# RuanJohn/Mava

Measured on AMD Instinct MI355X. Metric: env-steps/sec (whole node), ff_mappo RWARE tiny-4ag, higher is better.
Workload: dtype f32 via 2 x f16 split operands on the MFMA (3 products, f32 accumulate); 1 GPU; ff_mappo RWARE tiny-4ag-shaped synthetic obs, 4096 envs/GPU (update_batch_size=1 x num_envs=4096), rollout_length=128, ppo_epochs=4, num_minibatches=2, agents=4, obs=70/264, actions=5, one step = one PPO update = 524288 env-steps per GPU; parallelism=dp1

## Files before the change

### include/mava_hip.h

```cpp
#ifndef MAVA_HIP_H
#define MAVA_HIP_H

#include <stddef.h>
#include <stdint.h>

#ifdef __cplusplus
extern "C" {
#endif

typedef struct ihipStream_t* mava_stream_t;

const char* mava_last_error(void);
int mava_abi_version(void);

typedef struct mava_ctx mava_ctx;
enum {
  MAVA_CTX_MATMUL_MODE = 0,
  MAVA_CTX_CRITIC_AGGREGATION = 1,
  MAVA_CTX_GAE_VARIANT = 2,
  MAVA_CTX_POLICY_VARIANT = 3,
  MAVA_CTX_H2_LAUNCHES = 4,
  MAVA_CTX_TRAIN_VARIANT = 5,
  MAVA_CTX_W8_LAUNCHES = 6,
  MAVA_CTX_W1_SPLIT_FRESH = 7,
  MAVA_CTX_EXACT_TILES = 8
};
int mava_ctx_create(mava_ctx** out);
int mava_ctx_destroy(mava_ctx* ctx);
int mava_ctx_set(mava_ctx* ctx, int key, long value);
int mava_ctx_get(const mava_ctx* ctx, int key, long* value);

int mava_gae_f32(const mava_ctx* ctx, const float* reward, const float* value, const uint8_t* done,
                 const float* last_val, const uint8_t* last_done, int T, int N, float gamma,
                 float lambda, float* adv, float* tgt, mava_stream_t s);

int mava_permutation_i32(long n, uint64_t seed, uint64_t counter, int32_t* out, mava_stream_t s);

int mava_clip_adam(float* p, const float* g, float* m, float* v, int32_t* count,
                   const int* seg_off, const float* seg_lr, int n_seg, float grad_scale,
                   float max_norm, int decay, int steps_per_update, int num_updates, float b1,
                   float b2, float eps, const float* loss_sums, float vf_coef, float ent_coef,
                   float* metrics_out, mava_stream_t s);

size_t mava_ppo_finish_workspace_bytes(int Pa, int Pc);
int mava_ppo_finish_f32(mava_ctx* ctx, const float* slab_a, long stride_a, const float* slab_c, long stride_c, int n_slab,
                        int Pa, int Pc, float* g, float* p, float* m, float* v, int32_t* count, float lr_a, float lr_c,
                        float grad_scale, float max_norm, int decay, int steps_per_update, int num_updates, float b1,
                        float b2, float eps, float vf_coef, float ent_coef, float* metrics_out, int critic_din,
                        void* workspace, size_t workspace_bytes, mava_stream_t s);

int mava_slab_reduce_f32(const float* slab, int n_slab, long slab_stride, int n, int accumulate,
                         float* out, mava_stream_t s);

int mava_slab_reduce2_f32(const float* slab, int n_slab, long slab_stride, int n_main,
                          float* out_main, int n_tail, float* out_tail, int accumulate,
                          mava_stream_t s);

int mava_mlp_param_count(int din, int n_out);

int mava_mlp_forward_f32(const mava_ctx* ctx, const float* params, int din, int n_out, const float* x, int x_share,
                         int rows, float* out, mava_stream_t s);

int mava_policy_step_f32(const mava_ctx* ctx, const float* actor_params, int actor_din, int n_actions,
                         const float* agents_view, const uint8_t* action_mask,
                         const float* critic_params, int critic_din, const float* critic_input,
                         int critic_share, int critic_rows, int value_broadcast, int rows,
                         uint64_t seed, uint32_t step, const uint32_t* step_base, uint32_t row_offset, int greedy,
                         const int32_t* forced_action, int32_t* action, float* log_prob,
                         float* value, float* logits, mava_stream_t s);


int mava_adv_stats_blocks(void);

int mava_adv_stats_f64(const float* advantages, const int32_t* idx, long idx_base, int Rb, int A,
                       double* partials, mava_stream_t s);
int mava_adv_stats_batched_f64(const float* advantages, const int32_t* idx, long idx_stride, int Rb, int A,
                               int n_batch, double* partials, mava_stream_t s);

int mava_ppo_actor_grad_f32(mava_ctx* ctx, const float* params, int din, int n_actions, const float* agents_view,
                            const uint8_t* action_mask, const int32_t* action,
                            const float* old_log_prob, const float* advantages,
                            const double* adv_stats, const int32_t* idx, long idx_base, int Rb,
                            int A, float clip_eps, float ent_coef, float* slab, long slab_stride,
                            int n_slab, mava_stream_t s);

int mava_policy_step_continuous_f32(const mava_ctx* ctx, const float* actor_params, int actor_din, int action_dim, float min_scale,
                                    const float* agents_view, const float* critic_params, int critic_din,
                                    const float* critic_input, int critic_share, int critic_rows,
                                    int value_broadcast, int rows, uint64_t seed, uint32_t step,
                                    const uint32_t* step_base, uint32_t row_offset, int greedy,
                                    const float* forced_action, float* action, float* log_prob, float* value,
                                    float* mean, mava_stream_t s);
int mava_ppo_actor_grad_continuous_f32(const float* params, int din, int action_dim, float min_scale, const float* agents_view,
                                       const float* action, const float* old_log_prob, const float* advantages,
                                       const double* adv_stats, const int32_t* idx, long idx_base, int Rb, int A,
                                       float clip_eps, float ent_coef, uint64_t seed, uint32_t ent_step,
                                       uint32_t row_offset, float* slab, long slab_stride, int n_slab,
                                       mava_stream_t s);

int mava_ppo_critic_grad_f32(mava_ctx* ctx, const float* params, int din, const float* critic_input, int x_share,
                             const float* old_value, const float* targets, const int32_t* idx,
                             long idx_base, int Rb, int A, float clip_eps, float vf_coef,
                             float* slab, long slab_stride, int n_slab, mava_stream_t s);


int mava_synth_rware_step(int E, int A, int O, int n_actions, int gs_tiles, int state_dim, int time_limit,
                          uint64_t seed, uint32_t t, const uint32_t* t_base, uint32_t env_offset, int is_reset,
                          int32_t* step_count, float* run_return, int32_t* run_length,
                          float* ep_return, int32_t* ep_length, float* agents_view,
                          float* global_state, uint8_t* action_mask, int32_t* obs_step_count,
                          float* reward, uint8_t* done, float* info_return, int32_t* info_length,
                          uint8_t* info_terminal, const int32_t* action, int reward_mode, mava_stream_t s);

int mava_lbf_step(int E, int A, int F, int G, int fov, int max_agent_level, int force_coop, int individual_rewards,
                  int time_limit, uint64_t seed, uint32_t t, const uint32_t* t_base, uint32_t env_offset, int is_reset,
                  int32_t* agent_pos, int32_t* agent_level, int32_t* food_pos, int32_t* food_level, uint8_t* food_alive,
                  float* total_food_level, int32_t* step_count, float* run_return, int32_t* run_length,
                  float* ep_return, int32_t* ep_length, float* agents_view, float* global_state,
                  uint8_t* action_mask, int32_t* obs_step_count, float* reward, uint8_t* done, float* info_return,
                  int32_t* info_length, uint8_t* info_terminal, const int32_t* action, mava_stream_t s);

int mava_lbf_step_real_next(int E, int A, int F, int G, int fov, int max_agent_level, int force_coop, int individual_rewards,
                            int time_limit, uint64_t seed, uint32_t t, const uint32_t* t_base, uint32_t env_offset, int is_reset,
                            int32_t* agent_pos, int32_t* agent_level, int32_t* food_pos, int32_t* food_level, uint8_t* food_alive,
                            float* total_food_level, int32_t* step_count, float* run_return, int32_t* run_length,
                            float* ep_return, int32_t* ep_length, float* agents_view, float* global_state,
                            uint8_t* action_mask, int32_t* obs_step_count, float* reward, uint8_t* done, float* info_return,
                            int32_t* info_length, uint8_t* info_terminal, const int32_t* action, float* real_view,
                            uint8_t* real_mask, uint8_t* terminated, mava_stream_t s);

int mava_rware_step(int E, int A, int S, int R, int H, int W, int sensor_range, int time_limit, int collision_terminates,
                    const uint32_t* highway_rows, const int32_t* shelf_home, uint64_t seed, uint32_t t,
                    const uint32_t* t_base, uint32_t env_offset, int is_reset, int32_t* agent_pos, int32_t* agent_dir,
                    int32_t* agent_carry, int32_t* shelf_pos, int32_t* request_queue, int32_t* step_count,
                    float* run_return, int32_t* run_length, float* ep_return, int32_t* ep_length, float* agents_view,
                    float* global_state, uint8_t* action_mask, int32_t* obs_step_count, float* reward, uint8_t* done,
                    float* info_return, int32_t* info_length, uint8_t* info_terminal, const int32_t* action,
                    mava_stream_t s);

int mava_rware_step_real_next(int E, int A, int S, int R, int H, int W, int sensor_range, int time_limit,
                              int collision_terminates, const uint32_t* highway_rows, const int32_t* shelf_home,
                              uint64_t seed, uint32_t t, const uint32_t* t_base, uint32_t env_offset, int is_reset,
                              int32_t* agent_pos, int32_t* agent_dir, int32_t* agent_carry, int32_t* shelf_pos,
                              int32_t* request_queue, int32_t* step_count, float* run_return, int32_t* run_length,
                              float* ep_return, int32_t* ep_length, float* agents_view, float* global_state,
                              uint8_t* action_mask, int32_t* obs_step_count, float* reward, uint8_t* done,
                              float* info_return, int32_t* info_length, uint8_t* info_terminal, const int32_t* action,
                              float* real_view, uint8_t* real_mask, uint8_t* terminated, mava_stream_t s);

int mava_connector_step(int E, int A, int G, int time_limit, uint64_t seed, uint32_t t, const uint32_t* t_base,
                        uint32_t env_offset, int is_reset, int32_t* head, int32_t* target, uint8_t* connected,
                        uint8_t* grid, int32_t* step_count, float* run_return, int32_t* run_length, float* ep_return,
                        int32_t* ep_length, float* agents_view, float* global_state, uint8_t* action_mask,
                        int32_t* obs_step_count, float* reward, uint8_t* done, float* info_return, int32_t* info_length,
                        uint8_t* info_terminal, const int32_t* action, mava_stream_t s);

int mava_connector_step_real_next(int E, int A, int G, int time_limit, uint64_t seed, uint32_t t, const uint32_t* t_base,
                                  uint32_t env_offset, int is_reset, int32_t* head, int32_t* target, uint8_t* connected,
                                  uint8_t* grid, int32_t* step_count, float* run_return, int32_t* run_length,
                                  float* ep_return, int32_t* ep_length, float* agents_view, float* global_state,
                                  uint8_t* action_mask, int32_t* obs_step_count, float* reward, uint8_t* done,
                                  float* info_return, int32_t* info_length, uint8_t* info_terminal, const int32_t* action,
                                  float* real_view, uint8_t* real_mask, uint8_t* terminated, mava_stream_t s);

int mava_cleaner_step(int E, int A, int R, int C, int time_limit, uint64_t seed, uint32_t t, const uint32_t* t_base,
                      uint32_t env_offset, int is_reset, int32_t* pos, uint8_t* grid, int32_t* step_count,
                      float* run_return, int32_t* run_length, float* ep_return, int32_t* ep_length, float* agents_view,
                      float* global_state, uint8_t* action_mask, int32_t* obs_step_count, float* reward, uint8_t* done,
                      float* info_return, int32_t* info_length, uint8_t* info_terminal, uint8_t* info_won,
                      const int32_t* action, mava_stream_t s);

int mava_cleaner_step_real_next(int E, int A, int R, int C, int time_limit, uint64_t seed, uint32_t t,
                                const uint32_t* t_base, uint32_t env_offset, int is_reset, int32_t* pos, uint8_t* grid,
                                int32_t* step_count, float* run_return, int32_t* run_length, float* ep_return,
                                int32_t* ep_length, float* agents_view, float* global_state, uint8_t* action_mask,
                                int32_t* obs_step_count, float* reward, uint8_t* done, float* info_return,
                                int32_t* info_length, uint8_t* info_terminal, uint8_t* info_won, const int32_t* action,
                                float* real_view, uint8_t* real_mask, uint8_t* terminated, mava_stream_t s);

int mava_smax_step(int E, int A, int Ne, uint64_t ally_types, uint64_t enemy_types, int time_limit, int see_enemy_actions,
                   int walls_cause_death, uint64_t seed, uint32_t t, const uint32_t* t_base, uint32_t env_offset,
                   int is_reset, float* pos, float* health, int32_t* cd, int32_t* last_action, int32_t* step_count,
                   float* run_return, int32_t* run_length, float* ep_return, int32_t* ep_length, float* agents_view,
                   float* global_state, uint8_t* action_mask, int32_t* obs_step_count, float* reward, uint8_t* done,
                   float* info_return, int32_t* info_length, uint8_t* info_terminal, uint8_t* info_won,
                   const int32_t* action, mava_stream_t s);

int mava_smax_step_real_next(int E, int A, int Ne, uint64_t ally_types, uint64_t enemy_types, int time_limit,
                             int see_enemy_actions, int walls_cause_death, uint64_t seed, uint32_t t,
                             const uint32_t* t_base, uint32_t env_offset, int is_reset, float* pos, float* health,
                             int32_t* cd, int32_t* last_action, int32_t* step_count, float* run_return,
                             int32_t* run_length, float* ep_return, int32_t* ep_length, float* agents_view,
                             float* global_state, uint8_t* action_mask, int32_t* obs_step_count, float* reward,
                             uint8_t* done, float* info_return, int32_t* info_length, uint8_t* info_terminal,
                             uint8_t* info_won, const int32_t* action, float* real_view, uint8_t* real_mask,
                             uint8_t* terminated, mava_stream_t s);

int mava_spread_step(int E, int A, int add_agent_id, int time_limit, uint64_t seed, uint32_t t, const uint32_t* t_base,
                     uint32_t env_offset, int is_reset, float* agent_pos, float* landmark_pos, int32_t* step_count,
                     float* run_return, int32_t* run_length, float* ep_return, int32_t* ep_length, float* agents_view,
                     float* global_state, uint8_t* action_mask, int32_t* obs_step_count, float* reward, uint8_t* done,
                     float* info_return, int32_t* info_length, uint8_t* info_terminal, const float* action,
                     mava_stream_t s);

int mava_spread_step_real_next(int E, int A, int add_agent_id, int time_limit, uint64_t seed, uint32_t t,
                               const uint32_t* t_base, uint32_t env_offset, int is_reset, float* agent_pos,
                               float* landmark_pos, int32_t* step_count, float* run_return, int32_t* run_length,
                               float* ep_return, int32_t* ep_length, float* agents_view, float* global_state,
                               uint8_t* action_mask, int32_t* obs_step_count, float* reward, uint8_t* done,
                               float* info_return, int32_t* info_length, uint8_t* info_terminal, const float* action,
                               float* real_view, uint8_t* real_mask, uint8_t* terminated, float* real_state,
                               mava_stream_t s);

int mava_rollout_ff_f32(const float* actor_params, int n_actions, const float* critic_params, int critic_shared,
                        int E, int A, int O, int T, int time_limit, uint64_t policy_seed, uint64_t env_seed,
                        uint32_t t0, uint32_t row_offset, uint32_t env_offset, int reward_mode,
                        int32_t* step_count, float* run_return, int32_t* run_length, float* ep_return,
                        int32_t* ep_length, float* agents_view, float* global_state, uint8_t* action_mask,
                        int32_t* obs_step_count, int32_t* action, float* value, float* reward, float* log_prob,
                        uint8_t* done, float* last_val, float* info_return, int32_t* info_length,
                        uint8_t* info_terminal, float* adv, float* tgt, float gamma, float gae_lambda, mava_stream_t s);


int mava_rec_dense_f32(const mava_ctx* ctx, const float* x, int x_rowmajor, const int32_t* idx, int Rm, int E, int A,
                       int x_share, int x_ld, int accumulate, const float* w, int ldw, const float* bias,
                       const float* gate, float* y, int y_ld, int K, int N, int rows, int relu, mava_stream_t s);

int mava_rec_xty_f32(const mava_ctx* ctx, const float* x, int x_rowmajor, const int32_t* idx, int Rm, int E, int A,
                     int x_share, int x_ld, const float* y, int y_ld, const float* y_tail, int y_split, int y_tail_ld, int K, int N,
                     int rows, int want_bias, float out_scale, float* slab, long slab_stride, int n_slab, mava_stream_t s);
int mava_rec_gather_t32_f32(const float* x, const int32_t* idx, int Rm, int E, int A, int x_share, int x_ld, int K,
                            int rows, int k_pad, float* out, mava_stream_t s);

int mava_gru_scan_fwd_f32(const mava_ctx* ctx, int T, int Rm, int E, int A, const int32_t* idx, const uint8_t* done,
                          const float* h0, int h0_t32, const float* wh, const float* bhn,
                          const float* gi, float* hs, float* hprev, float* saved, mava_stream_t s);

int mava_gru_scan_bwd_f32(const mava_ctx* ctx, int T, int Rm, int E, int A, const int32_t* idx, const uint8_t* done,
                          const float* wh, const float* saved, const float* hprev, const float* dh_out,
                          float* dgi, float* dgh, int dgh_n_only, mava_stream_t s);

int mava_seq_actor_loss_f32(int T, int Rm, int E, int A, int n_actions, const int32_t* idx,
                            const float* logits, const uint8_t* mask, const int32_t* action,
                            const float* old_log_prob, const float* advantages, const double* adv_stats,
                            int n_stats, float clip_eps, float ent_coef, float grad_scale, float* dlogits,
                            float* loss_partials, int n_blocks, mava_stream_t s);
int mava_seq_actor_loss_continuous_f32(int T, int Rm, int E, int A, int action_dim, float min_scale, const int32_t* idx,
                                       const float* mean, const float* log_std, const float* log_std_rows,
                                       const float* action, const float* old_log_prob, const float* advantages,
                                       const double* adv_stats, int n_stats, float clip_eps, float ent_coef, uint64_t seed,
                                       uint32_t ent_step, uint32_t row_offset, float grad_scale, float* dmean,
                                       float* dlog_std_rows, float* loss_partials, float* dscale_partials, int n_blocks,
                                       mava_stream_t s);
int mava_seq_sample_continuous_f32(int rows, int action_dim, float min_scale, const float* mean, const float* log_std,
                                   const float* log_std_rows, uint64_t seed,
                                   uint32_t step, uint32_t row_offset, int greedy, float* action, float* log_prob,
                                   mava_stream_t s);
int mava_seq_critic_loss_f32(int T, int Rm, int E, int A, int agents_per_row, const int32_t* idx, const float* values,
                             const float* old_value, const float* targets, float clip_eps, float vf_coef,
                             float grad_scale, float* dvalues, float* loss_partials, int n_blocks, mava_stream_t s);

int mava_rec_out_f32(int T, int Rm, int E, int A, int n_out, int agents_per_row, const int32_t* idx, const float* hs,
                     const float* params_post_head, const uint8_t* mask, const int32_t* action, const float* f0,
                     const float* f1, const double* adv_stats, int n_stats, float clip_eps, float coef, float grad_scale,
                     int is_actor, float* dh, float* slab, long slab_stride, int n_slab, mava_stream_t s);

int mava_seq_sample_f32(int rows, int n_actions, const float* logits, const uint8_t* mask, uint64_t seed,
                        uint32_t step, uint32_t row_offset, int greedy, int32_t* action, float* log_prob,
                        mava_stream_t s);

int mava_rec_step_f32(const float* actor_params, int actor_din, int n_actions, const float* agents_view,
                      const uint8_t* action_mask, const uint8_t* done_a, const float* h_actor_in,
                      float* h_actor_out, int rows_a, uint64_t seed, uint32_t step, uint32_t row_offset,
                      int greedy, int32_t* action, float* log_prob, const float* critic_params, int critic_din,
                      const float* critic_input, int critic_share, const uint8_t* done_c, int done_c_stride,
                      const float* h_critic_in, float* h_critic_out, int rows_c, int value_broadcast,
                      float* value, mava_stream_t s);
int mava_rec_step_continuous_f32(const float* actor_params, int actor_din, int action_dim, float min_scale, const float* agents_view,
                                 const uint8_t* done_a, const float* h_actor_in, float* h_actor_out, int rows_a,
                                 uint64_t seed, uint32_t step, uint32_t row_offset, int greedy, float* action,
                                 float* log_prob, const float* critic_params, int critic_din,
                                 const float* critic_input, int critic_share, const uint8_t* done_c, int done_c_stride,
                                 const float* h_critic_in, float* h_critic_out, int rows_c, int value_broadcast,
                                 float* value, mava_stream_t s);

long mava_rec_step_pack_bytes(int din);
int mava_rec_step_pack_f32(const float* params, int din, void* pack, mava_stream_t s);
int mava_rec_step_packed_f32(const void* pack_a, const void* pack_c, const float* actor_params, int actor_din,
                             int n_actions, float min_scale, const float* agents_view, const uint8_t* action_mask, const uint8_t* done_a,
                             const float* h_actor_in, float* h_actor_out, int rows_a, uint64_t seed, uint32_t step,
                             uint32_t row_offset, int greedy, int32_t* action, float* action_f, float* log_prob,
                             const float* critic_params, int critic_din, const float* critic_input, int critic_share,
                             const uint8_t* done_c, int done_c_stride, const float* h_critic_in, float* h_critic_out,
                             int rows_c, int value_broadcast, float* value, mava_stream_t s);

int mava_rec_q_step_f32(const float* params, int din, int n_actions, const float* agents_view, const uint8_t* action_mask,
                        const uint8_t* done, const float* h_in, float* h_out, int rows, float eps, uint64_t seed, uint32_t step,
                        uint32_t row_offset, int32_t* action, float* q_out, mava_stream_t s);
int mava_replay_add_f32(int E, int A, int O, int n_actions, int capacity, int slot, const float* obs, const uint8_t* action_mask,
                        const int32_t* action, const float* reward, const uint8_t* terminal, const uint8_t* term_or_trunc,
                        const float* next_obs, const uint8_t* next_mask, float* b_obs, uint8_t* b_mask, int32_t* b_action,
                        float* b_reward, uint8_t* b_terminal, uint8_t* b_term_or_trunc, float* b_next_obs,
                        uint8_t* b_next_mask, mava_stream_t s);
int mava_replay_sample_f32(int E, int A, int O, int n_actions, int capacity, uint32_t n_added, int B, int S, int Rp, uint64_t seed,
                           uint32_t counter, const float* b_obs, const uint8_t* b_mask, const int32_t* b_action,
                           const float* b_reward, const uint8_t* b_terminal, const uint8_t* b_term_or_trunc,
                           const float* b_next_obs, const uint8_t* b_next_mask, float* obs, uint8_t* action_mask, int32_t* action,
                           float* reward, uint8_t* terminal, uint8_t* term_or_trunc, float* next_obs, uint8_t* next_mask,
                           int32_t* pairs, mava_stream_t s);
int mava_q_td_loss_f32(int L, int Rp, int n_actions, int n_real, const float* q, const float* q_next_online,
                       const float* q_next_target, const int32_t* action, const float* reward, const uint8_t* terminal_next,
                       const uint8_t* next_mask, float gamma, float grad_scale, float* dq, float* partials, int nblk,
                       mava_stream_t s);
int mava_target_update_f32(long n, const float* online, float* target, float tau, int hard, mava_stream_t s);

int mava_qmix_state_t32_f32(int L, int B, int A, int O, int Rp, int k_pad, const float* obs, const float* next_obs, float* state,
                            float* next_state, mava_stream_t s);
int mava_qmix_td_f32(int mode, int L, int B, int A, int Rp, int n_actions, int Em, const float* q, const float* q_next_online,
                     const float* q_next_target, const int32_t* action, const float* reward, const uint8_t* terminal_next,
                     const uint8_t* next_mask, const float* w1, const float* b1, const float* w2, const float* b2,
                     const float* w1_target, const float* b1_target, const float* w2_target, const float* b2_target, float gamma,
                     float grad_scale, float* dq, float* d_w1, float* d_b1, float* d_w2, float* d_b2, float* partials, int nblk,
                     mava_stream_t s);

int mava_sac_replay_add_f32(int E, int A, int O, int D, int S, int capacity, int head, const float* obs, const float* action,
                            const float* reward, const uint8_t* done, const float* next_obs, const float* gs,
                            const float* next_gs, float* b_obs, float* b_action, float* b_reward, uint8_t* b_done,
                            float* b_next_obs, float* b_gs, float* b_next_gs, mava_stream_t s);
int mava_sac_replay_sample_f32(int A, int O, int D, int S, int capacity, uint32_t n_added, int B, int Rp, uint64_t seed,
                               uint32_t counter, const float* b_obs, const float* b_action, const float* b_reward,
                               const uint8_t* b_done, const float* b_next_obs, const float* b_gs, const float* b_next_gs,
                               float* obs, float* action, float* reward, uint8_t* done, float* next_obs, float* gs,
                               float* next_gs, int32_t* index, mava_stream_t s);
int mava_sac_sample_f32(int rows, int n_real, int action_dim, float min_scale, const float* mean, const float* log_std,
                        uint64_t seed, uint32_t step, uint32_t row_offset, float* action, float* log_prob, float* eps,
                        mava_stream_t s);
int mava_sac_concat_f32(int rows, int n_real, int O, int x_share, int A, int action_dim, int joint, const float* state,
                        const float* action, const float* action_new, float* x, int x_ld, mava_stream_t s);
int mava_sac_q_loss_f32(int rows, int n_real, int A, const float* q1, const float* q2, const float* q1_target,
                        const float* q2_target, const float* log_prob_next, const float* reward, const uint8_t* done,
                        const float* log_alpha, float gamma, float grad_scale, float* dq1, float* dq2, float* target,
                        float* partials, int nblk, mava_stream_t s);
int mava_sac_actor_grad_f32(int rows, int n_real, int A, int action_dim, float min_scale, const float* mean,
                            const float* log_std, const float* eps, const float* action, const float* log_alpha,
                            const float* q1, const float* q2, const float* dx1, const float* dx2, int K, int action_offset,
                            int joint, float q_scale, float grad_scale, float* dmean, float* dlog_std, float* partials,
                            int nblk, mava_stream_t s);
int mava_sac_alpha_loss_f32(int n_real, int A, const float* log_prob, const float* log_alpha, float target_entropy,
                            float* grad, float* loss_parts, mava_stream_t s);

int mava_t32_convert_f32(const float* src, int N, int rows, int to_t32, float* dst, mava_stream_t s);

int mava_t32_norm_act_f32(const float* x, int N, long rows, int use_layer_norm, const float* ln_bias, int act, float* y,
                          float* xhat, float* rstd, mava_stream_t s);
int mava_t32_norm_act_bwd_f32(const float* dy, const float* y, int N, long rows, int use_layer_norm, const float* xhat,
                              const float* rstd, int act, float* dz, float* dx, mava_stream_t s);
int mava_t32_gru_mask_f32(const float* h, const uint8_t* done_t, const int32_t* idx, int E, int A, int Hd, long rows,
                          float* hprev, mava_stream_t s);
int mava_t32_gru_gates_f32(const float* gi, const float* gh, const float* bhn, const float* hprev, int Hd, long rows, float* hs,
                           float* saved, float* hprev_next, const uint8_t* done_next, const int32_t* idx, int E, int A,
                           mava_stream_t s);
int mava_t32_gru_gates_bwd_f32(const float* saved, const float* hprev, const float* dh_out, const float* acc_next,
                               const float* dhp_next, const uint8_t* done_next, const int32_t* idx, int E, int A, int Hd,
                               long rows, float* dgi, float* dgh, float* dhp, mava_stream_t s);
int mava_t32_colsum_f32(const float* y, int N, long rows, float scale, float* slab, long slab_stride, int n_slab,
                        mava_stream_t s);
int mava_t32_im2col_f32(const float* src, int src_flat, long samples, int Hin, int Win, int C, int k, int stride,
                        float* dst, mava_stream_t s);
int mava_t32_col2im_f32(const float* dcol, int src_flat, long samples, int Hin, int Win, int C, int k, int stride,
                        float* dsrc, mava_stream_t s);
int mava_t32_flatten_f32(const float* src, long samples, int P, int C, int to_flat, float* dst, mava_stream_t s);

int mava_mat_attn_fwd_f32(const float* q, const float* k, const float* v, long rows, int D, int B, int A, int n_head,
                          int causal, float* y, float* p, int n_blocks, mava_stream_t s);
int mava_mat_attn_bwd_f32(const float* dy, const float* q, const float* k, const float* v, long rows, int D, int B, int A,
                          int n_head, int causal, float* dq, float* dk, float* dv, int n_blocks, mava_stream_t s);
int mava_mat_ln_fwd_f32(const float* x, const float* res, const float* scale, const float* bias, int N, long rows,
                        long valid_rows, float* y, float* xhat, float* rstd, int n_blocks, mava_stream_t s);
int mava_mat_ln_bwd_f32(const float* dy, const float* xhat, const float* rstd, const float* scale, int N, long rows,
                        long valid_rows, float out_scale, float* dx, float* slab, long slab_stride, int n_slab, mava_stream_t s);
int mava_mat_gelu_f32(const float* x, long n, float* y, mava_stream_t s);
int mava_mat_gelu_bwd_f32(const float* dy, const float* x, long n, float* dx, mava_stream_t s);
int mava_mat_shift_onehot_f32(const int32_t* action, const int32_t* idx, int B, int A, int n_actions, int known, long rows,
                              int n_pad, float* out, mava_stream_t s);
int mava_mat_sample_f32(int B, int A, int agent, int n_actions, const float* logits, const uint8_t* mask, uint64_t seed,
                        uint32_t step, uint32_t row_offset, int greedy, int32_t* action, float* log_prob, mava_stream_t s);
int mava_mat_loss_f32(int Bm, int A, int n_actions, long rows, const int32_t* idx, const float* logits, const float* values,
                      const uint8_t* mask, const int32_t* action, const float* old_log_prob, const float* advantages,
                      const float* old_value, const float* targets, const double* adv_stats, int n_stats, float clip_eps,
                      float ent_coef, float vf_coef, float grad_scale, float* dlogits, float* dvalues, float* loss_partials,
                      int n_blocks, mava_stream_t s);

int mava_comm_unique_id(uint8_t* id128);
int mava_comm_create(void** h, int rank, int world, const uint8_t* id128);
int mava_allreduce_sum_f32(void* h, float* buf, size_t n, mava_stream_t s);
int mava_broadcast_f32(void* h, float* buf, size_t n, int root, mava_stream_t s);
int mava_comm_destroy(void* h);

#ifdef __cplusplus
}
#endif
#endif
```

### mava_amd/_lib.py

```python
from __future__ import annotations

import ctypes as C
import os
from typing import Optional

import torch

_HERE = os.path.dirname(os.path.abspath(__file__))
LIB_PATH = os.environ.get("MAVA_LIB_PATH") or os.path.join(_HERE, "libmavahip.so")

_lib: Optional[C.CDLL] = None


class MavaHipError(RuntimeError):
    pass


vp = C.c_void_p
i32 = C.c_int
u32 = C.c_uint32
u64 = C.c_uint64
f32 = C.c_float
lng = C.c_long

_SIGNATURES = {
    "mava_abi_version": [],
    "mava_ctx_create": [vp],
    "mava_ctx_destroy": [vp],
    "mava_ctx_set": [vp, i32, lng],
    "mava_ctx_get": [vp, i32, vp],
    "mava_gae_f32": [vp, vp, vp, vp, vp, vp, i32, i32, f32, f32, vp, vp, vp],
    "mava_permutation_i32": [lng, u64, u64, vp, vp],
    "mava_clip_adam": [vp, vp, vp, vp, vp, C.POINTER(i32), C.POINTER(f32), i32, f32, f32, i32, i32, i32,
                       f32, f32, f32, vp, f32, f32, vp, vp],
    "mava_slab_reduce_f32": [vp, i32, lng, i32, i32, vp, vp],
    "mava_ppo_finish_workspace_bytes": [i32, i32],
    "mava_ppo_finish_f32": [vp, vp, lng, vp, lng, i32, i32, i32, vp, vp, vp, vp, vp, f32, f32, f32, f32, i32, i32, i32, f32, f32, f32,
                            f32, f32, vp, i32, vp, C.c_size_t, vp],
    "mava_slab_reduce2_f32": [vp, i32, lng, i32, vp, i32, vp, i32, vp],
    "mava_mlp_param_count": [i32, i32],
    "mava_mlp_forward_f32": [vp, vp, i32, i32, vp, i32, i32, vp, vp],
    "mava_policy_step_f32": [vp, vp, i32, i32, vp, vp, vp, i32, vp, i32, i32, i32, i32, u64, u32, vp, u32, i32,
                             vp, vp, vp, vp, vp, vp],
    "mava_policy_step_continuous_f32": [vp, vp, i32, i32, f32, vp, vp, i32, vp, i32, i32, i32, i32, u64, u32, vp, u32, i32, vp, vp, vp, vp, vp, vp],
    "mava_ppo_actor_grad_continuous_f32": [vp, i32, i32, f32, vp, vp, vp, vp, vp, vp, lng, i32, i32, f32, f32, u64, u32, u32, vp, lng, i32, vp],
    "mava_seq_actor_loss_continuous_f32": [i32, i32, i32, i32, i32, f32, vp, vp, vp, vp, vp, vp, vp, vp, i32, f32, f32, u64, u32, u32, f32, vp, vp, vp, vp, i32, vp],
    "mava_seq_sample_continuous_f32": [i32, i32, f32, vp, vp, vp, u64, u32, u32, i32, vp, vp, vp],
    "mava_adv_stats_blocks": [],
    "mava_adv_stats_f64": [vp, vp, lng, i32, i32, vp, vp],
    "mava_adv_stats_batched_f64": [vp, vp, lng, i32, i32, i32, vp, vp],
    "mava_ppo_actor_grad_f32": [vp, vp, i32, i32, vp, vp, vp, vp, vp, vp, vp, lng, i32, i32, f32, f32, vp, lng, i32,
                                vp],
    "mava_ppo_critic_grad_f32": [vp, vp, i32, vp, i32, vp, vp, vp, lng, i32, i32, f32, f32, vp, lng, i32, vp],
    "mava_synth_rware_step": [i32, i32, i32, i32, i32, i32, i32, u64, u32, vp, u32, i32] + [vp] * 14 + [vp, i32, vp],
    "mava_lbf_step": [i32] * 9 + [u64, u32, vp, u32, i32] + [vp] * 21 + [vp],
    "mava_lbf_step_real_next": [i32] * 9 + [u64, u32, vp, u32, i32] + [vp] * 24 + [vp],
    "mava_rware_step": [i32] * 9 + [vp, vp, u64, u32, vp, u32, i32] + [vp] * 20 + [vp],
    "mava_rware_step_real_next": [i32] * 9 + [vp, vp, u64, u32, vp, u32, i32] + [vp] * 23 + [vp],
    "mava_connector_step": [i32] * 4 + [u64, u32, vp, u32, i32] + [vp] * 19 + [vp],
    "mava_connector_step_real_next": [i32] * 4 + [u64, u32, vp, u32, i32] + [vp] * 22 + [vp],
    "mava_cleaner_step": [i32] * 5 + [u64, u32, vp, u32, i32] + [vp] * 18 + [vp],
    "mava_cleaner_step_real_next": [i32] * 5 + [u64, u32, vp, u32, i32] + [vp] * 21 + [vp],
    "mava_smax_step": [i32] * 3 + [u64, u64] + [i32] * 3 + [u64, u32, vp, u32, i32] + [vp] * 20 + [vp],
    "mava_smax_step_real_next": [i32] * 3 + [u64, u64] + [i32] * 3 + [u64, u32, vp, u32, i32] + [vp] * 23 + [vp],
    "mava_spread_step": [i32] * 4 + [u64, u32, vp, u32, i32] + [vp] * 17 + [vp],
    "mava_spread_step_real_next": [i32] * 4 + [u64, u32, vp, u32, i32] + [vp] * 21 + [vp],
    "mava_rec_q_step_f32": [vp, i32, i32, vp, vp, vp, vp, vp, i32, f32, u64, u32, u32, vp, vp, vp],
    "mava_replay_add_f32": [i32] * 6 + [vp] * 16 + [vp],
    "mava_replay_sample_f32": [i32] * 5 + [u32, i32, i32, i32, u64, u32] + [vp] * 17 + [vp],
    "mava_q_td_loss_f32": [i32, i32, i32, i32] + [vp] * 7 + [f32, f32, vp, vp, i32, vp],
    "mava_target_update_f32": [lng, vp, vp, f32, i32, vp],
    "mava_qmix_state_t32_f32": [i32] * 6 + [vp] * 4 + [vp],
    "mava_qmix_td_f32": [i32] * 7 + [vp] * 15 + [f32, f32] + [vp] * 6 + [i32, vp],
    "mava_sac_replay_add_f32": [i32] * 7 + [vp] * 14 + [vp],
    "mava_sac_replay_sample_f32": [i32] * 5 + [u32, i32, i32, u64, u32] + [vp] * 15 + [vp],
    "mava_sac_sample_f32": [i32, i32, i32, f32, vp, vp, u64, u32, u32, vp, vp, vp, vp],
    "mava_sac_concat_f32": [i32] * 7 + [vp] * 4 + [i32, vp],
    "mava_sac_q_loss_f32": [i32] * 3 + [vp] * 8 + [f32, f32] + [vp] * 4 + [i32, vp],
    "mava_sac_actor_grad_f32": [i32] * 4 + [f32] + [vp] * 9 + [i32, i32, i32, f32, f32] + [vp] * 3 + [i32, vp],
    "mava_sac_alpha_loss_f32": [i32, i32, vp, vp, f32, vp, vp, vp],
    "mava_rollout_ff_f32": [vp, i32, vp, i32, i32, i32, i32, i32, i32, u64, u64, u32, u32, u32, i32] + [vp] * 18 + [vp, vp, f32, f32, vp],
    "mava_rec_dense_f32": [vp, vp, i32, vp, i32, i32, i32, i32, i32, i32, vp, i32, vp, vp, vp, i32, i32, i32, i32, i32, vp],
    "mava_rec_xty_f32": [vp, vp, i32, vp, i32, i32, i32, i32, i32, vp, i32, vp, i32, i32, i32, i32, i32, i32, f32, vp, lng, i32, vp],
    "mava_rec_gather_t32_f32": [vp, vp, i32, i32, i32, i32, i32, i32, i32, i32, vp, vp],
    "mava_gru_scan_fwd_f32": [vp, i32, i32, i32, i32, vp, vp, vp, i32, vp, vp, vp, vp, vp, vp, vp],
    "mava_t32_gru_mask_f32": [vp, vp, vp, i32, i32, i32, lng, vp, vp],
    "mava_t32_gru_gates_f32": [vp, vp, vp, vp, i32, lng, vp, vp, vp, vp, vp, i32, i32, vp],
    "mava_t32_gru_gates_bwd_f32": [vp, vp, vp, vp, vp, vp, vp, i32, i32, i32, lng, vp, vp, vp, vp],
    "mava_gru_scan_bwd_f32": [vp, i32, i32, i32, i32, vp, vp, vp, vp, vp, vp, vp, vp, i32, vp],
    "mava_seq_actor_loss_f32": [i32, i32, i32, i32, i32, vp, vp, vp, vp, vp, vp, vp, i32, f32, f32, f32, vp, vp, i32, vp],
    "mava_rec_step_continuous_f32": [vp, i32, i32, f32, vp, vp, vp, vp, i32, u64, u32, u32, i32, vp, vp, vp, i32, vp, i32, vp, i32, vp, vp, i32, i32, vp, vp],
    "mava_rec_step_f32": [vp, i32, i32, vp, vp, vp, vp, vp, i32, u64, u32, u32, i32, vp, vp, vp, i32, vp, i32, vp, i32, vp, vp,
                          i32, i32, vp, vp],
    "mava_seq_critic_loss_f32": [i32, i32, i32, i32, i32, vp, vp, vp, vp, f32, f32, f32, vp, vp, i32, vp],
    "mava_rec_out_f32": [i32, i32, i32, i32, i32, i32, vp, vp, vp, vp, vp, vp, vp, vp, i32, f32, f32, f32, i32, vp, vp, lng, i32, vp],
    "mava_rec_step_pack_bytes": [i32],
    "mava_t32_norm_act_f32": [vp, i32, lng, i32, vp, i32, vp, vp, vp, vp],
    "mava_t32_norm_act_bwd_f32": [vp, vp, i32, lng, i32, vp, vp, i32, vp, vp, vp],
    "mava_t32_colsum_f32": [vp, i32, lng, f32, vp, lng, i32, vp],
    "mava_t32_im2col_f32": [vp, i32, lng, i32, i32, i32, i32, i32, vp, vp],
    "mava_t32_col2im_f32": [vp, i32, lng, i32, i32, i32, i32, i32, vp, vp],
    "mava_t32_flatten_f32": [vp, lng, i32, i32, i32, vp, vp],
    "mava_comm_unique_id": [vp],
    "mava_comm_create": [vp, i32, i32, vp],
    "mava_allreduce_sum_f32": [vp, vp, C.c_size_t, vp],
    "mava_broadcast_f32": [vp, vp, C.c_size_t, i32, vp],
    "mava_comm_destroy": [vp],
    "mava_rec_step_pack_f32": [vp, i32, vp, vp],
    "mava_rec_step_packed_f32": [vp, vp, vp, i32, i32, f32, vp, vp, vp, vp, vp, i32, u64, u32, u32, i32, vp, vp, vp, vp, i32, vp, i32, vp, i32, vp, vp, i32, i32, vp, vp],
    "mava_seq_sample_f32": [i32, i32, vp, vp, u64, u32, u32, i32, vp, vp, vp],
    "mava_t32_convert_f32": [vp, i32, i32, i32, vp, vp],
    "mava_mat_attn_fwd_f32": [vp, vp, vp, lng, i32, i32, i32, i32, i32, vp, vp, i32, vp],
    "mava_mat_attn_bwd_f32": [vp, vp, vp, vp, lng, i32, i32, i32, i32, i32, vp, vp, vp, i32, vp],
    "mava_mat_ln_fwd_f32": [vp, vp, vp, vp, i32, lng, lng, vp, vp, vp, i32, vp],
    "mava_mat_ln_bwd_f32": [vp, vp, vp, vp, i32, lng, lng, f32, vp, vp, lng, i32, vp],
    "mava_mat_gelu_f32": [vp, lng, vp, vp],
    "mava_mat_gelu_bwd_f32": [vp, vp, lng, vp, vp],
    "mava_mat_shift_onehot_f32": [vp, vp, i32, i32, i32, i32, lng, i32, vp, vp],
    "mava_mat_sample_f32": [i32, i32, i32, i32, vp, vp, u64, u32, u32, i32, vp, vp, vp],
    "mava_mat_loss_f32": [i32, i32, i32, lng, vp, vp, vp, vp, vp, vp, vp, vp, vp, vp, i32, f32, f32, f32, f32, vp, vp, vp, i32, vp],
}
_RESTYPES = {"mava_last_error": C.c_char_p, "mava_rec_step_pack_bytes": C.c_long, "mava_ppo_finish_workspace_bytes": C.c_size_t}


def declared_symbols():
    return sorted(set(_SIGNATURES) | set(_RESTYPES))


def lib() -> C.CDLL:
    global _lib
    if _lib is None:
        if not os.path.exists(LIB_PATH):
            raise MavaHipError(
                f"{LIB_PATH} is missing: build it with `python -m mava_amd.build` "
                "(hipcc --offload-arch=gfx950). There is no CPU fallback."
            )
        _lib = C.CDLL(LIB_PATH)
        _lib.mava_last_error.restype = C.c_char_p
        _lib.mava_last_error.argtypes = []
        for name, args in _SIGNATURES.items():
            fn = getattr(_lib, name)
            fn.argtypes = args
            fn.restype = _RESTYPES.get(name, C.c_int)
    return _lib


class Ctx:

    MATMUL_MODE, CRITIC_AGGREGATION, GAE_VARIANT, POLICY_VARIANT, H2_LAUNCHES, TRAIN_VARIANT, W8_LAUNCHES, W1_SPLIT_FRESH = 0, 1, 2, 3, 4, 5, 6, 7
    EXACT_TILES = 8

    def __init__(self, matmul_mode: str = "f32", critic_aggregation: bool = True):
        if matmul_mode not in ("f32", "f16x2"):
            raise ValueError(f"matmul_mode must be 'f16x2' or 'f32', got {matmul_mode!r}")
        h = C.c_void_p()
        check(lib().mava_ctx_create(C.byref(h)), "mava_ctx_create")
        self.handle: Optional[int] = h.value
        self.set(self.MATMUL_MODE, 1 if matmul_mode == "f16x2" else 0)
        self.set(self.CRITIC_AGGREGATION, int(bool(critic_aggregation)))

    def set(self, key: int, value: int) -> None:
        check(lib().mava_ctx_set(self.handle, key, int(value)), "mava_ctx_set")

    def get(self, key: int) -> int:
        out = C.c_long()
        check(lib().mava_ctx_get(self.handle, key, C.byref(out)), "mava_ctx_get")
        return int(out.value)

    @property
    def matmul_mode(self) -> str:
        return "f16x2" if self.get(self.MATMUL_MODE) == 1 else "f32"

    @property
    def h2_launches(self) -> int:
        return self.get(self.H2_LAUNCHES)

    def close(self) -> None:
        if getattr(self, "handle", None) is not None and _lib is not None:
            _lib.mava_ctx_destroy(self.handle)
        self.handle = None

    def __del__(self):
        try:
            self.close()
        except Exception:
            pass


def ctx_ptr(ctx: Optional["Ctx"]) -> Optional[int]:
    return None if ctx is None else ctx.handle


def check(rc: int, what: str) -> None:
    if rc != 0:
        msg = lib().mava_last_error().decode("utf-8", "replace")
        raise MavaHipError(f"{what} failed with code {rc}: {msg}")


TIMERS: Optional[dict] = None


def launch(what: str, fn, *args, ok=(0,)) -> int:
    if TIMERS is None:
        rc = fn(*args)
    else:
        a, b = torch.cuda.Event(enable_timing=True), torch.cuda.Event(enable_timing=True)
        a.record()
        rc = fn(*args)
        b.record()
        TIMERS.setdefault(what, []).append((a, b))
    if rc not in ok:
        check(rc, what)
    return rc


def ptr(t: Optional[torch.Tensor]) -> Optional[int]:
    if t is None:
        return None
    return t.data_ptr()


def stream_ptr() -> int:
    return torch.cuda.current_stream().cuda_stream
```

### mava_amd/csrc/permutation.hip

```cpp
#include "common.h"

namespace {

constexpr int PERM_ROUNDS = 16;

struct PermKeys {
  uint32_t k[PERM_ROUNDS];
};

__device__ __host__ inline uint32_t perm_mix(uint32_t x, uint32_t k) {
  uint32_t h = x + k;
  h ^= h >> 16;
  h *= 0x7FEB352Du;
  h ^= h >> 15;
  h *= 0x846CA68Bu;
  h ^= h >> 16;
  return h;
}

__global__ __launch_bounds__(256) void permutation_kernel(uint32_t n, int lb, int rb, PermKeys keys,
                                                          int32_t* __restrict__ out) {
  const uint32_t i = blockIdx.x * 256u + threadIdx.x;
  if (i >= n) return;
  const uint32_t mask_r = (1u << rb) - 1u;
  uint32_t v = i;
  do {
    uint32_t L = v >> rb, R = v & mask_r;
#pragma unroll
    for (int r = 0; r < PERM_ROUNDS; r += 2) {
      L ^= perm_mix(R, keys.k[r]) >> (32 - lb);
      R ^= perm_mix(L, keys.k[r + 1]) >> (32 - rb);
    }
    v = (L << rb) | R;
  } while (v >= n);
  out[i] = (int32_t)v;
}

}

extern "C" int mava_permutation_i32(long n, uint64_t seed, uint64_t counter, int32_t* out, hipStream_t s) {
  MAVA_ARG_CHECK(n >= 1 && n < (1L << 31), 0, "mava_permutation_i32: n=%ld (1 <= n < 2^31)", n);
  MAVA_ARG_CHECK(out, 1, "mava_permutation_i32: null pointer argument");
  int b = 2;
  while ((1L << b) < n) ++b;
  const int lb = b >> 1, rb = b - lb;
  PermKeys keys;
  uint64_t st = seed + 0x9E3779B97F4A7C15ull * (counter + 1);
  for (int r = 0; r < PERM_ROUNDS; ++r) {
    st += 0x9E3779B97F4A7C15ull;
    uint64_t z = st;
    z = (z ^ (z >> 30)) * 0xBF58476D1CE4E5B9ull;
    z = (z ^ (z >> 27)) * 0x94D049BB133111EBull;
    z ^= z >> 31;
    keys.k[r] = (uint32_t)(z >> 32);
  }
  hipLaunchKernelGGL(permutation_kernel, dim3(mava_cdiv(n, 256)), dim3(256), 0, s, (uint32_t)n, lb, rb, keys, out);
  MAVA_LAUNCH_CHECK();
  return MAVA_OK;
}
```

### mava_amd/csrc/ppo_train.hip

```cpp
#include "mlp_core.h"
#include "ppo_train_task.h"
#include "ctx.h"
#include "tanh_normal.h"

namespace {

constexpr int STATS_BLOCKS = 128;
constexpr int LDT = 33;


#ifdef MAVA_STAMPS
#define STAMP_DECL unsigned long long st_prev = __builtin_readcyclecounter(), st_acc[16] = {0, 0, 0, 0, 0, 0, 0, 0, 0, 0, 0, 0, 0, 0, 0, 0};
#define STAMP(i)                                                   \
  do {                                                             \
    const unsigned long long st_now = __builtin_readcyclecounter(); \
    st_acc[i] += st_now - st_prev;                                 \
    st_prev = st_now;                                              \
  } while (0)
#else
#define STAMP_DECL
#define STAMP(i)
#endif

struct TrainLdsLayout {
  int h1t, h2t, dz2t, dz1t, yp, dy, xs, misc, end;
  int ldx;
};

template <int NO>
TrainLdsLayout make_layout(int kt1) {
  TrainLdsLayout L;
  const int tile = MLP_H * LDT;
  L.h1t = MlpLds<NO>::END;
  L.h2t = L.h1t + tile;
  L.dz2t = L.h2t + tile;
  L.yp = L.dz2t + tile;
  L.dy = L.yp + 4 * 32 * (NO + 1);
  L.ldx = 32 * kt1 + 4;
  L.xs = (L.dy + 32 * LDT + 3) & ~3;
  L.misc = L.xs + 32 * L.ldx;
  L.end = L.misc + 16;
  L.dz1t = L.h2t;
  if ((size_t)(L.end + tile) * sizeof(float) <= 163840) {
    L.dz1t = L.end;
    L.end += tile;
  }
  return L;
}

__global__ __launch_bounds__(256) void adv_stats_kernel(const float* __restrict__ adv,
                                                        const int32_t* __restrict__ idx,
                                                        long idx_base, int Rb, int A,
                                                        double* __restrict__ partials, long idx_stride) {
  __shared__ double sh[2][4];
  if (idx) idx += (long)blockIdx.y * idx_stride;
  partials += (long)blockIdx.y * 2 * gridDim.x;
  double s1 = 0.0, s2 = 0.0;
  const long stride = (long)gridDim.x * 256;
  for (long b0 = (long)blockIdx.x * 256 + threadIdx.x; b0 < Rb; b0 += 4 * stride) {
    long p[4];
#pragma unroll
    for (int u = 0; u < 4; ++u) {
      const long b = b0 + u * stride;
      const long bc = b < Rb ? b : b0;
      p[u] = idx ? (long)idx[bc] : idx_base + bc;
    }
#pragma unroll
    for (int u = 0; u < 4; ++u) {
      if (b0 + u * stride < Rb) {
        const float* row = adv + p[u] * A;
        for (int a = 0; a < A; ++a) {
          const double v = (double)row[a];
          s1 += v;
          s2 += v * v;
        }
      }
    }
  }
  for (int o = 32; o > 0; o >>= 1) {
    s1 += __shfl_down(s1, o, 64);
    s2 += __shfl_down(s2, o, 64);
  }
  const int lane = threadIdx.x & 63, w = threadIdx.x >> 6;
  if (lane == 0) { sh[0][w] = s1; sh[1][w] = s2; }
  __syncthreads();
  if (threadIdx.x == 0) {
    partials[2 * blockIdx.x + 0] = ((sh[0][0] + sh[0][1]) + sh[0][2]) + sh[0][3];
    partials[2 * blockIdx.x + 1] = ((sh[1][0] + sh[1][1]) + sh[1][2]) + sh[1][3];
  }
}

template <int V, int NR>
__device__ __forceinline__ void stage_load(const float* __restrict__ xrow, int nv, int l8, float (&xr)[NR]) {
#pragma unroll
  for (int i = 0; i < NR / V; ++i) {
    const int c = l8 + 8 * i;
    const int cc = (c < nv) ? c : 0;
    if (V == 4) {
      const float4 v = reinterpret_cast<const float4*>(xrow)[cc];
      xr[4 * i + 0] = v.x; xr[4 * i + 1] = v.y; xr[4 * i + 2] = v.z; xr[4 * i + 3] = v.w;
    } else {
      xr[i] = xrow[cc];
    }
  }
}
template <int V, int NR>
__device__ __forceinline__ void stage_write(float* xs_row, float* dummy, int nv, int l8, const float (&xr)[NR]) {
#pragma unroll
  for (int i = 0; i < NR / V; ++i) {
    const int c = l8 + 8 * i;
    float* q = (c < nv) ? (xs_row + V * c) : dummy;
    if (V == 4) {
      *reinterpret_cast<float4*>(q) = make_float4(xr[4 * i + 0], xr[4 * i + 1], xr[4 * i + 2], xr[4 * i + 3]);
    } else {
      *q = xr[i];
    }
  }
}

template <int CTRL>
__device__ __forceinline__ float dpp_f(float v) {
  return __builtin_bit_cast(float, __builtin_amdgcn_update_dpp(0, __builtin_bit_cast(int, v), CTRL, 0xF, 0xF, true));
}
template <int G, typename Op>
__device__ __forceinline__ float group_allreduce(float v, Op op) {
  v = op(v, dpp_f<0xB1>(v));
  v = op(v, dpp_f<0x4E>(v));
  if (G >= 8) v = op(v, dpp_f<0x141>(v));
  if (G >= 16) v = op(v, dpp_f<0x140>(v));
  if (G >= 32) v = op(v, __shfl_xor(v, 16, 64));
  return v;
}

template <int NO, int KT1, bool ACTOR, int XV, bool CONT>
__global__ __launch_bounds__(256, 1) void ppo_train_kernel(TrainTask tk, TrainLdsLayout L) {
  static_assert(!CONT || ACTOR, "the continuous head belongs to the actor");
  extern __shared__ __attribute__((aligned(16))) float lds[];
  float* const W2s = lds + MlpLds<NO>::W2;
  float* const W3s = lds + MlpLds<NO>::W3;
  float* const H1T = lds + L.h1t;
  float* const H2T = lds + L.h2t;
  float* const DZ1T = lds + L.dz1t;
  float* const DZ2T = lds + L.dz2t;
  float* const YP = lds + L.yp;
  float* const DY = lds + L.dy;
  float* const XS = lds + L.xs;
  float* const misc = lds + L.misc;
  constexpr int ldx = 32 * KT1 + 4;

  const int tid = threadIdx.x;
  const int lane = tid & 63, w = tid >> 6, h = lane >> 5, j = lane & 31;
  const int srow = tid >> 3, l8 = tid & 7;
  const int din = tk.din, no = tk.no;
  const long R = (!ACTOR && tk.agg > 1) ? (long)tk.Rb : (long)tk.Rb * tk.A;
  const float invR = 1.0f / (float)((long)tk.Rb * tk.A);
  constexpr int NR = 4 * KT1;

  mlp_fill_lds<NO>(lds, tk.params, din, no, 256);
  for (int i = tid; i < 32 * ldx; i += 256) XS[i] = 0.0f;
  for (int i = tid; i < 32 * LDT; i += 256) DY[i] = 0.0f;
  __syncthreads();
  if (tid < 32) XS[tid * ldx + din] = 1.0f;
  if (ACTOR && tid == 0) {
    double s1 = 0.0, s2 = 0.0;
    for (int i = 0; i < STATS_BLOCKS; ++i) { s1 += tk.stats[2 * i]; s2 += tk.stats[2 * i + 1]; }
    const double mean = s1 / (double)R;
    double var = s2 / (double)R - mean * mean;
    if (var < 0.0) var = 0.0;
    misc[0] = (float)mean;
    misc[1] = 1.0f / ((float)sqrt(var) + 1e-8f);
  }
  __syncthreads();
  const float adv_mean = ACTOR ? misc[0] : 0.0f;
  const float adv_rstd = ACTOR ? misc[1] : 0.0f;

  const float* const wcol1 = tk.params + 32 * w + j;
  const int fbase = 32 * w + 4 * h;

  f32x16 gW1[KT1], gW2[4];
#pragma unroll
  for (int t = 0; t < KT1; ++t)
#pragma unroll
    for (int r = 0; r < 16; ++r) gW1[t][r] = 0.0f;
#pragma unroll
  for (int t = 0; t < 4; ++t)
#pragma unroll
    for (int r = 0; r < 16; ++r) gW2[t][r] = 0.0f;
  f32x16 gW3;
#pragma unroll
  for (int r = 0; r < 16; ++r) gW3[r] = 0.0f;
  float w3h[16];
#pragma unroll
  for (int r = 0; r < 16; ++r) {
    const int f = fbase + (r & 3) + 8 * (r >> 2);
    w3h[r] = ACTOR ? ((j < NO) ? W3s[f * NO + j] : 0.0f) : W3s[f];
  }
  float w3a[ACTOR ? NO / 2 : 1];
#pragma unroll
  for (int s2 = 0; s2 < (ACTOR ? NO / 2 : 1); ++s2)
    w3a[s2] = ACTOR ? W3s[(32 * w + j) * NO + 2 * s2 + h] : 0.0f;
  float ab3 = 0.0f;
  float ab2[16], aW3r[ACTOR ? 1 : 16];
#pragma unroll
  for (int r = 0; r < 16; ++r) ab2[r] = 0.0f;
#pragma unroll
  for (int r = 0; r < (ACTOR ? 1 : 16); ++r) aW3r[r] = 0.0f;
  float loss_a = 0.f, loss_b = 0.f;
  float als = 0.0f;
  const float ls_raw = CONT ? tk.params[mlp_param_count(tk.din, tk.no) + ((lane & (NO - 1)) < tk.no ? (lane & (NO - 1)) : 0)] : 0.0f;
  const float sc_lo = CONT ? tn::scale_of(ls_raw, tk.min_scale) : 1.0f;


  constexpr int NP = ACTOR ? NO / 8 : 1;
  constexpr int GR = ACTOR ? 64 / NO : 32;
  const int lo = ACTOR ? (lane & (NO - 1)) : 0;
  auto loss_row = [&](int q) -> int { return ACTOR ? (8 * w + q * GR + lane / NO) : j; };
  const int slot = 2 * w + h;
  const int slot_c = (!ACTOR && tk.agg > 1) ? (slot < tk.agg ? slot : 0) : 0;
  auto load_row = [&](long fr, int& act, float& f0, float& f1, uint32_t& m) {
    if (ACTOR && CONT) {
      act = __builtin_bit_cast(int, tk.action_f[fr * no + (lo < no ? lo : 0)]);
      f0 = tk.old_logp[fr];
      f1 = tk.adv[fr];
      m = (uint32_t)fr;
    } else if (ACTOR) {
      act = tk.action[fr];
      f0 = tk.old_logp[fr];
      f1 = tk.adv[fr];
      const uint8_t* mk = (tk.mask != nullptr && lo < no) ? (tk.mask + fr * no + lo) : nullptr;
      m = 1u;
      if (mk != nullptr) m = *mk;
    } else {
      act = 0;
      const long fa = (tk.agg > 1) ? fr * tk.agg + slot_c : fr;
      f0 = tk.old_value[fa];
      f1 = tk.targets[fa];
      m = 0u;
    }
  };
  const uint32_t Au = (!ACTOR && tk.agg > 1) ? 1u : (uint32_t)tk.A;

  const uint32_t q_step = 32u * gridDim.x, b_step = q_step / Au, a_step = q_step % Au;
  const uint32_t b_last = (uint32_t)(R - 1) / Au, a_last = (uint32_t)(R - 1) % Au;
  struct Cursor { uint32_t q, b, a; };
  auto cursor_at = [&](int r) {
    Cursor c;
    c.q = 32u * blockIdx.x + (uint32_t)r;
    c.b = c.q / Au;
    c.a = c.q - c.b * Au;
    return c;
  };
  auto cursor_advance = [&](Cursor& c) {
    c.q += q_step; c.b += b_step; c.a += a_step;
    if (c.a >= Au) { c.a -= Au; c.b += 1u; }
  };
  auto cursor_gather = [&](const Cursor& c, int32_t& p_raw, uint32_t& a_out) {
    const bool in = c.q < (uint32_t)R;
    const uint32_t b = in ? c.b : b_last;
    a_out = in ? c.a : a_last;
    p_raw = tk.idx ? tk.idx[b] : (int32_t)(tk.idx_base + (long)b);
  };
  auto stage_row = [&](int32_t p_raw, uint32_t a) -> uint32_t {
    const uint32_t fr = (uint32_t)p_raw * Au + a;
    return (tk.xshare == 1) ? fr : ((uint32_t)tk.xshare == Au ? (uint32_t)p_raw : fr / (uint32_t)tk.xshare);
  };
  float* const xs_dummy = misc + 4;
  auto stage_issue = [&](uint32_t xrow_idx, float (&xr)[NR]) {
    stage_load<XV, NR>(tk.x + (long)xrow_idx * din, din / XV, l8, xr);
  };
  auto stage_commit = [&](const float (&xr)[NR]) {
    stage_write<XV, NR>(XS + srow * ldx, xs_dummy, din / XV, l8, xr);
  };

  constexpr int RD = (2 * KT1 <= 6) ? (2 * KT1) : (((2 * KT1) % 6 == 0) ? 6 : 4);
  constexpr bool W1_RESIDENT = (RD == 2 * KT1);
  float wr[RD][8];
  const float* const wcol1h = wcol1 + 8 * h * MLP_H;
#pragma unroll
  for (int d = 0; d < RD; ++d)
#pragma unroll
    for (int s = 0; s < 8; ++s) wr[d][s] = wcol1h[(16 * d + s) * MLP_H];

  const long ntiles = (R + 31) / 32;
  long it = blockIdx.x;
  float xr[NR];
  int r_act[NP] = {}, n_act[NP] = {};
  float r_f0[NP] = {}, r_f1[NP] = {}, n_f0[NP] = {}, n_f1[NP] = {};
  uint32_t r_m[NP] = {}, n_m[NP] = {};
  Cursor cs = cursor_at(srow), cl[NP];
#pragma unroll
  for (int q = 0; q < NP; ++q) cl[q] = cursor_at(loss_row(q));
  int32_t ps_next = 0, pl_next[NP] = {};
  uint32_t as_next = 0, al_next[NP] = {};
  if (it < ntiles) {
    cursor_gather(cs, ps_next, as_next);
    stage_issue(stage_row(ps_next, as_next), xr);
#pragma unroll
    for (int q = 0; q < NP; ++q) {
      cursor_gather(cl[q], pl_next[q], al_next[q]);
      load_row((long)((uint32_t)pl_next[q] * Au + al_next[q]), r_act[q], r_f0[q], r_f1[q], r_m[q]);
    }
    stage_commit(xr);
    cursor_advance(cs);
#pragma unroll
    for (int q = 0; q < NP; ++q) cursor_advance(cl[q]);
    if (it + gridDim.x < ntiles) {
      cursor_gather(cs, ps_next, as_next);
#pragma unroll
      for (int q = 0; q < NP; ++q) cursor_gather(cl[q], pl_next[q], al_next[q]);
      cursor_advance(cs);
#pragma unroll
      for (int q = 0; q < NP; ++q) cursor_advance(cl[q]);
    }
  }
  __syncthreads();

  STAMP_DECL
  for (; it < ntiles; it += gridDim.x) {
    STAMP(9);
    const bool valid = (it * 32 + j) < R;
    const long itn = it + gridDim.x;
    const bool have_next = itn < ntiles;
    uint32_t xrow_next = stage_row(ps_next, as_next);
    uint32_t fr_next[NP];
#pragma unroll
    for (int q = 0; q < NP; ++q) fr_next[q] = (uint32_t)pl_next[q] * Au + al_next[q];
    asm volatile("" : "+v"(xrow_next));
#pragma unroll
    for (int q = 0; q < NP; ++q) asm volatile("" : "+v"(fr_next[q]));

    f32x16 h1;
#pragma unroll
    for (int r = 0; r < 16; ++r) h1[r] = 0.0f;
    {
      const float* xb = XS + j * ldx + 8 * h;
      constexpr int NB = 2 * KT1;
      static_assert(NB % RD == 0, "ring depth must divide the batch count");
      float xo[RD][8];
      {
        const float4 v0 = *reinterpret_cast<const float4*>(xb), v1 = *reinterpret_cast<const float4*>(xb + 4);
        xo[0][0] = v0.x; xo[0][1] = v0.y; xo[0][2] = v0.z; xo[0][3] = v0.w;
        xo[0][4] = v1.x; xo[0][5] = v1.y; xo[0][6] = v1.z; xo[0][7] = v1.w;
      }
#pragma unroll 1
      for (int g = 0; g < NB / RD; ++g) {
#pragma unroll
        for (int d = 0; d < RD; ++d) {
          const int b = g * RD + d;
          const int bn = (b + 1 < NB) ? (b + 1) : b;
          {
            const float4 v0 = *reinterpret_cast<const float4*>(xb + 16 * bn);
            const float4 v1 = *reinterpret_cast<const float4*>(xb + 16 * bn + 4);
            float(&xn)[8] = xo[(d + 1) % RD];
            xn[0] = v0.x; xn[1] = v0.y; xn[2] = v0.z; xn[3] = v0.w;
            xn[4] = v1.x; xn[5] = v1.y; xn[6] = v1.z; xn[7] = v1.w;
          }
          if (16 * b <= din) {
#pragma unroll
            for (int s = 0; s < 8; ++s) h1 = MFMA32(wr[d][s], xo[d][s], h1);
          }
          if (!W1_RESIDENT) {
            int bf = b - 1 + RD;
            bf = (bf >= NB) ? (bf - NB) : bf;
            const float* wb = wcol1h + bf * (16 * MLP_H);
#pragma unroll
            for (int s = 0; s < 8; ++s) wr[(d + RD - 1) % RD][s] = wb[s * MLP_H];
          }
          __builtin_amdgcn_sched_barrier(0);
        }
      }
      if (!W1_RESIDENT) {
#pragma unroll
        for (int s = 0; s < 8; ++s) wr[RD - 1][s] = wcol1h[(16 * (RD - 1) + s) * MLP_H];
      }
    }
    STAMP(12);
    uint32_t relu1 = 0;
// ... 557 lines not shown
```

### mava_amd/csrc/rollout_h2.hip

```cpp
#include "h2_core.h"

#ifdef MAVA_STAMPS
#define RSTAMP_DECL unsigned long long rs_prev = __builtin_readcyclecounter(), rs_acc[8] = {0, 0, 0, 0, 0, 0, 0, 0};
#define RSTAMP(i)                                                   \
  do {                                                              \
    __builtin_amdgcn_sched_barrier(0);                              \
    const unsigned long long rs_now = __builtin_readcyclecounter(); \
    rs_acc[i] += rs_now - rs_prev;                                  \
    rs_prev = rs_now;                                               \
    __builtin_amdgcn_sched_barrier(0);                              \
  } while (0)
static __device__ unsigned long long g_rollout_stamps[16];
#else
#define RSTAMP_DECL
#define RSTAMP(i)
#endif

namespace {
using namespace h2;
typedef _Float16 half2v __attribute__((ext_vector_type(2)));

constexpr uint32_t ENV_STREAM = 0x454E5653u;
constexpr uint32_t POLICY_STREAM = 0x504f4c49u;

struct RolloutArgs {
  const float* pa;
  const float* pc;
  int E, A, O, no, T, time_limit;
  uint32_t pseed_lo, pseed_hi, eseed_lo, eseed_hi;
  uint32_t t0;
  uint32_t row_offset;
  uint32_t env_offset;
  int reward_mode;
  int32_t* step_count;
  float* run_return; int32_t* run_length; float* ep_return; int32_t* ep_length;
  float* agents_view;
  float* global_state;
  uint8_t* action_mask;
  int32_t* obs_step_count;
  int32_t* action; float* value; float* reward; float* log_prob; uint8_t* done;
  float* last_val;
  float* info_return; int32_t* info_length; uint8_t* info_terminal;
  float* adv; float* tgt;
  float gamma, lam;
};

struct RolloutLds {
  int xa, xa_row, xa_plane, xc, xc_row, xc_plane, h1, wl, ypa, ypc, act, mask, small, gum, xlf, end;
};
constexpr int W1_REG_STEPS = 12;

template <int NO, int S1A, int S1C, bool SHARED>
RolloutLds make_rollout_lds() {
  constexpr int KTA = (S1A + 1) / 2, KTC = (S1C + 1) / 2;
  RolloutLds L;
  L.xa = 0;
  L.xa_row = 2 * 32 * KTA + 16;
  L.xa_plane = 32 * L.xa_row;
  L.xc = L.xa + 2 * 2 * L.xa_plane;
  L.xc_row = 2 * 32 * KTC + 16;
  L.xc_plane = ((S1C > W1_REG_STEPS) ? 16 : 32) * L.xc_row;
  L.h1 = L.xc + (SHARED ? 2 * L.xc_plane : 0);
  L.wl = L.h1 + (SHARED ? 3 : 4) * IMG_BYTES;
  L.ypa = L.wl + ((S1C > W1_REG_STEPS) ? (S1C - W1_REG_STEPS) * 4 * 64 * 32 : 0);
  L.ypc = L.ypa + 2 * 4 * 32 * (NO + 1) * 4;
  L.act = L.ypc + 2 * 4 * 32 * 4;
  L.mask = L.act + 64 * 4;
  L.small = L.mask + 64 * 32;
  L.gum = L.small + (128 + 32 + 128 + 4 + 128) * 4;
  L.gum = (L.gum + 15) & ~15;
  L.xlf = L.gum + 64 * NO * 4;
  L.end = L.xlf + 16;
  L.end = (L.end + 15) & ~15;
  return L;
}

template <int NO, int S1A, int S1C, bool SHARED, int ROLE>
__device__ __forceinline__ void rollout_body(const RolloutArgs& a, const RolloutLds& L, u8* lds) {
  constexpr bool ACT_ROLE = ROLE == 0;
  const int t512 = threadIdx.x;
  const int tid = t512 & 255, lane = tid & 63, w = tid >> 6, h = lane >> 5, r = lane & 31;
  const int A = a.A, O = a.O, no = a.no, W = A + O, E = a.E;
  const int EB = 64 / A;
  const int e0 = blockIdx.x * EB;
  const int din_a = W, din_c = SHARED ? A * O : W;
  constexpr int NTC = SHARED ? 1 : 2;
  float* const B2a = reinterpret_cast<float*>(lds + L.small);
  float* const B3a = B2a + 128;
  float* const B2c = B3a + 32;
  float* const B3c = B2c + 128;
  float* const W3c = B3c + 4;
  int* const ACT = reinterpret_cast<int*>(lds + L.act);
  u8* const MASK = lds + L.mask;
  float* const GUM = reinterpret_cast<float*>(lds + L.gum);
  unsigned* const XLF = reinterpret_cast<unsigned*>(lds + L.xlf);
  float* const YPA = reinterpret_cast<float*>(lds + L.ypa);
  float* const YPC = reinterpret_cast<float*>(lds + L.ypc);
  const int xa_row = L.xa_row, xa_plane = L.xa_plane, xc_row = L.xc_row, xc_plane = L.xc_plane;

  for (int i = t512 * 16; i < L.end; i += 512 * 16) *reinterpret_cast<uint4*>(lds + i) = make_uint4(0, 0, 0, 0);
  __syncthreads();
  const int oW2a = mlp_off_w2(din_a), oW3a = mlp_off_w3(din_a), oW2c = mlp_off_w2(din_c), oW3c = mlp_off_w3(din_c);
  if (ACT_ROLE) {
    if (tid < 128) B2a[tid] = a.pa[mlp_off_b2(din_a) + tid];
    if (tid < no) B3a[tid] = a.pa[mlp_off_b3(din_a, no) + tid];
  } else {
    if (tid < 128) {
      B2c[tid] = a.pc[mlp_off_b2(din_c) + tid];
      W3c[tid] = a.pc[oW3c + tid];
    }
    if (tid == 0) B3c[0] = a.pc[mlp_off_b3(din_c, 1)];
  }
  constexpr int S1R = ACT_ROLE ? S1A : S1C;
  constexpr int S1REG = (S1R > W1_REG_STEPS) ? W1_REG_STEPS : S1R;
  constexpr int XC_ROWS = (S1C > W1_REG_STEPS) ? 16 : 32;
  uint4* const WL = reinterpret_cast<uint4*>(lds + L.wl) + 2 * (w * 64 + lane);
  const float* const PR = ACT_ROLE ? a.pa : a.pc;
  const int din_r = ACT_ROLE ? din_a : din_c, oW2r = ACT_ROLE ? oW2a : oW2c;
  Frag W1r[S1REG], W2r[8], W3h[2];
  {
    float c1 = 0.0f, c2 = 0.0f;
#pragma unroll
    for (int s = 0; s < S1R; ++s) {
      float v[8];
#pragma unroll
      for (int e = 0; e < 8; ++e) {
        const int k = 16 * s + 8 * h + e;
        v[e] = (k <= din_r) ? PR[k * MLP_H + 32 * w + r] : 0.0f;
      }
      const Frag f = split8_carry(v, c1);
      if (s < S1REG) {
        W1r[s] = f;
      } else {
        WL[512 * (s - S1REG)] = __builtin_bit_cast(uint4, f.hi);
        WL[512 * (s - S1REG) + 1] = __builtin_bit_cast(uint4, f.lo);
      }
      __builtin_amdgcn_sched_barrier(0);
    }
#pragma unroll
    for (int s = 0; s < 8; ++s) {
      float v[8];
#pragma unroll
      for (int e = 0; e < 8; ++e) v[e] = PR[oW2r + (16 * s + 8 * h + e) * MLP_H + 32 * w + r];
      W2r[s] = split8_carry(v, c2);
      __builtin_amdgcn_sched_barrier(0);
    }
#pragma unroll
    for (int s = 0; s < (ACT_ROLE ? 2 : 0); ++s) {
      float v[8];
#pragma unroll
      for (int e = 0; e < 8; ++e) {
        const int f = 32 * w + 16 * s + 8 * (e >> 2) + 4 * h + (e & 3);
        v[e] = (r < no) ? a.pa[oW3a + f * no + r] * W3_SCALE : 0.0f;
      }
      W3h[s] = split8(v);
    }
  }
  {
    const long slot0_av = 0;
    uint32_t lo_any = 0;
    for (int i = t512; i < 64 * W; i += 512) {
      const int row = i / W, c = i - row * W;
      const int e = e0 + row / A;
      const float v = (e < E) ? a.agents_view[slot0_av + ((long)e0 * A + row) * W + c] : 0.0f;
      _Float16 x0, x1;
      split1(v, x0, x1);
      u8* p = lds + L.xa + (row >> 5) * 2 * xa_plane + (row & 31) * xa_row + 2 * c;
      *reinterpret_cast<_Float16*>(p) = x0;
      *reinterpret_cast<_Float16*>(p + xa_plane) = x1;
      lo_any |= (uint32_t)__builtin_bit_cast(uint16_t, x1) & 0x7FFFu;
    }
    if (t512 < 64) {
      u8* p = lds + L.xa + (t512 >> 5) * 2 * xa_plane + (t512 & 31) * xa_row + 2 * din_a;
      *reinterpret_cast<_Float16*>(p) = (_Float16)1.0f;
    }
    if (SHARED) {
      const int gw = A * O;
      for (int i = t512; i < EB * gw; i += 512) {
        const int le = i / gw, c = i - le * gw;
        const float v = (e0 + le < E) ? a.global_state[(long)(e0 + le) * gw + c] : 0.0f;
        _Float16 x0, x1;
        split1(v, x0, x1);
        u8* p = lds + L.xc + le * xc_row + 2 * c;
        *reinterpret_cast<_Float16*>(p) = x0;
        *reinterpret_cast<_Float16*>(p + xc_plane) = x1;
        lo_any |= (uint32_t)__builtin_bit_cast(uint16_t, x1) & 0x7FFFu;
      }
      if (t512 < XC_ROWS) *reinterpret_cast<_Float16*>(lds + L.xc + t512 * xc_row + 2 * din_c) = (_Float16)1.0f;
    }
    for (int i = t512; i < 64 * no; i += 512) {
      const int row = i / no, o = i - row * no;
      MASK[row * 32 + o] = (e0 + row / A < E) ? a.action_mask[((long)e0 * A + row) * no + o] : 1;
    }
    if (lo_any != 0) *XLF = 1u;
  }
  __syncthreads();

  const int bk_le = tid / A, bk_ag = tid - bk_le * A;
  const bool bk_on = !ACT_ROLE && tid < 64 && (e0 + bk_le) < E;
  const long bk_k = (long)(e0 + bk_le) * A + bk_ag;
  int sc_reg = bk_on ? a.step_count[bk_k] : 0;
  float rr_reg = 0.0f, er_reg = 0.0f;
  int rl_reg = 0, el_reg = 0;
  if (bk_on && bk_ag == 0) {
    rr_reg = a.run_return[e0 + bk_le]; rl_reg = a.run_length[e0 + bk_le];
    er_reg = a.ep_return[e0 + bk_le]; el_reg = a.ep_length[e0 + bk_le];
  }

  const bool x_lo = __builtin_amdgcn_readfirstlane((int)*XLF) != 0;
  const int rowB = r * IMG_ROW + 16 * h;
  const long EA = (long)E * A;
  const uint32_t nch = (O - 2 + 15) / 16 > 0 ? (O - 2 + 15) / 16 : 1;

  constexpr int NT = ACT_ROLE ? 2 : NTC;
  RSTAMP_DECL
  auto forward = [&](bool active, bool noise, uint32_t noise_step) __attribute__((always_inline)) {
    f32x16 z[NT];
#pragma unroll
    for (int i = 0; i < NT; ++i)
#pragma unroll
      for (int q = 0; q < 16; ++q) z[i][q] = 0.0f;
    if (active) {
      auto x_frag = [&](int s, int t) {
        return (!ACT_ROLE && SHARED) ? read_row_frag(lds + L.xc, xc_plane, (r & (XC_ROWS - 1)) * xc_row + 16 * h + 32 * s)
                                     : read_row_frag(lds + L.xa + t * 2 * xa_plane, xa_plane, r * xa_row + 16 * h + 32 * s);
      };
      auto w_frag = [&](int s) {
        Frag wf;
        wf.hi = __builtin_bit_cast(half8, WL[512 * (s - S1REG)]);
        wf.lo = __builtin_bit_cast(half8, WL[512 * (s - S1REG) + 1]);
        return wf;
      };
      auto x_hi = [&](int s, int t) -> half8 {
        return (!ACT_ROLE && SHARED)
                   ? *reinterpret_cast<const half8*>(lds + L.xc + (r & (XC_ROWS - 1)) * xc_row + 16 * h + 32 * s)
                   : *reinterpret_cast<const half8*>(lds + L.xa + t * 2 * xa_plane + r * xa_row + 16 * h + 32 * s);
      };
      if (x_lo) {
      Frag bn[NT], wn;
#pragma unroll
      for (int t = 0; t < NT; ++t) bn[t] = x_frag(0, t);
      if (S1REG == 0) wn = w_frag(0);
#pragma unroll
      for (int s = 0; s < S1R; ++s) {
        Frag b[NT];
#pragma unroll
        for (int t = 0; t < NT; ++t) b[t] = bn[t];
        const Frag wf = (s < S1REG) ? W1r[s < S1REG ? s : 0] : wn;
        if (s + 1 < S1R) {
#pragma unroll
          for (int t = 0; t < NT; ++t) bn[t] = x_frag(s + 1, t);
          if (s + 1 >= S1REG) wn = w_frag(s + 1);
        }
#pragma unroll
        for (int t = 0; t < NT; ++t) z[t] = mfma3(wf, b[t], z[t]);
        __builtin_amdgcn_sched_barrier(0);
      }
      } else {
      half8 bn[NT];
      Frag wn;
#pragma unroll
      for (int t = 0; t < NT; ++t) bn[t] = x_hi(0, t);
      if (S1REG == 0) wn = w_frag(0);
#pragma unroll
      for (int s = 0; s < S1R; ++s) {
        half8 b[NT];
#pragma unroll
        for (int t = 0; t < NT; ++t) b[t] = bn[t];
        const Frag wf = (s < S1REG) ? W1r[s < S1REG ? s : 0] : wn;
        if (s + 1 < S1R) {
#pragma unroll
          for (int t = 0; t < NT; ++t) bn[t] = x_hi(s + 1, t);
          if (s + 1 >= S1REG) wn = w_frag(s + 1);
        }
#pragma unroll
        for (int t = 0; t < NT; ++t) {
          z[t] = __builtin_amdgcn_mfma_f32_32x32x16_f16(wf.lo, b[t], z[t], 0, 0, 0);
          z[t] = __builtin_amdgcn_mfma_f32_32x32x16_f16(wf.hi, b[t], z[t], 0, 0, 0);
        }
        __builtin_amdgcn_sched_barrier(0);
      }
      }
#pragma unroll
      for (int i = 0; i < NT; ++i) {
#pragma unroll
        for (int q = 0; q < 16; ++q) z[i][q] = fmaxf(z[i][q], 0.0f);
        half4 ph[4], pl[4];
        write_image(lds + L.h1 + ((ACT_ROLE ? 0 : 2) + i) * IMG_BYTES, r, 32 * w + 4 * h, z[i], ph, pl);
      }
    }
    if (ACT_ROLE && noise) {
      const int grow = tid >> 2, c = tid & 3;
      if (c < NO / 4) {
        const uint32_t gid = a.row_offset + (uint32_t)(e0 * A + grow);
        const Philox4 rnd = philox4x32_10(gid, noise_step, (uint32_t)c, POLICY_STREAM, a.pseed_lo, a.pseed_hi);
        float4 g;
        g.x = -logf(-logf(u01_open(rnd.x)));
        g.y = -logf(-logf(u01_open(rnd.y)));
        g.z = -logf(-logf(u01_open(rnd.z)));
        g.w = -logf(-logf(u01_open(rnd.w)));
        *reinterpret_cast<float4*>(GUM + grow * NO + 4 * c) = g;
      }
    }
    RSTAMP(0);
    __syncthreads();
    RSTAMP(1);
    if (active) {
      const float* b2 = ACT_ROLE ? B2a : B2c;
#pragma unroll
      for (int i = 0; i < NT; ++i)
#pragma unroll
        for (int q = 0; q < 16; ++q) z[i][q] = b2[32 * w + (q & 3) + 8 * (q >> 2) + 4 * h];
      {
        auto h_frag = [&](int s, int t) {
          return read_row_frag(lds + L.h1 + ((ACT_ROLE ? 0 : 2) + t) * IMG_BYTES, IMG_PLANE, rowB + 32 * s);
        };
        Frag bn[NT];
#pragma unroll
        for (int t = 0; t < NT; ++t) bn[t] = h_frag(0, t);
#pragma unroll
        for (int s = 0; s < 8; ++s) {
          Frag b[NT];
#pragma unroll
          for (int t = 0; t < NT; ++t) b[t] = bn[t];
          if (s + 1 < 8) {
#pragma unroll
            for (int t = 0; t < NT; ++t) bn[t] = h_frag(s + 1, t);
          }
#pragma unroll
          for (int t = 0; t < NT; ++t) z[t] = mfma3(W2r[s], b[t], z[t]);
          __builtin_amdgcn_sched_barrier(0);
        }
      }
      if (ACT_ROLE) {
#pragma unroll
        for (int t = 0; t < NT; ++t) {
          half4 ph[4], pl[4];
#pragma unroll
          for (int g = 0; g < 4; ++g)
#pragma unroll
            for (int e = 0; e < 4; ++e) {
              _Float16 x0, x1;
              split1(fmaxf(z[t][4 * g + e], 0.0f), x0, x1);
              ph[g][e] = x0;
              pl[g][e] = x1;
            }
          f32x16 y;
#pragma unroll
          for (int q = 0; q < 16; ++q) y[q] = 0.0f;
#pragma unroll
          for (int s = 0; s < 2; ++s) {
            Frag b;
            b.hi = __builtin_shufflevector(ph[2 * s], ph[2 * s + 1], 0, 1, 2, 3, 4, 5, 6, 7);
            b.lo = __builtin_shufflevector(pl[2 * s], pl[2 * s + 1], 0, 1, 2, 3, 4, 5, 6, 7);
            y = mfma3(W3h[s], b, y);
          }
#pragma unroll
          for (int q = 0; q < 16; ++q) {
            const int o = (q & 3) + 8 * (q >> 2) + 4 * h;
            if ((q & 3) + 8 * (q >> 2) < NO) {
              if (o < NO) YPA[((t * 4 + w) * 32 + r) * (NO + 1) + o] = y[q] * W3_UNSCALE;
            }
          }
        }
      } else {
#pragma unroll
        for (int t = 0; t < NT; ++t) {
          float4 w3g[4];
#pragma unroll
          for (int g = 0; g < 4; ++g) w3g[g] = *reinterpret_cast<const float4*>(W3c + 32 * w + 4 * h + 8 * g);
          float part = 0.0f;
#pragma unroll
          for (int q = 0; q < 16; ++q) {
            const float4 tv = w3g[q >> 2];
            const float w3 = (q & 3) == 0 ? tv.x : (q & 3) == 1 ? tv.y : (q & 3) == 2 ? tv.z : tv.w;
            part = fmaf(fmaxf(z[t][q], 0.0f), w3, part);
          }
          part += __shfl_xor(part, 32, 64);
          if (h == 0) YPC[(t * 4 + w) * 32 + r] = part;
        }
      }
    }
    RSTAMP(2);
    __syncthreads();
    RSTAMP(3);
  };
  auto value_of = [&](int crow) -> float {
    const float* yp = YPC + (crow >> 5) * 4 * 32 + (crow & 31);
    return (((yp[0] + yp[32]) + yp[64]) + yp[96]) + B3c[0];
  };

  const int rows_ok = min(64, (E - e0) * A), envs_ok = min(EB, E - e0);
  const int AO = A * O;
  auto write_out = [&](long slot, bool part_gs) {
    if (!part_gs) {
      float* dst = a.agents_view + (slot * EA + (long)e0 * A) * W;
      if ((W & 1) == 0) {
        const int W2 = W >> 1, d_r = 256 / W2, d_f = 256 - d_r * W2;
        int row = tid / W2, f = tid - row * W2;
        for (int j = tid; j < 64 * W2; j += 256) {
          if (row < rows_ok) {
            const u8* xa = lds + L.xa + (row >> 5) * 2 * xa_plane + (row & 31) * xa_row;
            const half2v v = *reinterpret_cast<const half2v*>(xa + 4 * f);
            reinterpret_cast<float2*>(dst)[j] = make_float2((float)v[0], (float)v[1]);
          }
          row += d_r; f += d_f;
          if (f >= W2) { f -= W2; ++row; }
        }
      } else {
        const int d_r = 256 / W, d_f = 256 - d_r * W;
        int row = tid / W, f = tid - row * W;
        for (int j = tid; j < 64 * W; j += 256) {
          if (row < rows_ok) {
            const u8* xa = lds + L.xa + (row >> 5) * 2 * xa_plane + (row & 31) * xa_row;
            dst[j] = (float)*reinterpret_cast<const _Float16*>(xa + 2 * f);
          }
          row += d_r; f += d_f;
          if (f >= W) { f -= W; ++row; }
        }
      }
    }
    if (part_gs && SHARED && a.global_state != nullptr) {
      float* dst = a.global_state + (slot * E + e0) * (long)AO;
      if ((AO & 3) == 0) {
        const int Q = AO >> 2, d_r = 256 / Q, d_f = 256 - d_r * Q;
        int le = tid / Q, k = tid - le * Q;
        for (int j = tid; j < EB * Q; j += 256) {
          if (le < envs_ok) {
            const half4 v = *reinterpret_cast<const half4*>(lds + L.xc + le * xc_row + 8 * k);
            reinterpret_cast<float4*>(dst)[j] = make_float4((float)v[0], (float)v[1], (float)v[2], (float)v[3]);
          }
          le += d_r; k += d_f;
          if (k >= Q) { k -= Q; ++le; }
        }
      } else {
        const int d_r = 256 / AO, d_f = 256 - d_r * AO;
        int le = tid / AO, k = tid - le * AO;
        for (int j = tid; j < EB * AO; j += 256) {
          if (le < envs_ok) dst[j] = (float)*reinterpret_cast<const _Float16*>(lds + L.xc + le * xc_row + 2 * k);
          le += d_r; k += d_f;
          if (k >= AO) { k -= AO; ++le; }
        }
      }
    }
    if (!part_gs) {
      uint8_t* dst = a.action_mask + (slot * EA + (long)e0 * A) * no;
      for (int j = tid; j < rows_ok * no; j += 256) {
        const int row = j / no, o = j - row * no;
        dst[j] = MASK[row * 32 + o];
      }
    }
  };

  for (int t = 0; t < a.T; ++t) {
    const uint32_t step = a.t0 + (uint32_t)t;
    forward(true, true, step);
    if (ACT_ROLE) {
      constexpr int RPP = 256 / NO;
#pragma unroll
      for (int pass = 0; pass < 64 / RPP; ++pass) {
        const int row = pass * RPP + tid / NO, o = tid & (NO - 1);
        const float* yp = YPA + (((row >> 5) * 4) * 32 + (row & 31)) * (NO + 1) + o;
        const float y = (((yp[0] + yp[32 * (NO + 1)]) + yp[2 * 32 * (NO + 1)]) + yp[3 * 32 * (NO + 1)]) + B3a[o];
        const bool legal = (o < no) && (MASK[row * 32 + o] != 0);
        const float z = legal ? y : -FLT_MAX;
        auto fmax_op = [](float p, float q) { return fmaxf(p, q); };
        auto add_op = [](float p, float q) { return p + q; };
        const float mx = group_allreduce<NO>(z, fmax_op);
        const float se = group_allreduce<NO>(expf(z - mx), add_op);
        const float logp = (mx == -FLT_MAX) ? ((o < no) ? -logf((float)no) : -FLT_MAX) : z - (mx + logf(se));
        float sc = (o < no) ? (z + GUM[row * NO + o]) : -FLT_MAX;
        if (!(sc > -FLT_MAX)) sc = -FLT_MAX;
        int best = o;
#pragma unroll
        for (int m = 1; m < NO; m <<= 1) {
          const float so = __shfl_xor(sc, m, 64);
          const int bo = __shfl_xor(best, m, 64);
          const bool take = (so > sc) || (so == sc && bo < best);
          sc = take ? so : sc;
          best = take ? bo : best;
        }
        const float lp = group_allreduce<NO>((o == best) ? logp : 0.0f, add_op);
        const int e = e0 + row / A;
        if (o == 0) {
          ACT[row] = best;
          if (e < E) {
            const long k = (long)t * EA + (long)e0 * A + row;
            a.action[k] = best;
            a.log_prob[k] = lp;
          }
        }
      }
    } else {
      if (tid < 64 && (e0 + tid / A) < E) {
        a.value[(long)t * EA + (long)e0 * A + tid] = value_of(SHARED ? tid / A : tid);
      }
      if (t > 0) write_out((long)t, false);
    }
    if (ACT_ROLE && t > 0) write_out((long)t, true);
    RSTAMP(4);
    __syncthreads();
    RSTAMP(5);
    {
      const uint32_t tn = step + 1;
      const long slot = (long)(t + 1);
      const uint32_t n_view = (uint32_t)(64 * nch);
      for (uint32_t i = ACT_ROLE ? (uint32_t)tid : n_view; i < n_view; i += 256) {
        const uint32_t row = i / nch, c = i - row * nch;
        const uint32_t le = row / A, ag = row - le * A, e = e0 + le;
        if ((int)e >= E) continue;
        const uint32_t ent = (a.env_offset + e) * A + ag;
        const Philox4 rv = philox4x32_10(ent, tn, c, ENV_STREAM, a.eseed_lo, a.eseed_hi);
        const uint32_t wds[4] = {rv.x, rv.y, rv.z, rv.w};
        const uint32_t f0 = 2 + 16 * c;
        const int n = (int)min(16u, (uint32_t)O - f0);
        u8* xa = lds + L.xa + (row >> 5) * 2 * xa_plane + (row & 31) * xa_row;
        u8* xc = lds + L.xc + le * xc_row + 2 * (ag * O);
        const bool pk_a = (n == 16) && (((uint32_t)A + f0) & 1u) == 0;
        const bool pk_c = (n == 16) && ((ag * (uint32_t)O + f0) & 1u) == 0;
        uint32_t pr[8];
#pragma unroll
        for (int q = 0; q < 16; q += 2) {
          const uint32_t b0 = (((wds[q >> 2] >> (8 * (q & 3))) & 0xFFu) < 51u) ? 0x3C00u : 0u;
          const uint32_t b1 = (((wds[(q + 1) >> 2] >> (8 * ((q + 1) & 3))) & 0xFFu) < 51u) ? 0x3C00u : 0u;
          pr[q >> 1] = b0 | (b1 << 16);
        }
        if (pk_a) {
#pragma unroll
          for (int q = 0; q < 8; ++q) *reinterpret_cast<uint32_t*>(xa + 2 * (A + f0) + 4 * q) = pr[q];
        } else {
#pragma unroll
          for (int q = 0; q < 16; ++q) {
            if (q < n) *reinterpret_cast<uint16_t*>(xa + 2 * (A + f0 + q)) = (uint16_t)(pr[q >> 1] >> (16 * (q & 1)));
          }
        }
        if (SHARED) {
          if (pk_c) {
#pragma unroll
            for (int q = 0; q < 8; ++q) *reinterpret_cast<uint32_t*>(xc + 2 * f0 + 4 * q) = pr[q];
          } else {
#pragma unroll
            for (int q = 0; q < 16; ++q) {
              if (q < n) *reinterpret_cast<uint16_t*>(xc + 2 * (f0 + q)) = (uint16_t)(pr[q >> 1] >> (16 * (q & 1)));
            }
          }
        }
      }
      if (!ACT_ROLE && tid >= 64 && tid < 128) {
        const uint32_t row = (uint32_t)(tid - 64);
        const uint32_t le = row / A, ag = row - le * A, e = e0 + le;
        if ((int)e < E) {
          const uint32_t ent = (a.env_offset + e) * A + ag;
          u8* xa = lds + L.xa + (row >> 5) * 2 * xa_plane + (row & 31) * xa_row;
          u8* xc = lds + L.xc + le * xc_row + 2 * (ag * O);
          const Philox4 cm = philox4x32_10(ent, tn, 0xFFFFu, ENV_STREAM, a.eseed_lo, a.eseed_hi);
          const float c0 = (float)(cm.x % 10u), c1 = (float)(cm.y % 10u);
          *reinterpret_cast<_Float16*>(xa + 2 * A) = (_Float16)c0;
          *reinterpret_cast<_Float16*>(xa + 2 * (A + 1)) = (_Float16)c1;
          if (SHARED) {
            *reinterpret_cast<_Float16*>(xc) = (_Float16)c0;
            *reinterpret_cast<_Float16*>(xc + 2) = (_Float16)c1;
          }
          const bool m1 = !((cm.z & 0xFFu) < 51u);
          for (int o = 0; o < no; ++o) MASK[row * 32 + o] = (o == 1 && no > 1) ? (m1 ? 1 : 0) : 1;
        }
      }
      if (bk_on) {
        const uint32_t env_id = a.env_offset + (uint32_t)(e0 + bk_le);
        const Philox4 ev = philox4x32_10(env_id, tn, 0u, ENV_STREAM ^ 1u, a.eseed_lo, a.eseed_hi);
        float rew = (u01_open(ev.x) < 0.02f) ? 1.0f : 0.0f;
        if (a.reward_mode == 1) {
          int hits = 0;
          for (int a2 = 0; a2 < A; ++a2) {
            const Philox4 pc2 = philox4x32_10(env_id * A + a2, tn - 1u, 0xFFFFu, ENV_STREAM, a.eseed_lo, a.eseed_hi);
            hits += (ACT[bk_le * A + a2] == (int)((pc2.x % 10u) % (uint32_t)no)) ? 1 : 0;
          }
          rew = (float)hits / (float)A;
        }
        const int sc_new = sc_reg + 1;
        const bool term = (sc_new >= a.time_limit) || (u01_open(ev.y) < 0.002f);
        const int sc_obs = term ? 0 : sc_new;
        sc_reg = sc_obs;
        a.obs_step_count[slot * EA + bk_k] = sc_obs;
        a.reward[(long)t * EA + bk_k] = rew;
        a.done[(long)t * EA + bk_k] = term ? 1 : 0;
        if (bk_ag == 0) {
          const float new_ret = rr_reg + rew;
          const int new_len = rl_reg + 1;
          er_reg = term ? new_ret : er_reg;
          el_reg = term ? new_len : el_reg;
          rr_reg = term ? 0.0f : new_ret;
          rl_reg = term ? 0 : new_len;
          const long ie = (long)t * E + e0 + bk_le;
          a.info_return[ie] = er_reg;
          a.info_length[ie] = el_reg;
          a.info_terminal[ie] = term ? 1 : 0;
        }
      }
    }
    RSTAMP(6);
    __syncthreads();
    RSTAMP(7);
  }
#ifdef MAVA_STAMPS
  if (blockIdx.x == 0 && tid == 0)
    for (int i = 0; i < 8; ++i) g_rollout_stamps[(ACT_ROLE ? 0 : 8) + i] = rs_acc[i];
#endif
  write_out((long)a.T, ACT_ROLE);
  forward(!ACT_ROLE, false, 0u);
  if (bk_on) {
    const float lv = value_of(SHARED ? tid / A : tid);
    a.last_val[bk_k] = lv;
    if (a.adv != nullptr) {
      float g = 0.0f, nv = lv;
      const float gl = a.gamma * a.lam;
      for (int tb = a.T; tb > 0; tb -= 8) {
        float rw[8], vv[8];
        uint8_t dd[8];
#pragma unroll
        for (int i = 0; i < 8; ++i) {
          const int t = tb - 1 - i;
          const long k = (long)(t >= 0 ? t : 0) * EA + bk_k;
          rw[i] = a.reward[k]; vv[i] = a.value[k]; dd[i] = a.done[k];
        }
#pragma unroll
        for (int i = 0; i < 8; ++i) {
          const int t = tb - 1 - i;
          if (t >= 0) {
            const float nd = dd[i] ? 0.0f : 1.0f;
            const float delta = rw[i] + a.gamma * nv * nd - vv[i];
            g = delta + gl * nd * g;
            const long k = (long)t * EA + bk_k;
            a.adv[k] = g;
            a.tgt[k] = g + vv[i];
            nv = vv[i];
          }
        }
      }
    }
  }
  if (bk_on) {
    a.step_count[bk_k] = sc_reg;
    if (bk_ag == 0) {
      a.run_return[e0 + bk_le] = rr_reg; a.run_length[e0 + bk_le] = rl_reg;
      a.ep_return[e0 + bk_le] = er_reg; a.ep_length[e0 + bk_le] = el_reg;
    }
  }
}

template <int NO, int S1A, int S1C, bool SHARED>
__global__ __launch_bounds__(512, 2) void rollout_h2_kernel(RolloutArgs a, RolloutLds L) {
  extern __shared__ __attribute__((aligned(16))) u8 lds[];
  if (threadIdx.x < 256) {
    rollout_body<NO, S1A, S1C, SHARED, 0>(a, L, lds);
  } else {
    rollout_body<NO, S1A, S1C, SHARED, 1>(a, L, lds);
  }
}

int g_rollout_last_instance = 0;

template <int NO, int S1A, int S1C, bool SHARED>
int launch_rollout(const RolloutArgs& a, hipStream_t s) {
  g_rollout_last_instance = NO * 100000 + S1A * 1000 + S1C * 10 + (SHARED ? 1 : 0);
  const RolloutLds L = make_rollout_lds<NO, S1A, S1C, SHARED>();
  MAVA_ARG_CHECK(L.end <= 163840, 8, "mava_rollout_ff_f32: %d bytes of LDS exceed the 160 KiB of a CU", L.end);
  const int lds_bytes = L.end > 83968 ? L.end : 83968;
  static bool attr_set = false;
  if (!attr_set) {
    MAVA_HIP_CHECK(hipFuncSetAttribute((const void*)rollout_h2_kernel<NO, S1A, S1C, SHARED>,
                                       hipFuncAttributeMaxDynamicSharedMemorySize, lds_bytes));
    attr_set = true;
  }
  const int EB = 64 / a.A;
  hipLaunchKernelGGL((rollout_h2_kernel<NO, S1A, S1C, SHARED>), dim3(mava_cdiv(a.E, EB)), dim3(512), lds_bytes, s, a, L);
  MAVA_LAUNCH_CHECK();
  return MAVA_OK;
}

}

#ifdef MAVA_STAMPS
extern "C" int mava_debug_get_rollout_stamps(unsigned long long* out16) {
  return -(int)hipMemcpyFromSymbol(out16, HIP_SYMBOL(g_rollout_stamps), 16 * sizeof(unsigned long long));
}
#endif

extern "C" int mava_debug_rollout_last_instance(void) { return g_rollout_last_instance; }

extern "C" int mava_rollout_ff_f32(const float* actor_params, int n_actions, const float* critic_params, int critic_shared,
                                   int E, int A, int O, int T, int time_limit, uint64_t policy_seed, uint64_t env_seed,
                                   uint32_t t0, uint32_t row_offset, uint32_t env_offset, int reward_mode,
                                   int32_t* step_count, float* run_return, int32_t* run_length, float* ep_return,
                                   int32_t* ep_length, float* agents_view, float* global_state, uint8_t* action_mask,
                                   int32_t* obs_step_count, int32_t* action, float* value, float* reward, float* log_prob,
                                   uint8_t* done, float* last_val, float* info_return, int32_t* info_length,
                                   uint8_t* info_terminal, float* adv, float* tgt, float gamma, float gae_lambda,
                                   hipStream_t s) {
  MAVA_ARG_CHECK(E >= 1 && A >= 1 && O >= 2 && T >= 1 && n_actions >= 1 && time_limit >= 1, 0,
                 "mava_rollout_ff_f32: bad shape E=%d A=%d O=%d T=%d nA=%d", E, A, O, T, n_actions);
  MAVA_ARG_CHECK(actor_params && critic_params && step_count && run_return && run_length && ep_return && ep_length &&
                     agents_view && action_mask && obs_step_count && action && value && reward && log_prob && done &&
                     last_val && info_return && info_length && info_terminal && (!critic_shared || global_state),
                 1, "mava_rollout_ff_f32: null pointer argument");
  if (64 % A != 0 || n_actions > 8) return 1;
  if (critic_shared && A < 2) return 1;
  const int s1a = (A + O + 1 + 15) / 16, s1c = critic_shared ? (A * O + 1 + 15) / 16 : s1a;
  RolloutArgs a = {};
  a.pa = actor_params; a.pc = critic_params; a.E = E; a.A = A; a.O = O; a.no = n_actions; a.T = T; a.time_limit = time_limit;
  a.pseed_lo = (uint32_t)policy_seed; a.pseed_hi = (uint32_t)(policy_seed >> 32);
  a.eseed_lo = (uint32_t)env_seed; a.eseed_hi = (uint32_t)(env_seed >> 32);
  a.t0 = t0; a.row_offset = row_offset; a.env_offset = env_offset; a.reward_mode = reward_mode;
  a.step_count = step_count; a.run_return = run_return; a.run_length = run_length; a.ep_return = ep_return;
  a.ep_length = ep_length; a.agents_view = agents_view; a.global_state = critic_shared ? global_state : nullptr;
  a.action_mask = action_mask; a.obs_step_count = obs_step_count; a.action = action; a.value = value; a.reward = reward;
  a.log_prob = log_prob; a.done = done; a.last_val = last_val; a.info_return = info_return; a.info_length = info_length;
  a.info_terminal = info_terminal;
  MAVA_ARG_CHECK((adv == nullptr) == (tgt == nullptr), 1, "mava_rollout_ff_f32: adv and tgt go together");
  a.adv = adv; a.tgt = tgt; a.gamma = gamma; a.lam = gae_lambda;
  if (critic_shared) {
    if (s1a == 5 && s1c == 17 && A >= 4) return launch_rollout<8, 5, 17, true>(a, s);
#ifndef MAVA_FAST_BUILD
    if (s1a <= 2 && s1c <= 2) return launch_rollout<8, 2, 2, true>(a, s);
    if (s1a <= 2 && s1c <= 4) return launch_rollout<8, 2, 4, true>(a, s);
    if (s1a <= 5 && s1c <= 9) return launch_rollout<8, 5, 9, true>(a, s);
#endif
    return 1;
  }
  if (s1a == 5) return launch_rollout<8, 5, 5, false>(a, s);
#ifndef MAVA_FAST_BUILD
  if (s1a <= 2) return launch_rollout<8, 2, 2, false>(a, s);
#endif
  return 1;
}
```

### mava_amd/learner.py

```python
from __future__ import annotations

import math
import contextlib
import os
from typing import Any, Dict, List, Optional, Tuple

import torch

from . import ops, parallel
from .guards import check_f16_range
from .learner_common import bind_learn, matmul_ctx
from .networks import FeedForwardActor, FeedForwardValueNet, MLPTorso, make_action_head
from .types import (AdamState, ExperimentOutput, LearnerState, Observation, ObservationGlobalState, OptStates, Params,
                    TimeStep)

NUM_CU = 256


def _dist_info() -> Tuple[int, int]:
    return parallel.rank_world()


class _Replica:

    def __init__(self, env, T: int, n_upd: int, critic_uses_state: bool, device, continuous: bool = False):
        E, A = env.num_envs, env.num_agents
        self.env = env
        self.state = env.alloc_state()
        d = device
        self.agents_view = torch.empty((T + 1, E, A, env.obs_dim), device=d)
        self.global_state = torch.empty((T + 1, E, env.gs_tiles, env.state_dim), device=d)
        self.action_mask = torch.empty((T + 1, E, A, env.action_dim), dtype=torch.uint8, device=d)
        self.step_count = torch.empty((T + 1, E, A), dtype=torch.int32, device=d)
        self.action = (torch.empty((T, E, A, env.action_dim), device=d) if continuous
                       else torch.empty((T, E, A), dtype=torch.int32, device=d))
        self.value = torch.empty((T, E, A), device=d)
        self.reward = torch.empty((T, E, A), device=d)
        self.log_prob = torch.empty((T, E, A), device=d)
        self.done = torch.empty((T, E, A), dtype=torch.uint8, device=d)
        self.last_val = torch.empty((E, A), device=d)
        self.adv = torch.empty((T, E, A), device=d)
        self.tgt = torch.empty((T, E, A), device=d)
        self.info_return = torch.zeros((n_upd, T, E), device=d)
        self.info_length = torch.zeros((n_upd, T, E), dtype=torch.int32, device=d)
        self.info_terminal = torch.zeros((n_upd, T, E), dtype=torch.uint8, device=d)
        self.cur_return = torch.zeros((T, E), device=d)
        self.cur_length = torch.zeros((T, E), dtype=torch.int32, device=d)
        self.cur_terminal = torch.zeros((T, E), dtype=torch.uint8, device=d)
        self.last_reward = torch.zeros((E, A), device=d)
        self.last_done = torch.zeros((E, A), dtype=torch.uint8, device=d)

    def obs_slot(self, t: int) -> Dict[str, torch.Tensor]:
        return {"agents_view": self.agents_view[t], "global_state": self.global_state[t],
                "action_mask": self.action_mask[t], "step_count": self.step_count[t]}


class FFLearner:
    def __init__(self, env, config, centralised_critic: bool, device: Optional[torch.device] = None):
        self.config = config
        self.centralised = centralised_critic
        self.device = device if device is not None else torch.device("cuda", torch.cuda.current_device())
        self.rank, self.world = _dist_info()
        s, arch = config.system, config.arch
        self.E, self.U, self.T = int(arch.num_envs), int(s.update_batch_size), int(s.rollout_length)
        self.K, self.M = int(s.ppo_epochs), int(s.num_minibatches)
        if (self.T * self.E) % self.M:
            raise ValueError("rollout_length * num_envs must be divisible by num_minibatches (ff_mappo.py:277-279)")
        self.n_upd = int(s.get("num_updates_per_eval", 1))
        self.reps: List[_Replica] = []
        if env.num_envs != self.E:
            raise ValueError(f"env.num_envs={env.num_envs} != arch.num_envs={self.E}")
        if centralised_critic and not getattr(env, "add_global_state", False):
            raise ValueError("Global state must be provided to the centralised critic.")
        action_head = make_action_head(config.network.get("action_head", None), env.action_dim)
        self.continuous = type(action_head).__name__ == "ContinuousActionHead"
        self.min_scale = float(getattr(action_head, "min_scale", 1e-3))
        self._env_reads_action = not self.continuous or getattr(env, "continuous_actions", False)
        for u in range(self.U):
            rep_env = env.clone(env_offset=getattr(env, "env_offset", 0) + (self.rank * self.U + u) * self.E)
            self.reps.append(_Replica(rep_env, self.T, self.n_upd, centralised_critic, self.device, self.continuous))
        env0 = self.reps[0].env
        self.A, self.nA = env0.num_agents, env0.action_dim
        config.system.num_agents = self.A
        self.Oa = env0.obs_dim
        if centralised_critic:
            self.Oc = env0.state_dim
            self.critic_share = self.A if env0.global_state_shared else 1
        else:
            self.Oc = self.Oa
            self.critic_share = 1

        net = config.network
        from . import generic_networks as gn

        self.generic = (not gn.is_default_mlp(net.actor_network.pre_torso) or not gn.is_default_mlp(net.critic_network.pre_torso)
                        or (self.continuous and not action_head.independent_std))
        if self.generic:
            if (self.E * env0.num_agents) % 32 or ((self.T * self.E // self.M) * env0.num_agents) % 32:
                raise ValueError("the general network path needs num_envs * num_agents and the agent rows of a minibatch to be "
                                 "multiples of 32")
            obs_shape = getattr(env0, "obs_shape", None)
            state_shape = getattr(env0, "state_shape", None) if centralised_critic else obs_shape
            self.actor_network = gn.GenericActor(gn.torso_from_config(net.actor_network.pre_torso), action_head, self.Oa, obs_shape)
            self.critic_network = gn.GenericCritic(gn.torso_from_config(net.critic_network.pre_torso), centralised_critic, self.Oc,
                                                   state_shape)
        else:
            a_torso = MLPTorso(**{k: v for k, v in net.actor_network.pre_torso.items() if k != "_target_"})
            c_torso = MLPTorso(**{k: v for k, v in net.critic_network.pre_torso.items() if k != "_target_"})
            self.actor_network = FeedForwardActor(a_torso, action_head, self.Oa)
            self.critic_network = FeedForwardValueNet(c_torso, centralised_critic, self.Oc)
        self.Pa, self.Pc = self.actor_network.num_params, self.critic_network.num_params
        self.P = self.Pa + self.Pc

        d = self.device
        self.p = torch.zeros(self.P, device=d)
        self.m = torch.zeros(self.P, device=d)
        self.v = torch.zeros(self.P, device=d)
        self.count = torch.zeros(2, dtype=torch.int32, device=d)
        self.g = torch.zeros(self.P + 4, device=d)
        self.seg_off = [0, self.Pa, self.P]
        self.seg_lr = [float(s.actor_lr), float(s.critic_lr)]

        self.Rb = self.T * self.E // self.M
        ntiles = (self.Rb * self.A + 31) // 32
        self.rccl_cus = int(s.get("rccl_cus", None) if s.get("rccl_cus", None) is not None
                            else os.environ.get("MAVA_RCCL_CUS", "8" if self.world > 1 else "0"))
        self.n_slab = max(1, min(NUM_CU - max(0, min(self.rccl_cus, NUM_CU - 1)), ntiles))
        self.slab_a = torch.zeros((self.n_slab, self.Pa + 2), device=d)
        self.slab_c = torch.zeros((self.n_slab, self.Pc + 2), device=d)
        self.stats = torch.zeros((ops.lib().mava_adv_stats_blocks(), 2), dtype=torch.float64, device=d)
        self.train_metrics = torch.zeros((self.n_upd, self.K, self.M, 4), device=d)
        self.perm_count = 0
        self.t_global = 0
        self.ent_step = 0
        self.step_dev = torch.zeros(1, dtype=torch.int32, device=d)
        mode = os.environ.get("MAVA_GRAPH_ROLLOUT", "1")
        self.graph_rollout = (mode == "force" or (mode != "0" and self.world == 1)) and not self.generic
        self._graphs: Dict[int, Any] = {}
        self._graph_seen: set = set()
        self.seed = int(s.seed)
        self.timers: Optional[Dict[str, list]] = None
        self.matmul_mode, self.ctx = matmul_ctx(s, critic_aggregation=os.environ.get("MAVA_CRITIC_AGGREGATION", "1") != "0")
        self.ctx.set(self.ctx.TRAIN_VARIANT, int(os.environ.get("MAVA_TRAIN_VARIANT", "0")))
        for net_ in (self.actor_network, self.critic_network):
            net_.ctx = self.ctx
        self.fused_rollout = (self.matmul_mode == "f16x2" and not self.continuous and not self.generic
                              and os.environ.get("MAVA_FUSED_ROLLOUT", "1") != "0"
                              and bool(getattr(env0, "supports_fused_rollout", False))
                              and int(getattr(env0, "synth_state_dim", 0)) == 0
                              and (not centralised_critic or (env0.gs_tiles == 1 and env0.global_state_shared)))
        self._learn_calls = 0
        self.fused_tail = (self.world == 1 and not self.generic and os.environ.get("MAVA_FUSED_TAIL", "1") != "0")
        self._finish_ws = ops.ppo_finish_workspace(self.Pa, self.Pc, d) if self.fused_tail else None
        self._finish_ws_mr = (ops.ppo_finish_workspace(self.Pa, self.Pc, d)
                              if (not self.fused_tail and not self.generic and os.environ.get("MAVA_FUSED_TAIL", "1") != "0") else None)
        if self.fused_tail and self.U > 1:
            self.slab_a = torch.zeros((self.U * self.n_slab, self.Pa + 2), device=d)
            self.slab_c = torch.zeros((self.U * self.n_slab, self.Pc + 2), device=d)

    def _timed(self, name: str, fn, *args, **kwargs):
        if self.timers is None:
            return fn(*args, **kwargs)
        a, b = torch.cuda.Event(enable_timing=True), torch.cuda.Event(enable_timing=True)
        a.record()
        out = fn(*args, **kwargs)
        b.record()
        self.timers.setdefault(name, []).append((a, b))
        return out

    def init_params(self, actor_seed: int, critic_seed: int) -> None:
        self.p[: self.Pa].copy_(self.actor_network.init_flat(actor_seed))
        self.p[self.Pa :].copy_(self.critic_network.init_flat(critic_seed))
        self.m.zero_()
        self.v.zero_()
        self.count.zero_()

    def reset_envs(self) -> None:
        for rep in self.reps:
            rep.env.step_into(rep.state, 0, rep.obs_slot(0), is_reset=True)
        self.t_global = 0
        self.ent_step = 0
        self.step_dev.zero_()
        self.perm_count = 0

    def _params_tree(self) -> Params:
        lead = (1, self.U)
        return Params(self.actor_network.tree(self.p[: self.Pa], lead), self.critic_network.tree(self.p[self.Pa :], lead))

    def _opt_tree(self) -> OptStates:
        lead = (1, self.U)
        out = []
        for i, (net, sl) in enumerate(((self.actor_network, slice(0, self.Pa)), (self.critic_network, slice(self.Pa, self.P)))):
            out.append(AdamState(self.count[i].expand(1, self.U), net.tree(self.m[sl], lead), net.tree(self.v[sl], lead)))
        return OptStates(*out)

    def _timestep(self, slot: int) -> TimeStep:
        def stack(f):
            return torch.stack([f(r) for r in self.reps], 0).unsqueeze(0)

        av = stack(lambda r: r.agents_view[slot])
        mask = stack(lambda r: r.action_mask[slot]).bool()
        sc = stack(lambda r: r.step_count[slot])
        if self.centralised:
            gs = stack(lambda r: r.global_state[slot].expand(-1, self.A, -1) if r.env.gs_tiles == 1 else r.global_state[slot])
            obs: Any = ObservationGlobalState(av, mask, gs, sc)
        else:
            obs = Observation(av, mask, sc)
        done = stack(lambda r: r.last_done[:, 0]).bool()
        step_type = torch.where(done, 2, 1).to(torch.int8)
        reward = stack(lambda r: r.last_reward)
        n = max(self.n_upd - 1, 0)
        extras = {"episode_metrics": {
            "episode_return": stack(lambda r: r.info_return[n, -1]),
            "episode_length": stack(lambda r: r.info_length[n, -1]),
            "is_terminal_step": stack(lambda r: r.info_terminal[n, -1]).bool()}}
        return TimeStep(step_type, reward, 1.0 - stack(lambda r: r.last_done).float(), obs, extras)

    def learner_state(self) -> LearnerState:
        key = torch.tensor([[[self.seed, self.t_global]] * self.U], dtype=torch.int64)
        env_state = {
            "step_count": torch.stack([r.state.step_count for r in self.reps], 0).unsqueeze(0),
            "running_count_episode_return": torch.stack([r.state.run_return for r in self.reps], 0).unsqueeze(0),
            "running_count_episode_length": torch.stack([r.state.run_length for r in self.reps], 0).unsqueeze(0),
            "episode_return": torch.stack([r.state.ep_return for r in self.reps], 0).unsqueeze(0),
            "episode_length": torch.stack([r.state.ep_length for r in self.reps], 0).unsqueeze(0),
        }
        return LearnerState(self._params_tree(), self._opt_tree(), key, env_state, self._timestep(0))

    def adopt(self, state: LearnerState) -> None:
        pa = self.actor_network.first_leaf(state.params.actor_params)
        if pa.data_ptr() != self.p.data_ptr():
            self.actor_network.flat_from_tree(state.params.actor_params, self.p[: self.Pa])
            self.critic_network.flat_from_tree(state.params.critic_params, self.p[self.Pa :])
            for i, (net, sl, st) in enumerate(((self.actor_network, slice(0, self.Pa), state.opt_states.actor_opt_state),
                                               (self.critic_network, slice(self.Pa, self.P), state.opt_states.critic_opt_state))):
                net.flat_from_tree(st.mu, self.m[sl])
                net.flat_from_tree(st.nu, self.v[sl])
                self.count[i] = int(st.count.reshape(-1)[0])
            self.ctx.set(self.ctx.W1_SPLIT_FRESH, 0)

    def _rollout(self, n: int) -> None:
        if self.fused_rollout and self._rollout_fused(n):
            self.t_global += self.T
            return
        if not self.graph_rollout or self.timers is not None:
            self._rollout_body()
            self._bootstrap_and_gae()
        else:
            key = self.seed
            graph = self._graphs.get(key)
            if graph is None and key in self._graph_seen:
                graph = torch.cuda.CUDAGraph()
                with torch.cuda.graph(graph, capture_error_mode="thread_local"):
                    self._rollout_body()
                    self._bootstrap_and_gae()
                self._graphs[key] = graph
            if graph is None:
                self._graph_seen.add(key)
                self._rollout_body()
                self._bootstrap_and_gae()
            else:
                graph.replay()
        for rep in self.reps:
            rep.info_return[n].copy_(rep.cur_return)
            rep.info_length[n].copy_(rep.cur_length)
            rep.info_terminal[n].copy_(rep.cur_terminal)
        self.t_global += self.T

    def _rollout_fused(self, n: int) -> bool:
        s = self.config.system
        pa, pc = self.p[: self.Pa], self.p[self.Pa :]
        EA = self.E * self.A
        main = torch.cuda.current_stream() if self.device.type == "cuda" else None
        side = self.U > 1 and self.timers is None and main is not None and os.environ.get("MAVA_ROLLOUT_STREAMS", "1") != "0"
        if side and not hasattr(self, "_roll_streams"):
            from .streams import overlapping_stream

            self._roll_streams = [overlapping_stream(self.device) for _ in range(self.U - 1)]
            if any(st is None for st in self._roll_streams):
                self._roll_streams = []
        side = side and len(self._roll_streams) == self.U - 1
        if side:
            for st in self._roll_streams:
                st.wait_stream(main)
        for u, rep in enumerate(self.reps):
            env = rep.env
            with (torch.cuda.stream(self._roll_streams[u - 1]) if (side and u > 0) else contextlib.nullcontext()):
              ok = self._timed(
                "rollout_fused", ops.rollout_ff, pa, pc, n_actions=self.nA, critic_shared=self.centralised, E=self.E,
                A=self.A, O=env.raw_obs_dim, T=self.T, time_limit=env.time_limit, policy_seed=self.seed,
                env_seed=env.seed, t0=self.t_global, row_offset=(self.rank * self.U + u) * EA, env_offset=env.env_offset,
                reward_mode=1 if env.reward_mode == "match" else 0, env_state=rep.state, agents_view=rep.agents_view,
                global_state=rep.global_state, action_mask=rep.action_mask, obs_step_count=rep.step_count,
                action=rep.action, value=rep.value, reward=rep.reward, log_prob=rep.log_prob, done=rep.done,
                last_val=rep.last_val, info_return=rep.info_return[n], info_length=rep.info_length[n],
                info_terminal=rep.info_terminal[n], adv=rep.adv, tgt=rep.tgt, gamma=float(s.gamma),
                gae_lambda=float(s.gae_lambda))
              if not ok:
                assert u == 0
                self.fused_rollout = False
                return False
              rep.last_reward.copy_(rep.reward[self.T - 1])
              rep.last_done.copy_(rep.done[self.T - 1])
        if side:
            for st in self._roll_streams:
                main.wait_stream(st)
        self.step_dev.add_(self.T)
        return True

    def _rollout_body(self) -> None:
        pa, pc = self.p[: self.Pa], self.p[self.Pa :]
        EA = self.E * self.A
        for t in range(self.T):
            step = t
            for u, rep in enumerate(self.reps):
                av = rep.agents_view[t].view(EA, self.Oa)
                if self.centralised:
                    cx = rep.global_state[t].view(-1, self.Oc)
                else:
                    cx = av
                shared = self.critic_share == self.A and self.A > 1
                common = dict(critic_share=1 if shared else self.critic_share, critic_rows=self.E if shared else EA,
                              value_broadcast=self.A if shared else 1, seed=self.seed, step=step,
                              step_base=self.step_dev, row_offset=(self.rank * self.U + u) * EA, ctx=self.ctx)
                if self.generic:
                    self._timed("policy_step", self._generic_act, u, rep, t, step)
                elif self.continuous:
                    self._timed("policy_step", ops.policy_step_continuous, pa, pc, av, cx, action_dim=self.nA, min_scale=self.min_scale,
                                out=(rep.action[t].view(EA, self.nA), rep.log_prob[t].view(EA), rep.value[t].view(EA)),
                                **common)
                else:
                    self._timed("policy_step", ops.policy_step, pa, pc, av, rep.action_mask[t].view(EA, self.nA), cx,
                                n_actions=self.nA,
                                out=(rep.action[t].view(EA), rep.log_prob[t].view(EA), rep.value[t].view(EA)), **common)
                last = t == self.T - 1
                self._timed("env_step", rep.env.step_into, rep.state, step + 1, rep.obs_slot(t + 1), rep.reward[t], rep.done[t],
                            rep.cur_return[t], rep.cur_length[t], rep.cur_terminal[t], t_base=self.step_dev,
                            action=rep.action[t] if self._env_reads_action else None)
                if last:
                    rep.last_reward.copy_(rep.reward[t])
                    rep.last_done.copy_(rep.done[t])
        self.step_dev.add_(self.T)

    def _bootstrap_and_gae(self) -> None:
        s = self.config.system
        pc = self.p[self.Pa :]
        EA = self.E * self.A
        for rep in self.reps:
            cx = rep.global_state[self.T].view(-1, self.Oc) if self.centralised else rep.agents_view[self.T].view(EA, self.Oa)
            if self.generic:
                v = self.critic_network.net.forward(pc, self._gws_roll[1], cx.view(1, self.E, -1, self.Oc), self.critic_share, None, EA,
                                                    self.E, self.A)[0]
                rep.last_val.view(EA).copy_(v)
            else:
                ops.mlp_forward(pc, self.Oc, 1, cx, rows=EA, x_share=self.critic_share, out=rep.last_val.view(EA, 1), ctx=self.ctx)
            self._timed("gae", ops.gae, rep.reward.view(self.T, EA), rep.value.view(self.T, EA), rep.done.view(self.T, EA),
                        rep.last_val.view(EA), float(s.gamma), float(s.gae_lambda),
                        out=(rep.adv.view(self.T, EA), rep.tgt.view(self.T, EA)), ctx=self.ctx)

    def _minibatch(self, n: int, k: int, mb: int, perm: Optional[torch.Tensor]) -> None:
        s = self.config.system
        T, E, A = self.T, self.E, self.A
        TEA = T * E * A
        pa, pc = self.p[: self.Pa], self.p[self.Pa :]
        idx = None if perm is None else perm[mb * self.Rb : (mb + 1) * self.Rb]
        base = mb * self.Rb
        if self.generic:
            return self._minibatch_generic(n, k, mb, idx if idx is not None else torch.arange(base, base + self.Rb, dtype=torch.int32,
                                                                                             device=self.device))
        ns = self.n_slab
        per_rep = self.fused_tail and self.U > 1
        for u, rep in enumerate(self.reps):
            slab_a = self.slab_a[u * ns : (u + 1) * ns] if per_rep else self.slab_a
            av = rep.agents_view[:T].view(TEA, self.Oa)
            if getattr(self, "_stats_batched", False) and perm is self._perm_bufs[k]:
                stats = self._stats_all[u, k * self.M + mb]
            else:
                stats = ops.adv_stats(rep.adv.view(TEA), idx, base, self.Rb, A, out=self.stats)
            if self.continuous:
                self._timed("actor_grad", ops.ppo_actor_grad_continuous, pa, av, rep.action.view(TEA, self.nA),
                            rep.log_prob.view(TEA), rep.adv.view(TEA), stats, idx, base, self.Rb, A, self.nA,
                            float(s.clip_eps), float(s.ent_coef), self.seed, self.ent_step,
                            (self.rank * self.U + u) * TEA, slab_a, min_scale=self.min_scale)
            else:
                self._timed("actor_grad", ops.ppo_actor_grad, pa, av, rep.action_mask[:T].view(TEA, self.nA),
                            rep.action.view(TEA), rep.log_prob.view(TEA), rep.adv.view(TEA), stats, idx, base,
                            self.Rb, A, self.nA, float(s.clip_eps), float(s.ent_coef), slab_a, ctx=self.ctx)
            if not self.fused_tail:
                ops.slab_reduce2(self.slab_a, self.Pa, self.g[: self.Pa], 2, self.g[self.P : self.P + 2], accumulate=u > 0)
        w_actor = parallel.allreduce_sum_async(self.g[: self.Pa])
        for u, rep in enumerate(self.reps):
            av = rep.agents_view[:T].view(TEA, self.Oa)
            cx = rep.global_state[:T].view(-1, self.Oc) if self.centralised else av
            self._timed("critic_grad", ops.ppo_critic_grad, pc, cx, self.critic_share, rep.value.view(TEA), rep.tgt.view(TEA),
                        idx, base, self.Rb, A, float(s.clip_eps), float(s.vf_coef),
                        self.slab_c[u * ns : (u + 1) * ns] if per_rep else self.slab_c, ctx=self.ctx)
            if not self.fused_tail:
                ops.slab_reduce2(self.slab_c, self.Pc, self.g[self.Pa : self.P], 1, self.g[self.P + 2 : self.P + 3], accumulate=u > 0)
        if self.fused_tail:
            self._timed("finish", ops.ppo_finish, self.ctx, self.slab_a, self.slab_c, self.Pa, self.Pc, self.g, self.p, self.m, self.v,
                        self.count, self.seg_lr[0], self.seg_lr[1], grad_scale=1.0 / self.U, max_norm=float(s.max_grad_norm),
                        decay=bool(s.decay_learning_rates), steps_per_update=self.K * self.M,
                        num_updates=int(s.get("num_updates", 1) or 1), vf_coef=float(s.vf_coef), ent_coef=float(s.ent_coef),
                        metrics_out=self.train_metrics[n, k, mb], critic_din=self.Oc, workspace=self._finish_ws)
            self.ent_step += 1
            return
        w_rest = parallel.allreduce_sum_async(self.g[self.Pa :])
        for wk in (w_actor, w_rest):
            if wk is not None:
                wk.wait()
        if self._finish_ws_mr is not None:
            self._timed("clip_adam", ops.ppo_finish, self.ctx, None, None, self.Pa, self.Pc, self.g, self.p, self.m, self.v, self.count,
                        self.seg_lr[0], self.seg_lr[1], grad_scale=1.0 / (self.U * self.world), max_norm=float(s.max_grad_norm),
                        decay=bool(s.decay_learning_rates), steps_per_update=self.K * self.M,
                        num_updates=int(s.get("num_updates", 1) or 1), vf_coef=float(s.vf_coef), ent_coef=float(s.ent_coef),
                        metrics_out=self.train_metrics[n, k, mb], critic_din=self.Oc, workspace=self._finish_ws_mr)
            self.ent_step += 1
            return
        self._timed("clip_adam", ops.clip_adam, self.p, self.g, self.m, self.v, self.count, self.seg_off, self.seg_lr,
                      grad_scale=1.0 / (self.U * self.world), max_norm=float(s.max_grad_norm),
                      decay=bool(s.decay_learning_rates), steps_per_update=self.K * self.M,
                      num_updates=int(s.get("num_updates", 1) or 1), loss_sums=self.g[self.P :], vf_coef=float(s.vf_coef),
                      ent_coef=float(s.ent_coef), metrics_out=self.train_metrics[n, k, mb])
        self.ent_step += 1

    def _generic_setup(self) -> None:
        d = self.device
        EA, Rm = self.E * self.A, self.Rb * self.A
        a, c = self.actor_network.net, self.critic_network.net
        self._gws_roll = (a.workspace(EA, d, False), c.workspace(EA, d, False))
        self._gws = (a.workspace(Rm, d, True), c.workspace(Rm, d, True))
        self._g_scale = float(2 ** math.ceil(math.log2(Rm)))
        self._g_dscale = torch.zeros((self._gws[0].loss_partials.shape[0], max(self.nA, 1)), device=d)

    def _generic_act(self, u: int, rep, t: int, step: int) -> None:
        if not hasattr(self, "_gws_roll"):
            self._generic_setup()
        L, st = ops.lib(), ops.stream_ptr()
        pa, pc = self.p[: self.Pa], self.p[self.Pa :]
        E, A, EA = self.E, self.A, self.E * self.A
        an = self.actor_network
        outs = an.net.forward(pa, self._gws_roll[0], rep.agents_view[t : t + 1], 1, None, EA, E, A)
        seed, row_off = self.seed & (2**64 - 1), ((self.rank * self.U + u) * EA) & 0xFFFFFFFF
        gstep = (self.t_global + step) & 0xFFFFFFFF
        if self.continuous:
            ind = an.independent_std
            ops.check(L.mava_seq_sample_continuous_f32(EA, self.nA, self.min_scale, ops.ptr(outs[0]), ops.ptr(an.log_std(pa)) if ind else None,
                                                       None if ind else ops.ptr(outs[1]), seed, gstep, row_off, 0, ops.ptr(rep.action[t]),
                                                       ops.ptr(rep.log_prob[t]), st), "mava_seq_sample_continuous_f32")
        else:
            ops.check(L.mava_seq_sample_f32(EA, self.nA, ops.ptr(outs[0]), ops.ptr(rep.action_mask[t]), seed, gstep, row_off, 0,
                                            ops.ptr(rep.action[t]), ops.ptr(rep.log_prob[t]), st), "mava_seq_sample_f32")
        cx = rep.global_state[t : t + 1] if self.centralised else rep.agents_view[t : t + 1]
        v = self.critic_network.net.forward(pc, self._gws_roll[1], cx, self.critic_share, None, EA, E, A)[0]
        rep.value[t].view(EA).copy_(v)

    def _minibatch_generic(self, n: int, k: int, mb: int, idx: torch.Tensor) -> None:
        if not hasattr(self, "_gws"):
            self._generic_setup()
        s = self.config.system
        T, E, A = self.T, self.E, self.A
        TE, Rm = T * E, self.Rb * A
        L, st = ops.lib(), ops.stream_ptr()
        pa, pc = self.p[: self.Pa], self.p[self.Pa :]
        idx = idx.contiguous()
        wa, wc = self._gws
        an, cn, gs = self.actor_network, self.critic_network, self._g_scale
        nblk = wa.loss_partials.shape[0]
        for u, rep in enumerate(self.reps):
            acc = u > 0
            outs = an.net.forward(pa, wa, rep.agents_view[:T].view(1, TE, A, self.Oa), 1, idx, Rm, TE, A)
            ops.adv_stats(rep.adv.view(-1), idx, 0, self.Rb, A, out=self.stats)
            if self.continuous:
                ind = an.independent_std
                ops.check(L.mava_seq_actor_loss_continuous_f32(
                    1, Rm, TE, A, self.nA, self.min_scale, ops.ptr(idx), ops.ptr(outs[0]), ops.ptr(an.log_std(pa)) if ind else None,
                    None if ind else ops.ptr(outs[1]), ops.ptr(rep.action), ops.ptr(rep.log_prob), ops.ptr(rep.adv), ops.ptr(self.stats),
                    self.stats.shape[0], float(s.clip_eps), float(s.ent_coef), self.seed & (2**64 - 1), self.ent_step & 0xFFFFFFFF,
                    ((self.rank * self.U + u) * TE * A) & 0xFFFFFFFF, gs, ops.ptr(wa.dout[0]), None if ind else ops.ptr(wa.dout[1]),
                    ops.ptr(wa.loss_partials), ops.ptr(self._g_dscale), nblk, st), "mava_seq_actor_loss_continuous_f32")
                if ind:
                    ops.slab_reduce(self._g_dscale, self.nA, an.log_std(self.g[: self.Pa]), accumulate=acc)
            else:
                ops.check(L.mava_seq_actor_loss_f32(1, Rm, TE, A, self.nA, ops.ptr(idx), ops.ptr(outs[0]), ops.ptr(rep.action_mask[:T]),
                                                    ops.ptr(rep.action), ops.ptr(rep.log_prob), ops.ptr(rep.adv), ops.ptr(self.stats),
                                                    self.stats.shape[0], float(s.clip_eps), float(s.ent_coef), gs, ops.ptr(wa.dout[0]),
                                                    ops.ptr(wa.loss_partials), nblk, st), "mava_seq_actor_loss_f32")
            ops.slab_reduce(wa.loss_partials, 2, self.g[self.P : self.P + 2], accumulate=acc)
            an.net.backward(pa, wa, wa.dout[: len(an.net.heads)], self.g[: self.Pa], accumulate=acc, grad_scale=gs)
        w_actor = parallel.allreduce_sum_async(self.g[: self.Pa])
        for u, rep in enumerate(self.reps):
            acc = u > 0
            cx = (rep.global_state[:T].view(1, TE, -1, self.Oc) if self.centralised else rep.agents_view[:T].view(1, TE, A, self.Oa))
            v = cn.net.forward(pc, wc, cx, self.critic_share, idx, Rm, TE, A)[0]
            ops.check(L.mava_seq_critic_loss_f32(1, Rm, TE, A, 1, ops.ptr(idx), ops.ptr(v), ops.ptr(rep.value), ops.ptr(rep.tgt),
                                                 float(s.clip_eps), float(s.vf_coef), gs, ops.ptr(wc.dout[0]), ops.ptr(wc.loss_partials),
                                                 nblk, st), "mava_seq_critic_loss_f32")
            ops.slab_reduce(wc.loss_partials, 1, self.g[self.P + 2 : self.P + 3], accumulate=acc)
            cn.net.backward(pc, wc, [wc.dout[0]], self.g[self.Pa : self.P], accumulate=acc, grad_scale=gs)
        w_rest = parallel.allreduce_sum_async(self.g[self.Pa :])
        for wk in (w_actor, w_rest):
            if wk is not None:
                wk.wait()
        ops.clip_adam(self.p, self.g, self.m, self.v, self.count, self.seg_off, self.seg_lr,
                      grad_scale=1.0 / (self.U * self.world), max_norm=float(s.max_grad_norm),
                      decay=bool(s.decay_learning_rates), steps_per_update=self.K * self.M,
                      num_updates=int(s.get("num_updates", 1) or 1), loss_sums=self.g[self.P :], vf_coef=float(s.vf_coef),
                      ent_coef=float(s.ent_coef), metrics_out=self.train_metrics[n, k, mb])
        self.ent_step += 1

    def _permutations(self) -> List[torch.Tensor]:
        if not hasattr(self, "_perm_bufs"):
            self._perm_all = torch.empty((self.K, self.T * self.E), dtype=torch.int32, device=self.device)
            self._perm_bufs = [self._perm_all[k] for k in range(self.K)]
            self._stats_all = torch.empty((self.U, self.K * self.M, self.stats.shape[0], 2), dtype=torch.float64, device=self.device)
        for buf in self._perm_bufs:
            ops.permutation(self.T * self.E, self.seed, self.perm_count, out=buf)
            self.perm_count += 1
        return self._perm_bufs

    def update(self, n: int, permutations: Optional[List[torch.Tensor]] = None) -> None:
        own = permutations is None
        if own:
            permutations = self._permutations()
        self.ctx.set(self.ctx.W1_SPLIT_FRESH, 0)
        self._rollout(n)
        self._stats_batched = own and not self.generic and self.T * self.E == self.M * self.Rb
        if self._stats_batched:
            for u, rep in enumerate(self.reps):
                ops.adv_stats_batched(rep.adv.view(-1), self._perm_all.view(-1), self.Rb, self.A, self.K * self.M,
                                      out=self._stats_all[u])
        for k in range(self.K):
            perm = permutations[k]
            for mb in range(self.M):
                self._minibatch(n, k, mb, perm)
        for rep in self.reps:
            rep.agents_view[0].copy_(rep.agents_view[self.T])
            rep.global_state[0].copy_(rep.global_state[self.T])
            rep.action_mask[0].copy_(rep.action_mask[self.T])
            rep.step_count[0].copy_(rep.step_count[self.T])

    def learn(self, learner_state: LearnerState) -> ExperimentOutput:
        self.adopt(learner_state)
        if self.matmul_mode == "f16x2":
            obs = [t for r in self.reps for t in (r.agents_view[0], r.global_state[0] if self.centralised else None)]
            check_f16_range(self.p, obs, self.train_metrics if self._learn_calls else None, type(self).__name__)
        self._learn_calls += 1
        for n in range(self.n_upd):
            self.update(n)
        U = self.U
        episode_metrics = {
            "episode_return": torch.stack([r.info_return for r in self.reps], 1).unsqueeze(0),
            "episode_length": torch.stack([r.info_length for r in self.reps], 1).unsqueeze(0),
            "is_terminal_step": torch.stack([r.info_terminal for r in self.reps], 1).unsqueeze(0).bool(),
        }
        tm = self.train_metrics.unsqueeze(1).expand(self.n_upd, U, self.K, self.M, 4).unsqueeze(0)
        train_metrics = {"total_loss": tm[..., 0], "value_loss": tm[..., 1], "actor_loss": tm[..., 2], "entropy": tm[..., 3]}
        return ExperimentOutput(self.learner_state(), episode_metrics, train_metrics)


def learner_setup(env, keys, config, centralised_critic: bool, device=None):
    key, actor_key, critic_key = (int(k) for k in keys)
    learner = FFLearner(env, config, centralised_critic, device)
    learner.seed = key
    learner.init_params(actor_key, critic_key)
    parallel.broadcast_(learner.p, src=0)
    learner.reset_envs()
    return bind_learn(learner), learner.actor_network, learner.learner_state()


def get_final_step_metrics(metrics: Dict[str, torch.Tensor]) -> Tuple[Dict[str, torch.Tensor], bool]:
    metrics = dict(metrics)
    is_final = metrics.pop("is_terminal_step").bool()
    has_final = bool(is_final.any())
    if not has_final:
        return {k: torch.zeros_like(v) for k, v in metrics.items()}, False
    return {k: v[is_final] for k, v in metrics.items()}, True
```

### mava_amd/ops.py

```python
from __future__ import annotations

import ctypes as C
from typing import Optional, Sequence, Tuple

import torch

from . import _lib
from ._lib import Ctx, check, ctx_ptr, lib, ptr, stream_ptr


def _req(t: torch.Tensor, dtype: torch.dtype, name: str, shape: Optional[Tuple[int, ...]] = None) -> None:
    if not isinstance(t, torch.Tensor):
        raise TypeError(f"{name}: expected a torch.Tensor")
    if not t.is_cuda:
        raise _lib.MavaHipError(f"{name}: tensor must live on the GPU (got {t.device}); there is no CPU path")
    if t.dtype != dtype:
        raise TypeError(f"{name}: expected dtype {dtype}, got {t.dtype}")
    if not t.is_contiguous():
        raise ValueError(f"{name}: tensor must be contiguous")
    if shape is not None and tuple(t.shape) != tuple(shape):
        raise ValueError(f"{name}: expected shape {tuple(shape)}, got {tuple(t.shape)}")


def _as_u8(t: torch.Tensor) -> torch.Tensor:
    return t.view(torch.uint8) if t.dtype == torch.bool else t


def permutation(n: int, seed: int, counter: int, out: Optional[torch.Tensor] = None) -> torch.Tensor:
    if out is None:
        out = torch.empty(n, dtype=torch.int32, device=torch.device("cuda", torch.cuda.current_device()))
    _req(out, torch.int32, "out", (n,))
    check(lib().mava_permutation_i32(n, seed & (2**64 - 1), counter & (2**64 - 1), ptr(out), stream_ptr()), "mava_permutation_i32")
    return out


def gae(reward, value, done, last_val, gamma: float, gae_lambda: float, last_done=None, out=None, ctx: Optional[Ctx] = None):
    T = reward.shape[0]
    N = reward[0].numel() if T > 0 else last_val.numel()
    done = _as_u8(done)
    _req(reward, torch.float32, "reward")
    _req(value, torch.float32, "value", reward.shape)
    _req(done, torch.uint8, "done", reward.shape)
    _req(last_val, torch.float32, "last_val")
    if last_val.numel() != N:
        raise ValueError(f"last_val: expected {N} elements, got {last_val.numel()}")
    if last_done is not None:
        last_done = _as_u8(last_done)
        _req(last_done, torch.uint8, "last_done")
        if last_done.numel() != N:
            raise ValueError(f"last_done: expected {N} elements, got {last_done.numel()}")
    if out is None:
        adv = torch.empty_like(reward)
        tgt = torch.empty_like(reward)
    else:
        adv, tgt = out
        _req(adv, torch.float32, "adv", reward.shape)
        _req(tgt, torch.float32, "tgt", reward.shape)
    check(
        lib().mava_gae_f32(ctx_ptr(ctx), ptr(reward), ptr(value), ptr(done), ptr(last_val), ptr(last_done), T, N,
                           gamma, gae_lambda, ptr(adv), ptr(tgt), stream_ptr()),
        "mava_gae_f32",
    )
    return adv, tgt


def clip_adam(p, g, m, v, count, seg_off: Sequence[int], seg_lr: Sequence[float], *, grad_scale: float,
              max_norm: float, decay: bool = False, steps_per_update: int = 1, num_updates: int = 1,
              b1: float = 0.9, b2: float = 0.999, eps: float = 1e-5, loss_sums=None, vf_coef: float = 0.0,
              ent_coef: float = 0.0, metrics_out=None) -> None:
    n_seg = len(seg_lr)
    if len(seg_off) != n_seg + 1:
        raise ValueError("seg_off must have len(seg_lr)+1 entries")
    total = int(seg_off[-1])
    for name, t in (("p", p), ("g", g), ("m", m), ("v", v)):
        _req(t, torch.float32, name)
        if t.numel() < total:
            raise ValueError(f"{name}: needs at least {total} elements, has {t.numel()}")
    _req(count, torch.int32, "count")
    if count.numel() < n_seg:
        raise ValueError("count: one int32 per segment required")
    if loss_sums is not None:
        _req(loss_sums, torch.float32, "loss_sums")
        if loss_sums.numel() < 3:
            raise ValueError("loss_sums: 3 floats required")
    if metrics_out is not None:
        _req(metrics_out, torch.float32, "metrics_out")
        if metrics_out.numel() < 4:
            raise ValueError("metrics_out: 4 floats required")
    off = (C.c_int * (n_seg + 1))(*[int(x) for x in seg_off])
    lr = (C.c_float * n_seg)(*[float(x) for x in seg_lr])
    check(
        lib().mava_clip_adam(ptr(p), ptr(g), ptr(m), ptr(v), ptr(count), off, lr, n_seg, grad_scale, max_norm,
                             int(decay), steps_per_update, num_updates, b1, b2, eps, ptr(loss_sums), vf_coef,
                             ent_coef, ptr(metrics_out), stream_ptr()),
        "mava_clip_adam",
    )


def slab_reduce(slab: torch.Tensor, n: int, out: torch.Tensor, accumulate: bool = False) -> None:
    _req(slab, torch.float32, "slab")
    _req(out, torch.float32, "out")
    if slab.dim() != 2 or slab.shape[1] < n or out.numel() < n:
        raise ValueError("slab must be (n_slab, stride>=n) and out must hold n floats")
    check(
        lib().mava_slab_reduce_f32(ptr(slab), slab.shape[0], slab.shape[1], n, int(accumulate), ptr(out),
                                   stream_ptr()),
        "mava_slab_reduce_f32",
    )


def slab_reduce_cols(slab: torch.Tensor, col0: int, n: int, out: torch.Tensor, accumulate: bool = False) -> None:
    _req(slab, torch.float32, "slab")
    _req(out, torch.float32, "out")
    if slab.dim() != 2 or col0 < 0 or slab.shape[1] < col0 + n or out.numel() < n:
        raise ValueError("slab must be (n_slab, stride >= col0 + n) and out must hold n floats")
    check(lib().mava_slab_reduce_f32(slab.data_ptr() + 4 * col0, slab.shape[0], slab.shape[1], n, int(accumulate), ptr(out), stream_ptr()),
          "mava_slab_reduce_f32")


def ppo_finish_workspace(Pa: int, Pc: int, device) -> torch.Tensor:
    n = int(lib().mava_ppo_finish_workspace_bytes(Pa, Pc))
    return torch.zeros((n + 7) // 8, dtype=torch.float64, device=device)


def ppo_finish(ctx: Optional[Ctx], slab_a, slab_c, Pa: int, Pc: int, g, p, m, v, count, lr_a: float, lr_c: float, *,
               grad_scale: float, max_norm: float, decay: bool, steps_per_update: int, num_updates: int, vf_coef: float,
               ent_coef: float, metrics_out, critic_din: int, workspace: torch.Tensor, b1: float = 0.9, b2: float = 0.999,
               eps: float = 1e-5) -> None:
    reduced = slab_a is None
    if not reduced:
        _req(slab_a, torch.float32, "slab_a")
        _req(slab_c, torch.float32, "slab_c")
        if slab_a.dim() != 2 or slab_c.dim() != 2 or slab_a.shape[0] != slab_c.shape[0] or slab_a.shape[1] < Pa + 2 or slab_c.shape[1] < Pc + 1:
            raise ValueError("ppo_finish: slabs must be (n_slab, >= P + 2) with equal slab counts")
    for name, t, n in (("g", g, Pa + Pc + 3), ("p", p, Pa + Pc), ("m", m, Pa + Pc), ("v", v, Pa + Pc)):
        _req(t, torch.float32, name)
        if t.numel() < n:
            raise ValueError(f"{name}: needs at least {n} elements")
    _req(count, torch.int32, "count")
    _req(workspace, torch.float64, "workspace")
    if metrics_out is not None:
        _req(metrics_out, torch.float32, "metrics_out")
    check(lib().mava_ppo_finish_f32(ctx_ptr(ctx), ptr(slab_a), 0 if reduced else slab_a.shape[1], ptr(slab_c),
                                    0 if reduced else slab_c.shape[1], 0 if reduced else slab_a.shape[0], Pa, Pc,
                                    ptr(g), ptr(p), ptr(m), ptr(v), ptr(count), lr_a, lr_c, grad_scale, max_norm, int(decay),
                                    steps_per_update, num_updates, b1, b2, eps, vf_coef, ent_coef, ptr(metrics_out), critic_din,
                                    ptr(workspace), workspace.numel() * 8, stream_ptr()), "mava_ppo_finish_f32")


def mlp_param_count(din: int, n_out: int) -> int:
    return lib().mava_mlp_param_count(din, n_out)


def mlp_forward(params: torch.Tensor, din: int, n_out: int, x: torch.Tensor, rows: Optional[int] = None,
                x_share: int = 1, out: Optional[torch.Tensor] = None, ctx: Optional[Ctx] = None) -> torch.Tensor:
    _req(params, torch.float32, "params")
    if params.numel() != mlp_param_count(din, n_out):
        raise ValueError(f"params: expected {mlp_param_count(din, n_out)} floats, got {params.numel()}")
    _req(x, torch.float32, "x")
    if x.dim() != 2 or x.shape[1] != din:
        raise ValueError(f"x: expected (rows, {din}), got {tuple(x.shape)}")
    if rows is None:
        rows = x.shape[0] * x_share
    if (rows + x_share - 1) // x_share > x.shape[0]:
        raise ValueError("x has too few rows for rows/x_share")
    if out is None:
        out = torch.empty((rows, n_out), dtype=torch.float32, device=x.device)
    else:
        _req(out, torch.float32, "out")
        if out.numel() != rows * n_out:
            raise ValueError(f"out: expected {rows * n_out} elements, got {out.numel()}")
    check(lib().mava_mlp_forward_f32(ctx_ptr(ctx), ptr(params), din, n_out, ptr(x), x_share, rows, ptr(out), stream_ptr()),
          "mava_mlp_forward_f32")
    return out


def policy_step(actor_params, critic_params, agents_view, action_mask, critic_input, *, n_actions: int,
                critic_share: int = 1, critic_rows: Optional[int] = None, value_broadcast: int = 1, seed: int,
                step: int, row_offset: int = 0, greedy: bool = False, forced_action=None, out=None,
                want_logits: bool = False, step_base: Optional[torch.Tensor] = None, ctx: Optional[Ctx] = None):
    if step_base is not None:
        _req(step_base, torch.int32, "step_base")
    _req(agents_view, torch.float32, "agents_view")
    rows, actor_din = agents_view.shape
    _req(critic_input, torch.float32, "critic_input")
    critic_din = critic_input.shape[1]
    if critic_rows is None:
        critic_rows = critic_input.shape[0] * critic_share
    if (critic_rows + critic_share - 1) // critic_share > critic_input.shape[0]:
        raise ValueError("critic_input has too few rows")
    _req(actor_params, torch.float32, "actor_params")
    _req(critic_params, torch.float32, "critic_params")
    if actor_params.numel() != mlp_param_count(actor_din, n_actions):
        raise ValueError("actor_params: wrong size")
    if critic_params.numel() != mlp_param_count(critic_din, 1):
        raise ValueError("critic_params: wrong size")
    if action_mask is not None:
        action_mask = _as_u8(action_mask)
        _req(action_mask, torch.uint8, "action_mask", (rows, n_actions))
    if forced_action is not None:
        _req(forced_action, torch.int32, "forced_action", (rows,))
    dev = agents_view.device
    if out is None:
        action = torch.empty((rows,), dtype=torch.int32, device=dev)
        log_prob = torch.empty((rows,), dtype=torch.float32, device=dev)
        value = torch.empty((critic_rows * value_broadcast,), dtype=torch.float32, device=dev)
    else:
        action, log_prob, value = out
        _req(action, torch.int32, "action")
        _req(log_prob, torch.float32, "log_prob")
        _req(value, torch.float32, "value")
        if action.numel() != rows or log_prob.numel() != rows or value.numel() != critic_rows * value_broadcast:
            raise ValueError("policy_step: output buffers have the wrong size")
    logits = torch.empty((rows, n_actions), dtype=torch.float32, device=dev) if want_logits else None
    check(
        lib().mava_policy_step_f32(ctx_ptr(ctx), ptr(actor_params), actor_din, n_actions, ptr(agents_view), ptr(action_mask),
                                   ptr(critic_params), critic_din, ptr(critic_input), critic_share, critic_rows,
                                   value_broadcast, rows, seed & 0xFFFFFFFFFFFFFFFF, step & 0xFFFFFFFF,
                                   ptr(step_base), row_offset & 0xFFFFFFFF, int(greedy), ptr(forced_action), ptr(action),
                                   ptr(log_prob), ptr(value), ptr(logits), stream_ptr()),
        "mava_policy_step_f32",
    )
    return action, log_prob, value, logits


def continuous_param_count(din: int, action_dim: int) -> int:
    return mlp_param_count(din, action_dim) + action_dim


def policy_step_continuous(actor_params, critic_params, agents_view, critic_input, *, action_dim: int,
                           critic_share: int = 1, critic_rows: Optional[int] = None, value_broadcast: int = 1,
                           seed: int, step: int, row_offset: int = 0, greedy: bool = False, forced_action=None,
                           out=None, want_mean: bool = False, step_base: Optional[torch.Tensor] = None,
                           ctx: Optional[Ctx] = None, min_scale: float = 1e-3):
    if step_base is not None:
        _req(step_base, torch.int32, "step_base")
    _req(agents_view, torch.float32, "agents_view")
    rows, actor_din = agents_view.shape
    _req(critic_input, torch.float32, "critic_input")
    critic_din = critic_input.shape[1]
    if critic_rows is None:
        critic_rows = critic_input.shape[0] * critic_share
    if (critic_rows + critic_share - 1) // critic_share > critic_input.shape[0]:
        raise ValueError("critic_input has too few rows")
    _req(actor_params, torch.float32, "actor_params")
    _req(critic_params, torch.float32, "critic_params")
    if actor_params.numel() != continuous_param_count(actor_din, action_dim):
        raise ValueError("actor_params: wrong size")
    if critic_params.numel() != mlp_param_count(critic_din, 1):
        raise ValueError("critic_params: wrong size")
    if forced_action is not None:
        _req(forced_action, torch.float32, "forced_action", (rows, action_dim))
    dev = agents_view.device
    if out is None:
        action = torch.empty((rows, action_dim), dtype=torch.float32, device=dev)
        log_prob = torch.empty(rows, dtype=torch.float32, device=dev)
        value = torch.empty(critic_rows * value_broadcast, dtype=torch.float32, device=dev)
    else:
        action, log_prob, value = out
        _req(action, torch.float32, "action")
        _req(log_prob, torch.float32, "log_prob")
        _req(value, torch.float32, "value")
        if action.numel() != rows * action_dim or log_prob.numel() != rows or value.numel() != critic_rows * value_broadcast:
            raise ValueError("out: wrong sizes")
    mean = torch.empty((rows, action_dim), dtype=torch.float32, device=dev) if want_mean else None
    check(
        lib().mava_policy_step_continuous_f32(ctx_ptr(ctx), ptr(actor_params), actor_din, action_dim, float(min_scale), ptr(agents_view),
                                              ptr(critic_params), critic_din, ptr(critic_input), critic_share,
                                              critic_rows, value_broadcast, rows, seed & 0xFFFFFFFFFFFFFFFF,
                                              step & 0xFFFFFFFF, ptr(step_base), row_offset & 0xFFFFFFFF, int(greedy),
                                              ptr(forced_action), ptr(action), ptr(log_prob), ptr(value), ptr(mean),
                                              stream_ptr()),
        "mava_policy_step_continuous_f32",
    )
    return action, log_prob, value, mean


def ppo_actor_grad_continuous(params, agents_view, action, old_log_prob, advantages, stats, idx, idx_base: int,
                              Rb: int, A: int, action_dim: int, clip_eps: float, ent_coef: float, seed: int,
                              ent_step: int, row_offset: int, slab: torch.Tensor, min_scale: float = 1e-3) -> None:
    _req(agents_view, torch.float32, "agents_view")
    rows, din = agents_view.shape
    if rows % A:
        raise ValueError("agents_view rows must be a multiple of A")
    TE = rows // A
    _req(params, torch.float32, "params")
    P = continuous_param_count(din, action_dim)
    if params.numel() != P:
        raise ValueError(f"params: expected {P} floats")
    _req(action, torch.float32, "action")
    _req(old_log_prob, torch.float32, "old_log_prob")
    _req(advantages, torch.float32, "advantages")
    for n, t, k in (("action", action, action_dim), ("old_log_prob", old_log_prob, 1), ("advantages", advantages, 1)):
        if t.numel() != rows * k:
            raise ValueError(f"{n}: expected {rows * k} elements, got {t.numel()}")
    _req(stats, torch.float64, "stats", (lib().mava_adv_stats_blocks(), 2))
    _check_idx(idx, idx_base, Rb, TE)
    if rows >= 2 ** 31:
        raise ValueError("trajectory too large: TE*A must be < 2^31 (32-bit row arithmetic in the kernel)")
    _req(slab, torch.float32, "slab")
    if slab.dim() != 2 or slab.shape[1] < P + 2:
        raise ValueError("slab must be (n_slab, >= P+2)")
    check(
        lib().mava_ppo_actor_grad_continuous_f32(ptr(params), din, action_dim, float(min_scale), ptr(agents_view), ptr(action),
                                                 ptr(old_log_prob), ptr(advantages), ptr(stats), ptr(idx), idx_base,
                                                 Rb, A, clip_eps, ent_coef, seed & 0xFFFFFFFFFFFFFFFF,
                                                 ent_step & 0xFFFFFFFF, row_offset & 0xFFFFFFFF, ptr(slab),
                                                 slab.shape[1], slab.shape[0], stream_ptr()),
        "mava_ppo_actor_grad_continuous_f32",
    )


def adv_stats_batched(advantages: torch.Tensor, idx: torch.Tensor, Rb: int, A: int, n_batch: int,
                      out: Optional[torch.Tensor] = None) -> torch.Tensor:
    _req(advantages, torch.float32, "advantages")
    _req(idx, torch.int32, "idx")
    if idx.numel() < n_batch * Rb:
        raise ValueError("idx shorter than n_batch * Rb")
    nb = lib().mava_adv_stats_blocks()
    if out is None:
        out = torch.empty((n_batch, nb, 2), dtype=torch.float64, device=advantages.device)
    _req(out, torch.float64, "out", (n_batch, nb, 2))
    check(lib().mava_adv_stats_batched_f64(ptr(advantages), ptr(idx), Rb, Rb, A, n_batch, ptr(out), stream_ptr()),
          "mava_adv_stats_batched_f64")
    return out


def adv_stats(advantages: torch.Tensor, idx: Optional[torch.Tensor], idx_base: int, Rb: int, A: int,
              out: Optional[torch.Tensor] = None) -> torch.Tensor:
    _req(advantages, torch.float32, "advantages")
    if idx is not None:
        _req(idx, torch.int32, "idx")
        if idx.numel() < Rb:
            raise ValueError("idx shorter than Rb")
    elif (idx_base + Rb) * A > advantages.numel():
        raise ValueError("minibatch exceeds the trajectory")
    nb = lib().mava_adv_stats_blocks()
    if out is None:
        out = torch.empty((nb, 2), dtype=torch.float64, device=advantages.device)
    else:
        _req(out, torch.float64, "out", (nb, 2))
    check(lib().mava_adv_stats_f64(ptr(advantages), ptr(idx), idx_base, Rb, A, ptr(out), stream_ptr()),
          "mava_adv_stats_f64")
    return out


def _check_idx(idx, idx_base, Rb, TE):
    if idx is not None:
        _req(idx, torch.int32, "idx")
        if idx.numel() < Rb:
            raise ValueError("idx shorter than Rb")
    elif idx_base < 0 or idx_base + Rb > TE:
        raise ValueError("minibatch exceeds the trajectory")


def ppo_actor_grad(params, agents_view, action_mask, action, old_log_prob, advantages, stats, idx, idx_base: int,
                   Rb: int, A: int, n_actions: int, clip_eps: float, ent_coef: float, slab: torch.Tensor,
                   ctx: Optional[Ctx] = None) -> None:
    _req(agents_view, torch.float32, "agents_view")
    rows, din = agents_view.shape
    if rows % A:
        raise ValueError("agents_view rows must be a multiple of A")
    TE = rows // A
    _req(params, torch.float32, "params")
    P = mlp_param_count(din, n_actions)
    if params.numel() != P:
        raise ValueError(f"params: expected {P} floats")
    if action_mask is not None:
        action_mask = _as_u8(action_mask)
        _req(action_mask, torch.uint8, "action_mask", (rows, n_actions))
    _req(action, torch.int32, "action")
    _req(old_log_prob, torch.float32, "old_log_prob")
    _req(advantages, torch.float32, "advantages")
    for n, t in (("action", action), ("old_log_prob", old_log_prob), ("advantages", advantages)):
        if t.numel() != rows:
            raise ValueError(f"{n}: expected {rows} elements, got {t.numel()}")
    _req(stats, torch.float64, "stats", (lib().mava_adv_stats_blocks(), 2))
    _check_idx(idx, idx_base, Rb, TE)
    if rows >= 2 ** 31:
        raise ValueError("trajectory too large: TE*A must be < 2^31 (32-bit row arithmetic in the kernel)")
    _req(slab, torch.float32, "slab")
    if slab.dim() != 2 or slab.shape[1] < P + 2:
        raise ValueError("slab must be (n_slab, >= P+2)")
    check(
        lib().mava_ppo_actor_grad_f32(ctx_ptr(ctx), ptr(params), din, n_actions, ptr(agents_view), ptr(action_mask), ptr(action),
                                      ptr(old_log_prob), ptr(advantages), ptr(stats), ptr(idx), idx_base, Rb, A,
                                      clip_eps, ent_coef, ptr(slab), slab.shape[1], slab.shape[0], stream_ptr()),
        "mava_ppo_actor_grad_f32",
    )


def ppo_critic_grad(params, critic_input, x_share: int, old_value, targets, idx, idx_base: int, Rb: int, A: int,
                    clip_eps: float, vf_coef: float, slab: torch.Tensor, ctx: Optional[Ctx] = None) -> None:
    _req(critic_input, torch.float32, "critic_input")
    din = critic_input.shape[1]
    _req(params, torch.float32, "params")
    P = mlp_param_count(din, 1)
    if params.numel() != P:
        raise ValueError(f"params: expected {P} floats")
    _req(old_value, torch.float32, "old_value")
    _req(targets, torch.float32, "targets")
    rows = old_value.numel()
    if targets.numel() != rows or rows % A:
        raise ValueError("old_value/targets must hold TE*A elements")
    if (rows + x_share - 1) // x_share > critic_input.shape[0]:
        raise ValueError("critic_input has too few rows")
    _check_idx(idx, idx_base, Rb, rows // A)
    if rows >= 2 ** 31:
        raise ValueError("trajectory too large: TE*A must be < 2^31 (32-bit row arithmetic in the kernel)")
    _req(slab, torch.float32, "slab")
    if slab.dim() != 2 or slab.shape[1] < P + 2:
        raise ValueError("slab must be (n_slab, >= P+2)")
    check(
        lib().mava_ppo_critic_grad_f32(ctx_ptr(ctx), ptr(params), din, ptr(critic_input), x_share, ptr(old_value), ptr(targets),
                                       ptr(idx), idx_base, Rb, A, clip_eps, vf_coef, ptr(slab), slab.shape[1],
                                       slab.shape[0], stream_ptr()),
        "mava_ppo_critic_grad_f32",
    )


def slab_reduce2(slab: torch.Tensor, n_main: int, out_main: torch.Tensor, n_tail: int, out_tail: torch.Tensor,
                 accumulate: bool = False) -> None:
    _req(slab, torch.float32, "slab")
    _req(out_main, torch.float32, "out_main")
    _req(out_tail, torch.float32, "out_tail")
    if slab.dim() != 2 or slab.shape[1] < n_main + n_tail or out_main.numel() < n_main or out_tail.numel() < n_tail:
        raise ValueError("slab_reduce2: inconsistent sizes")
    check(
        lib().mava_slab_reduce2_f32(ptr(slab), slab.shape[0], slab.shape[1], n_main, ptr(out_main), n_tail, ptr(out_tail),
                                    int(accumulate), stream_ptr()),
        "mava_slab_reduce2_f32",
    )


def rollout_ff(actor_params, critic_params, *, n_actions: int, critic_shared: bool, E: int, A: int, O: int, T: int,
               time_limit: int, policy_seed: int, env_seed: int, t0: int, row_offset: int, env_offset: int,
               reward_mode: int, env_state, agents_view, global_state, action_mask, obs_step_count, action, value,
               reward, log_prob, done, last_val, info_return, info_length, info_terminal, adv=None, tgt=None,
               gamma: float = 0.99, gae_lambda: float = 0.95) -> bool:
    W = A + O
    _req(actor_params, torch.float32, "actor_params")
    _req(critic_params, torch.float32, "critic_params")
    if actor_params.numel() != mlp_param_count(W, n_actions):
        raise ValueError("actor_params: wrong size")
    if critic_params.numel() != mlp_param_count(A * O if critic_shared else W, 1):
        raise ValueError("critic_params: wrong size")
    _req(agents_view, torch.float32, "agents_view", (T + 1, E, A, W))
    if critic_shared:
        _req(global_state, torch.float32, "global_state", (T + 1, E, 1, A * O))
    _req(action_mask, torch.uint8, "action_mask", (T + 1, E, A, n_actions))
    _req(obs_step_count, torch.int32, "obs_step_count", (T + 1, E, A))
    _req(action, torch.int32, "action", (T, E, A))
    for name, t, dt in (("value", value, torch.float32), ("reward", reward, torch.float32),
                        ("log_prob", log_prob, torch.float32), ("done", done, torch.uint8)):
        _req(t, dt, name, (T, E, A))
    _req(last_val, torch.float32, "last_val", (E, A))
    if adv is not None or tgt is not None:
        _req(adv, torch.float32, "adv", (T, E, A))
        _req(tgt, torch.float32, "tgt", (T, E, A))
    _req(info_return, torch.float32, "info_return", (T, E))
    _req(info_length, torch.int32, "info_length", (T, E))
    _req(info_terminal, torch.uint8, "info_terminal", (T, E))
    _req(env_state.step_count, torch.int32, "step_count", (E, A))
    for name, t, dt in (("run_return", env_state.run_return, torch.float32), ("run_length", env_state.run_length, torch.int32),
                        ("ep_return", env_state.ep_return, torch.float32), ("ep_length", env_state.ep_length, torch.int32)):
        _req(t, dt, name, (E,))
    rc = lib().mava_rollout_ff_f32(
        ptr(actor_params), n_actions, ptr(critic_params), int(critic_shared), E, A, O, T, time_limit,
        policy_seed & 0xFFFFFFFFFFFFFFFF, env_seed & 0xFFFFFFFFFFFFFFFF, t0 & 0xFFFFFFFF, row_offset & 0xFFFFFFFF,
        env_offset & 0xFFFFFFFF, reward_mode, ptr(env_state.step_count), ptr(env_state.run_return),
        ptr(env_state.run_length), ptr(env_state.ep_return), ptr(env_state.ep_length), ptr(agents_view),
        ptr(global_state) if critic_shared else None, ptr(action_mask), ptr(obs_step_count), ptr(action), ptr(value),
        ptr(reward), ptr(log_prob), ptr(done), ptr(last_val), ptr(info_return), ptr(info_length), ptr(info_terminal),
        ptr(adv), ptr(tgt), gamma, gae_lambda, stream_ptr())
    if rc == 1:
        return False
    check(rc, "mava_rollout_ff_f32")
    return True
```

Before: 78.57 million env-steps/s.

## Batch permutations, fuse rollout tail copies, vectorise adv stats, strength-reduce rollout indexing

Generates all epoch permutations in one batched launch. Moves the last_reward/last_done copies and the step counter increment into a rollout tail kernel. Replaces the four slot-carry copies with a single carry kernel. It also vectorises the advantage-statistics loads and replaces integer divisions and kernarg reads in the rollout kernel with multiply-shift and constexpr layouts. The aim is fewer small launches and less per-step integer overhead, at the cost of extra code paths and an assumption that A is a power of two in the shift-based indexing.

```diff
diff --git a/include/mava_hip.h b/include/mava_hip.h
--- a/include/mava_hip.h
+++ b/include/mava_hip.h
@@ -35,6 +35,8 @@
                  float lambda, float* adv, float* tgt, mava_stream_t s);
 
 int mava_permutation_i32(long n, uint64_t seed, uint64_t counter, int32_t* out, mava_stream_t s);
+int mava_permutation_batched_i32(long n, uint64_t seed, uint64_t counter, int n_perm, int32_t* out, long out_stride,
+                                 mava_stream_t s);
 
 int mava_clip_adam(float* p, const float* g, float* m, float* v, int32_t* count,
                    const int* seg_off, const float* seg_lr, int n_seg, float grad_scale,
@@ -220,6 +222,17 @@
                         int32_t* obs_step_count, int32_t* action, float* value, float* reward, float* log_prob,
                         uint8_t* done, float* last_val, float* info_return, int32_t* info_length,
                         uint8_t* info_terminal, float* adv, float* tgt, float gamma, float gae_lambda, mava_stream_t s);
+int mava_rollout_ff_tail_f32(const float* actor_params, int n_actions, const float* critic_params, int critic_shared,
+                             int E, int A, int O, int T, int time_limit, uint64_t policy_seed, uint64_t env_seed,
+                             uint32_t t0, uint32_t row_offset, uint32_t env_offset, int reward_mode,
+                             int32_t* step_count, float* run_return, int32_t* run_length, float* ep_return,
+                             int32_t* ep_length, float* agents_view, float* global_state, uint8_t* action_mask,
+                             int32_t* obs_step_count, int32_t* action, float* value, float* reward, float* log_prob,
+                             uint8_t* done, float* last_val, float* info_return, int32_t* info_length,
+                             uint8_t* info_terminal, float* adv, float* tgt, float gamma, float gae_lambda,
+                             float* last_reward, uint8_t* last_done, int32_t* step_counter, mava_stream_t s);
+int mava_rollout_carry(int T, int E, int A, int obs_dim, long gs_dim, int n_actions, float* agents_view,
+                       float* global_state, uint8_t* action_mask, int32_t* step_count, mava_stream_t s);
 
 
 int mava_rec_dense_f32(const mava_ctx* ctx, const float* x, int x_rowmajor, const int32_t* idx, int Rm, int E, int A,
diff --git a/mava_amd/_lib.py b/mava_amd/_lib.py
--- a/mava_amd/_lib.py
+++ b/mava_amd/_lib.py
@@ -31,6 +31,7 @@
     "mava_ctx_get": [vp, i32, vp],
     "mava_gae_f32": [vp, vp, vp, vp, vp, vp, i32, i32, f32, f32, vp, vp, vp],
     "mava_permutation_i32": [lng, u64, u64, vp, vp],
+    "mava_permutation_batched_i32": [lng, u64, u64, i32, vp, lng, vp],
     "mava_clip_adam": [vp, vp, vp, vp, vp, C.POINTER(i32), C.POINTER(f32), i32, f32, f32, i32, i32, i32,
                        f32, f32, f32, vp, f32, f32, vp, vp],
     "mava_slab_reduce_f32": [vp, i32, lng, i32, i32, vp, vp],
@@ -80,6 +81,9 @@
     "mava_sac_actor_grad_f32": [i32] * 4 + [f32] + [vp] * 9 + [i32, i32, i32, f32, f32] + [vp] * 3 + [i32, vp],
     "mava_sac_alpha_loss_f32": [i32, i32, vp, vp, f32, vp, vp, vp],
     "mava_rollout_ff_f32": [vp, i32, vp, i32, i32, i32, i32, i32, i32, u64, u64, u32, u32, u32, i32] + [vp] * 18 + [vp, vp, f32, f32, vp],
+    "mava_rollout_ff_tail_f32": [vp, i32, vp, i32, i32, i32, i32, i32, i32, u64, u64, u32, u32, u32, i32] + [vp] * 18
+                                + [vp, vp, f32, f32, vp, vp, vp, vp],
+    "mava_rollout_carry": [i32, i32, i32, i32, lng, i32, vp, vp, vp, vp, vp],
     "mava_rec_dense_f32": [vp, vp, i32, vp, i32, i32, i32, i32, i32, i32, vp, i32, vp, vp, vp, i32, i32, i32, i32, i32, vp],
     "mava_rec_xty_f32": [vp, vp, i32, vp, i32, i32, i32, i32, i32, vp, i32, vp, i32, i32, i32, i32, i32, i32, f32, vp, lng, i32, vp],
     "mava_rec_gather_t32_f32": [vp, vp, i32, i32, i32, i32, i32, i32, i32, i32, vp, vp],
diff --git a/mava_amd/csrc/permutation.hip b/mava_amd/csrc/permutation.hip
--- a/mava_amd/csrc/permutation.hip
+++ b/mava_amd/csrc/permutation.hip
@@ -18,10 +18,7 @@
   return h;
 }
 
-__global__ __launch_bounds__(256) void permutation_kernel(uint32_t n, int lb, int rb, PermKeys keys,
-                                                          int32_t* __restrict__ out) {
-  const uint32_t i = blockIdx.x * 256u + threadIdx.x;
-  if (i >= n) return;
+__device__ __forceinline__ uint32_t perm_walk(uint32_t i, uint32_t n, int lb, int rb, const PermKeys& keys) {
   const uint32_t mask_r = (1u << rb) - 1u;
   uint32_t v = i;
   do {
@@ -33,7 +30,37 @@
     }
     v = (L << rb) | R;
   } while (v >= n);
-  out[i] = (int32_t)v;
+  return v;
+}
+
+__global__ __launch_bounds__(256) void permutation_kernel(uint32_t n, int lb, int rb, PermKeys keys,
+                                                          int32_t* __restrict__ out) {
+  const uint32_t i = blockIdx.x * 256u + threadIdx.x;
+  if (i >= n) return;
+  out[i] = (int32_t)perm_walk(i, n, lb, rb, keys);
+}
+
+constexpr int PERM_MAX_BATCH = 16;
+struct PermKeysBatch {
+  PermKeys e[PERM_MAX_BATCH];
+};
+__global__ __launch_bounds__(256) void permutation_batched_kernel(uint32_t n, int lb, int rb, PermKeysBatch keys,
+                                                                  int32_t* __restrict__ out, long out_stride) {
+  const uint32_t i = blockIdx.x * 256u + threadIdx.x;
+  if (i >= n) return;
+  out[(long)blockIdx.y * out_stride + i] = (int32_t)perm_walk(i, n, lb, rb, keys.e[blockIdx.y]);
+}
+
+void perm_keys(uint64_t seed, uint64_t counter, PermKeys& keys) {
+  uint64_t st = seed + 0x9E3779B97F4A7C15ull * (counter + 1);
+  for (int r = 0; r < PERM_ROUNDS; ++r) {
+    st += 0x9E3779B97F4A7C15ull;
+    uint64_t z = st;
+    z = (z ^ (z >> 30)) * 0xBF58476D1CE4E5B9ull;
+    z = (z ^ (z >> 27)) * 0x94D049BB133111EBull;
+    z ^= z >> 31;
+    keys.k[r] = (uint32_t)(z >> 32);
+  }
 }
 
 }
@@ -45,16 +72,25 @@
   while ((1L << b) < n) ++b;
   const int lb = b >> 1, rb = b - lb;
   PermKeys keys;
-  uint64_t st = seed + 0x9E3779B97F4A7C15ull * (counter + 1);
-  for (int r = 0; r < PERM_ROUNDS; ++r) {
-    st += 0x9E3779B97F4A7C15ull;
-    uint64_t z = st;
-    z = (z ^ (z >> 30)) * 0xBF58476D1CE4E5B9ull;
-    z = (z ^ (z >> 27)) * 0x94D049BB133111EBull;
-    z ^= z >> 31;
-    keys.k[r] = (uint32_t)(z >> 32);
-  }
+  perm_keys(seed, counter, keys);
   hipLaunchKernelGGL(permutation_kernel, dim3(mava_cdiv(n, 256)), dim3(256), 0, s, (uint32_t)n, lb, rb, keys, out);
   MAVA_LAUNCH_CHECK();
   return MAVA_OK;
 }
+
+extern "C" int mava_permutation_batched_i32(long n, uint64_t seed, uint64_t counter, int n_perm, int32_t* out,
+                                            long out_stride, hipStream_t s) {
+  MAVA_ARG_CHECK(n >= 1 && n < (1L << 31), 0, "mava_permutation_batched_i32: n=%ld (1 <= n < 2^31)", n);
+  MAVA_ARG_CHECK(n_perm >= 1 && n_perm <= PERM_MAX_BATCH && out_stride >= n, 0,
+                 "mava_permutation_batched_i32: n_perm=%d (1..%d) out_stride=%ld (>= n)", n_perm, PERM_MAX_BATCH, out_stride);
+  MAVA_ARG_CHECK(out, 1, "mava_permutation_batched_i32: null pointer argument");
+  int b = 2;
+  while ((1L << b) < n) ++b;
+  const int lb = b >> 1, rb = b - lb;
+  PermKeysBatch keys = {};
+  for (int k = 0; k < n_perm; ++k) perm_keys(seed, counter + (uint64_t)k, keys.e[k]);
+  hipLaunchKernelGGL(permutation_batched_kernel, dim3(mava_cdiv(n, 256), n_perm), dim3(256), 0, s, (uint32_t)n, lb, rb,
+                     keys, out, out_stride);
+  MAVA_LAUNCH_CHECK();
+  return MAVA_OK;
+}
diff --git a/mava_amd/csrc/ppo_train.hip b/mava_amd/csrc/ppo_train.hip
--- a/mava_amd/csrc/ppo_train.hip
+++ b/mava_amd/csrc/ppo_train.hip
@@ -57,6 +57,13 @@
   partials += (long)blockIdx.y * 2 * gridDim.x;
   double s1 = 0.0, s2 = 0.0;
   const long stride = (long)gridDim.x * 256;
+  const uintptr_t adv_addr = reinterpret_cast<uintptr_t>(adv);
+  const int vec = (A == 4 && (adv_addr & 15) == 0) ? 4 : (A == 8 && (adv_addr & 15) == 0) ? 8 : (A == 2 && (adv_addr & 7) == 0) ? 2 : 0;
+  auto add = [&](float f) {
+    const double v = (double)f;
+    s1 += v;
+    s2 += v * v;
+  };
   for (long b0 = (long)blockIdx.x * 256 + threadIdx.x; b0 < Rb; b0 += 4 * stride) {
     long p[4];
 #pragma unroll
@@ -65,14 +72,38 @@
       const long bc = b < Rb ? b : b0;
       p[u] = idx ? (long)idx[bc] : idx_base + bc;
     }
-#pragma unroll
-    for (int u = 0; u < 4; ++u) {
-      if (b0 + u * stride < Rb) {
-        const float* row = adv + p[u] * A;
-        for (int a = 0; a < A; ++a) {
-          const double v = (double)row[a];
-          s1 += v;
-          s2 += v * v;
+    if (vec == 4) {
+      float4 q[4];
+#pragma unroll
+      for (int u = 0; u < 4; ++u) q[u] = *reinterpret_cast<const float4*>(adv + p[u] * 4);
+#pragma unroll
+      for (int u = 0; u < 4; ++u) {
+        if (b0 + u * stride < Rb) { add(q[u].x); add(q[u].y); add(q[u].z); add(q[u].w); }
+      }
+    } else if (vec == 8) {
+#pragma unroll
+      for (int u = 0; u < 4; ++u) {
+        if (b0 + u * stride < Rb) {
+          const float4 q0 = *reinterpret_cast<const float4*>(adv + p[u] * 8);
+          const float4 q1 = *reinterpret_cast<const float4*>(adv + p[u] * 8 + 4);
+          add(q0.x); add(q0.y); add(q0.z); add(q0.w);
+          add(q1.x); add(q1.y); add(q1.z); add(q1.w);
+        }
+      }
+    } else if (vec == 2) {
+      float2 q[4];
+#pragma unroll
+      for (int u = 0; u < 4; ++u) q[u] = *reinterpret_cast<const float2*>(adv + p[u] * 2);
+#pragma unroll
+      for (int u = 0; u < 4; ++u) {
+        if (b0 + u * stride < Rb) { add(q[u].x); add(q[u].y); }
+      }
+    } else {
+#pragma unroll
+      for (int u = 0; u < 4; ++u) {
+        if (b0 + u * stride < Rb) {
+          const float* row = adv + p[u] * A;
+          for (int a = 0; a < A; ++a) add(row[a]);
         }
       }
     }
diff --git a/mava_amd/csrc/rollout_h2.hip b/mava_amd/csrc/rollout_h2.hip
--- a/mava_amd/csrc/rollout_h2.hip
+++ b/mava_amd/csrc/rollout_h2.hip
@@ -43,7 +43,17 @@
   float* info_return; int32_t* info_length; uint8_t* info_terminal;
   float* adv; float* tgt;
   float gamma, lam;
+  float* last_reward; uint8_t* last_done; int32_t* step_counter;
 };
+
+#define MAVA_AS4 __attribute__((address_space(4)))
+__device__ __forceinline__ const MAVA_AS4 RolloutArgs& args_here() {
+  const MAVA_AS4 RolloutArgs* p = (const MAVA_AS4 RolloutArgs*)__builtin_amdgcn_kernarg_segment_ptr();
+  asm volatile("" : "+s"(p));
+  return *p;
+}
+
+__device__ __forceinline__ uint32_t div_small(uint32_t x, uint32_t m) { return __umul24(x, m) >> 16; }
 
 struct RolloutLds {
   int xa, xa_row, xa_plane, xc, xc_row, xc_plane, h1, wl, ypa, ypc, act, mask, small, gum, xlf, end;
@@ -51,9 +61,9 @@
 constexpr int W1_REG_STEPS = 12;
 
 template <int NO, int S1A, int S1C, bool SHARED>
-RolloutLds make_rollout_lds() {
+constexpr RolloutLds make_rollout_lds() {
   constexpr int KTA = (S1A + 1) / 2, KTC = (S1C + 1) / 2;
-  RolloutLds L;
+  RolloutLds L{};
   L.xa = 0;
   L.xa_row = 2 * 32 * KTA + 16;
   L.xa_plane = 32 * L.xa_row;
@@ -76,8 +86,9 @@
 }
 
 template <int NO, int S1A, int S1C, bool SHARED, int ROLE>
-__device__ __forceinline__ void rollout_body(const RolloutArgs& a, const RolloutLds& L, u8* lds) {
+__device__ __forceinline__ void rollout_body(const RolloutArgs& a, u8* lds) {
   constexpr bool ACT_ROLE = ROLE == 0;
+  constexpr RolloutLds L = make_rollout_lds<NO, S1A, S1C, SHARED>();
   const int t512 = threadIdx.x;
   const int tid = t512 & 255, lane = tid & 63, w = tid >> 6, h = lane >> 5, r = lane & 31;
   const int A = a.A, O = a.O, no = a.no, W = A + O, E = a.E;
@@ -96,7 +107,7 @@
   unsigned* const XLF = reinterpret_cast<unsigned*>(lds + L.xlf);
   float* const YPA = reinterpret_cast<float*>(lds + L.ypa);
   float* const YPC = reinterpret_cast<float*>(lds + L.ypc);
-  const int xa_row = L.xa_row, xa_plane = L.xa_plane, xc_row = L.xc_row, xc_plane = L.xc_plane;
+  constexpr int xa_row = L.xa_row, xa_plane = L.xa_plane, xc_row = L.xc_row, xc_plane = L.xc_plane;
 
   for (int i = t512 * 16; i < L.end; i += 512 * 16) *reinterpret_cast<uint4*>(lds + i) = make_uint4(0, 0, 0, 0);
   __syncthreads();
@@ -196,9 +207,10 @@
   }
   __syncthreads();
 
-  const int bk_le = tid / A, bk_ag = tid - bk_le * A;
+  const int lgA = __builtin_ctz((unsigned)A);
+  const int bk_le = tid >> lgA, bk_ag = tid & (A - 1);
   const bool bk_on = !ACT_ROLE && tid < 64 && (e0 + bk_le) < E;
-  const long bk_k = (long)(e0 + bk_le) * A + bk_ag;
+  const long bk_k = (long)e0 * A + tid;
   int sc_reg = bk_on ? a.step_count[bk_k] : 0;
   float rr_reg = 0.0f, er_reg = 0.0f;
   int rl_reg = 0, el_reg = 0;
@@ -291,6 +303,7 @@
     }
     if (ACT_ROLE && noise) {
       const int grow = tid >> 2, c = tid & 3;
+      const auto& a = args_here();
       if (c < NO / 4) {
         const uint32_t gid = a.row_offset + (uint32_t)(e0 * A + grow);
         const Philox4 rnd = philox4x32_10(gid, noise_step, (uint32_t)c, POLICY_STREAM, a.pseed_lo, a.pseed_hi);
@@ -392,12 +405,19 @@
 
   const int rows_ok = min(64, (E - e0) * A), envs_ok = min(EB, E - e0);
   const int AO = A * O;
+  const uint32_t no_m = 65536u / (uint32_t)no + 1u, nch_m = 65536u / nch + 1u;
+  const int tid_w = tid, wo_q = (W >> 1) > 0 ? (W >> 1) : 1, gs_q = (AO >> 2) > 0 ? (AO >> 2) : 1;
+  const int wo_dr = 256 / wo_q, gs_dr = 256 / gs_q;
+  const uint32_t wo_m = 65536u / (uint32_t)wo_q + 1u, gs_m = 65536u / (uint32_t)gs_q + 1u;
   auto write_out = [&](long slot, bool part_gs) {
+    const auto& a = args_here();
+    int tid = tid_w;
+    asm volatile("" : "+v"(tid));
     if (!part_gs) {
       float* dst = a.agents_view + (slot * EA + (long)e0 * A) * W;
       if ((W & 1) == 0) {
-        const int W2 = W >> 1, d_r = 256 / W2, d_f = 256 - d_r * W2;
-        int row = tid / W2, f = tid - row * W2;
+        const int W2 = W >> 1, d_r = wo_dr, d_f = 256 - d_r * W2;
+        int row = (int)div_small((uint32_t)tid, wo_m), f = tid - row * W2;
         for (int j = tid; j < 64 * W2; j += 256) {
           if (row < rows_ok) {
             const u8* xa = lds + L.xa + (row >> 5) * 2 * xa_plane + (row & 31) * xa_row;
@@ -423,8 +443,8 @@
     if (part_gs && SHARED && a.global_state != nullptr) {
       float* dst = a.global_state + (slot * E + e0) * (long)AO;
       if ((AO & 3) == 0) {
-        const int Q = AO >> 2, d_r = 256 / Q, d_f = 256 - d_r * Q;
-        int le = tid / Q, k = tid - le * Q;
+        const int Q = AO >> 2, d_r = gs_dr, d_f = 256 - d_r * Q;
+        int le = (int)div_small((uint32_t)tid, gs_m), k = tid - le * Q;
         for (int j = tid; j < EB * Q; j += 256) {
           if (le < envs_ok) {
             const half4 v = *reinterpret_cast<const half4*>(lds + L.xc + le * xc_row + 8 * k);
@@ -446,15 +466,18 @@
     if (!part_gs) {
       uint8_t* dst = a.action_mask + (slot * EA + (long)e0 * A) * no;
       for (int j = tid; j < rows_ok * no; j += 256) {
-        const int row = j / no, o = j - row * no;
+        const int row = (int)div_small((uint32_t)j, no_m), o = j - row * no;
         dst[j] = MASK[row * 32 + o];
       }
     }
   };
 
-  for (int t = 0; t < a.T; ++t) {
-    const uint32_t step = a.t0 + (uint32_t)t;
+  const int T_steps = a.T;
+  const uint32_t t0 = a.t0;
+  for (int t = 0; t < T_steps; ++t) {
+    const uint32_t step = t0 + (uint32_t)t;
     forward(true, true, step);
+    const auto& a = args_here();
     if (ACT_ROLE) {
       constexpr int RPP = 256 / NO;
 #pragma unroll
@@ -481,7 +504,7 @@
           best = take ? bo : best;
         }
         const float lp = group_allreduce<NO>((o == best) ? logp : 0.0f, add_op);
-        const int e = e0 + row / A;
+        const int e = e0 + (row >> lgA);
         if (o == 0) {
           ACT[row] = best;
           if (e < E) {
@@ -492,8 +515,8 @@
         }
       }
     } else {
-      if (tid < 64 && (e0 + tid / A) < E) {
-        a.value[(long)t * EA + (long)e0 * A + tid] = value_of(SHARED ? tid / A : tid);
+      if (tid < 64 && (e0 + (tid >> lgA)) < E) {
+        a.value[(long)t * EA + (long)e0 * A + tid] = value_of(SHARED ? (tid >> lgA) : tid);
       }
       if (t > 0) write_out((long)t, false);
     }
@@ -502,12 +525,13 @@
     __syncthreads();
     RSTAMP(5);
     {
+      const auto& a = args_here();
       const uint32_t tn = step + 1;
       const long slot = (long)(t + 1);
       const uint32_t n_view = (uint32_t)(64 * nch);
       for (uint32_t i = ACT_ROLE ? (uint32_t)tid : n_view; i < n_view; i += 256) {
-        const uint32_t row = i / nch, c = i - row * nch;
-        const uint32_t le = row / A, ag = row - le * A, e = e0 + le;
+        const uint32_t row = div_small(i, nch_m), c = i - row * nch;
+        const uint32_t le = row >> lgA, ag = row - (le << lgA), e = e0 + le;
         if ((int)e >= E) continue;
         const uint32_t ent = (a.env_offset + e) * A + ag;
         const Philox4 rv = philox4x32_10(ent, tn, c, ENV_STREAM, a.eseed_lo, a.eseed_hi);
@@ -548,7 +572,7 @@
       }
       if (!ACT_ROLE && tid >= 64 && tid < 128) {
         const uint32_t row = (uint32_t)(tid - 64);
-        const uint32_t le = row / A, ag = row - le * A, e = e0 + le;
+        const uint32_t le = row >> lgA, ag = row - (le << lgA), e = e0 + le;
         if ((int)e < E) {
           const uint32_t ent = (a.env_offset + e) * A + ag;
           u8* xa = lds + L.xa + (row >> 5) * 2 * xa_plane + (row & 31) * xa_row;
@@ -606,55 +630,87 @@
   if (blockIdx.x == 0 && tid == 0)
     for (int i = 0; i < 8; ++i) g_rollout_stamps[(ACT_ROLE ? 0 : 8) + i] = rs_acc[i];
 #endif
-  write_out((long)a.T, ACT_ROLE);
+  write_out((long)T_steps, ACT_ROLE);
   forward(!ACT_ROLE, false, 0u);
+  {
+  const auto& a = args_here();
+  float lv = 0.0f;
   if (bk_on) {
-    const float lv = value_of(SHARED ? tid / A : tid);
+    lv = value_of(SHARED ? (tid >> lgA) : tid);
     a.last_val[bk_k] = lv;
-    if (a.adv != nullptr) {
-      float g = 0.0f, nv = lv;
-      const float gl = a.gamma * a.lam;
-      for (int tb = a.T; tb > 0; tb -= 8) {
-        float rw[8], vv[8];
-        uint8_t dd[8];
-#pragma unroll
-        for (int i = 0; i < 8; ++i) {
-          const int t = tb - 1 - i;
-          const long k = (long)(t >= 0 ? t : 0) * EA + bk_k;
-          rw[i] = a.reward[k]; vv[i] = a.value[k]; dd[i] = a.done[k];
-        }
-#pragma unroll
-        for (int i = 0; i < 8; ++i) {
-          const int t = tb - 1 - i;
-          if (t >= 0) {
-            const float nd = dd[i] ? 0.0f : 1.0f;
-            const float delta = rw[i] + a.gamma * nv * nd - vv[i];
-            g = delta + gl * nd * g;
-            const long k = (long)t * EA + bk_k;
-            a.adv[k] = g;
-            a.tgt[k] = g + vv[i];
-            nv = vv[i];
-          }
-        }
-      }
-    }
-  }
-  if (bk_on) {
     a.step_count[bk_k] = sc_reg;
     if (bk_ag == 0) {
       a.run_return[e0 + bk_le] = rr_reg; a.run_length[e0 + bk_le] = rl_reg;
       a.ep_return[e0 + bk_le] = er_reg; a.ep_length[e0 + bk_le] = el_reg;
     }
+    if (a.last_reward != nullptr) {
+      const long k = (long)(a.T - 1) * EA + bk_k;
+      a.last_reward[bk_k] = a.reward[k];
+      a.last_done[bk_k] = a.done[k];
+    }
+  }
+  if (a.adv != nullptr) {
+    const int T = a.T;
+    const int TC = min(T, (L.ypa / (64 * 9)) & ~7);
+    float* const RW = reinterpret_cast<float*>(lds);
+    float* const VV = RW + TC * 64;
+    u8* const DD = reinterpret_cast<u8*>(VV + TC * 64);
+    const long col0 = (long)e0 * A;
+    const float gl = a.gamma * a.lam;
+    float g = 0.0f, nv = lv;
+    for (int tb = T; tb > 0; tb -= TC) {
+      const int t_lo = max(tb - TC, 0), n = (tb - t_lo) * 64;
+      __syncthreads();
+      for (int i0 = t512; i0 < n; i0 += 512 * 8) {
+        float rw[8], vv[8];
+        uint8_t dd[8];
+#pragma unroll
+        for (int i = 0; i < 8; ++i) {
+          const int j = min(i0 + 512 * i, n - 1);
+          const long k = (long)(t_lo + (j >> 6)) * EA + col0 + min(j & 63, rows_ok - 1);
+          rw[i] = a.reward[k]; vv[i] = a.value[k]; dd[i] = a.done[k];
+        }
+#pragma unroll
+        for (int i = 0; i < 8; ++i) {
+          const int j = i0 + 512 * i;
+          if (j < n) { RW[j] = rw[i]; VV[j] = vv[i]; DD[j] = dd[i]; }
+        }
+      }
+      __syncthreads();
+      if (bk_on) {
+#pragma unroll 8
+        for (int t = tb - 1; t >= t_lo; --t) {
+          const int j = (t - t_lo) * 64 + tid;
+          const float rw = RW[j], vv = VV[j];
+          const float nd = DD[j] ? 0.0f : 1.0f;
+          const float delta = rw + a.gamma * nv * nd - vv;
+          g = delta + gl * nd * g;
+          RW[j] = g;
+          VV[j] = g + vv;
+          nv = vv;
+        }
+      }
+      __syncthreads();
+      for (int j = t512; j < n; j += 512) {
+        if ((j & 63) < rows_ok) {
+          const long k = (long)(t_lo + (j >> 6)) * EA + col0 + (j & 63);
+          a.adv[k] = RW[j];
+          a.tgt[k] = VV[j];
+        }
+      }
+    }
+  }
+  if (!ACT_ROLE && blockIdx.x == 0 && tid == 0 && a.step_counter != nullptr) *a.step_counter += a.T;
   }
 }
 
 template <int NO, int S1A, int S1C, bool SHARED>
-__global__ __launch_bounds__(512, 2) void rollout_h2_kernel(RolloutArgs a, RolloutLds L) {
+__global__ __launch_bounds__(512, 2) void rollout_h2_kernel(RolloutArgs a) {
   extern __shared__ __attribute__((aligned(16))) u8 lds[];
   if (threadIdx.x < 256) {
-    rollout_body<NO, S1A, S1C, SHARED, 0>(a, L, lds);
+    rollout_body<NO, S1A, S1C, SHARED, 0>(a, lds);
   } else {
-    rollout_body<NO, S1A, S1C, SHARED, 1>(a, L, lds);
+    rollout_body<NO, S1A, S1C, SHARED, 1>(a, lds);
   }
 }
 
@@ -663,7 +719,7 @@
 template <int NO, int S1A, int S1C, bool SHARED>
 int launch_rollout(const RolloutArgs& a, hipStream_t s) {
   g_rollout_last_instance = NO * 100000 + S1A * 1000 + S1C * 10 + (SHARED ? 1 : 0);
-  const RolloutLds L = make_rollout_lds<NO, S1A, S1C, SHARED>();
+  constexpr RolloutLds L = make_rollout_lds<NO, S1A, S1C, SHARED>();
   MAVA_ARG_CHECK(L.end <= 163840, 8, "mava_rollout_ff_f32: %d bytes of LDS exceed the 160 KiB of a CU", L.end);
   const int lds_bytes = L.end > 83968 ? L.end : 83968;
   static bool attr_set = false;
@@ -673,7 +729,7 @@
     attr_set = true;
   }
   const int EB = 64 / a.A;
-  hipLaunchKernelGGL((rollout_h2_kernel<NO, S1A, S1C, SHARED>), dim3(mava_cdiv(a.E, EB)), dim3(512), lds_bytes, s, a, L);
+  hipLaunchKernelGGL((rollout_h2_kernel<NO, S1A, S1C, SHARED>), dim3(mava_cdiv(a.E, EB)), dim3(512), lds_bytes, s, a);
   MAVA_LAUNCH_CHECK();
   return MAVA_OK;
 }
@@ -688,15 +744,15 @@
 
 extern "C" int mava_debug_rollout_last_instance(void) { return g_rollout_last_instance; }
 
-extern "C" int mava_rollout_ff_f32(const float* actor_params, int n_actions, const float* critic_params, int critic_shared,
-                                   int E, int A, int O, int T, int time_limit, uint64_t policy_seed, uint64_t env_seed,
-                                   uint32_t t0, uint32_t row_offset, uint32_t env_offset, int reward_mode,
-                                   int32_t* step_count, float* run_return, int32_t* run_length, float* ep_return,
-                                   int32_t* ep_length, float* agents_view, float* global_state, uint8_t* action_mask,
-                                   int32_t* obs_step_count, int32_t* action, float* value, float* reward, float* log_prob,
-                                   uint8_t* done, float* last_val, float* info_return, int32_t* info_length,
-                                   uint8_t* info_terminal, float* adv, float* tgt, float gamma, float gae_lambda,
-                                   hipStream_t s) {
+static int rollout_ff_impl(const float* actor_params, int n_actions, const float* critic_params, int critic_shared,
+                           int E, int A, int O, int T, int time_limit, uint64_t policy_seed, uint64_t env_seed,
+                           uint32_t t0, uint32_t row_offset, uint32_t env_offset, int reward_mode,
+                           int32_t* step_count, float* run_return, int32_t* run_length, float* ep_return,
+                           int32_t* ep_length, float* agents_view, float* global_state, uint8_t* action_mask,
+                           int32_t* obs_step_count, int32_t* action, float* value, float* reward, float* log_prob,
+                           uint8_t* done, float* last_val, float* info_return, int32_t* info_length,
+                           uint8_t* info_terminal, float* adv, float* tgt, float gamma, float gae_lambda,
+                           float* last_reward, uint8_t* last_done, int32_t* step_counter, hipStream_t s) {
   MAVA_ARG_CHECK(E >= 1 && A >= 1 && O >= 2 && T >= 1 && n_actions >= 1 && time_limit >= 1, 0,
                  "mava_rollout_ff_f32: bad shape E=%d A=%d O=%d T=%d nA=%d", E, A, O, T, n_actions);
   MAVA_ARG_CHECK(actor_params && critic_params && step_count && run_return && run_length && ep_return && ep_length &&
@@ -718,6 +774,7 @@
   a.info_terminal = info_terminal;
   MAVA_ARG_CHECK((adv == nullptr) == (tgt == nullptr), 1, "mava_rollout_ff_f32: adv and tgt go together");
   a.adv = adv; a.tgt = tgt; a.gamma = gamma; a.lam = gae_lambda;
+  a.last_reward = last_reward; a.last_done = last_done; a.step_counter = step_counter;
   if (critic_shared) {
     if (s1a == 5 && s1c == 17 && A >= 4) return launch_rollout<8, 5, 17, true>(a, s);
 #ifndef MAVA_FAST_BUILD
@@ -733,3 +790,82 @@
 #endif
   return 1;
 }
+
+extern "C" int mava_rollout_ff_f32(const float* actor_params, int n_actions, const float* critic_params, int critic_shared,
+                                   int E, int A, int O, int T, int time_limit, uint64_t policy_seed, uint64_t env_seed,
+                                   uint32_t t0, uint32_t row_offset, uint32_t env_offset, int reward_mode,
+                                   int32_t* step_count, float* run_return, int32_t* run_length, float* ep_return,
+                                   int32_t* ep_length, float* agents_view, float* global_state, uint8_t* action_mask,
+                                   int32_t* obs_step_count, int32_t* action, float* value, float* reward, float* log_prob,
+                                   uint8_t* done, float* last_val, float* info_return, int32_t* info_length,
+                                   uint8_t* info_terminal, float* adv, float* tgt, float gamma, float gae_lambda,
+                                   hipStream_t s) {
+  return rollout_ff_impl(actor_params, n_actions, critic_params, critic_shared, E, A, O, T, time_limit, policy_seed, env_seed,
+                         t0, row_offset, env_offset, reward_mode, step_count, run_return, run_length, ep_return, ep_length,
+                         agents_view, global_state, action_mask, obs_step_count, action, value, reward, log_prob, done,
+                         last_val, info_return, info_length, info_terminal, adv, tgt, gamma, gae_lambda, nullptr, nullptr,
+                         nullptr, s);
+}
+
+extern "C" int mava_rollout_ff_tail_f32(const float* actor_params, int n_actions, const float* critic_params,
+                                        int critic_shared, int E, int A, int O, int T, int time_limit,
+                                        uint64_t policy_seed, uint64_t env_seed, uint32_t t0, uint32_t row_offset,
+                                        uint32_t env_offset, int reward_mode, int32_t* step_count, float* run_return,
+                                        int32_t* run_length, float* ep_return, int32_t* ep_length, float* agents_view,
+                                        float* global_state, uint8_t* action_mask, int32_t* obs_step_count,
+                                        int32_t* action, float* value, float* reward, float* log_prob, uint8_t* done,
+                                        float* last_val, float* info_return, int32_t* info_length, uint8_t* info_terminal,
+                                        float* adv, float* tgt, float gamma, float gae_lambda, float* last_reward,
+                                        uint8_t* last_done, int32_t* step_counter, hipStream_t s) {
+  MAVA_ARG_CHECK(last_reward && last_done, 1, "mava_rollout_ff_tail_f32: null pointer argument");
+  return rollout_ff_impl(actor_params, n_actions, critic_params, critic_shared, E, A, O, T, time_limit, policy_seed, env_seed,
+                         t0, row_offset, env_offset, reward_mode, step_count, run_return, run_length, ep_return, ep_length,
+                         agents_view, global_state, action_mask, obs_step_count, action, value, reward, log_prob, done,
+                         last_val, info_return, info_length, info_terminal, adv, tgt, gamma, gae_lambda, last_reward,
+                         last_done, step_counter, s);
+}
+
+namespace {
+struct CarryArgs {
+  uint8_t* base[4];
+  long slot_bytes[4];
+  int T;
+};
+template <typename V>
+__device__ __forceinline__ void carry_copy(uint8_t* dst, const uint8_t* src, long bytes) {
+  const long nv = bytes / (long)sizeof(V), stride = (long)gridDim.x * blockDim.x;
+  const long i0 = (long)blockIdx.x * blockDim.x + threadIdx.x;
+  for (long i = i0; i < nv; i += stride) reinterpret_cast<V*>(dst)[i] = reinterpret_cast<const V*>(src)[i];
+  for (long i = nv * (long)sizeof(V) + i0; i < bytes; i += stride) dst[i] = src[i];
+}
+__global__ __launch_bounds__(256) void rollout_carry_kernel(CarryArgs c) {
+  uint8_t* const dst = c.base[blockIdx.y];
+  const long bytes = c.slot_bytes[blockIdx.y];
+  if (dst == nullptr || bytes <= 0) return;
+  const uint8_t* const src = dst + (long)c.T * bytes;
+  const uintptr_t al = reinterpret_cast<uintptr_t>(dst) | reinterpret_cast<uintptr_t>(src);
+  if ((al & 15) == 0) carry_copy<uint4>(dst, src, bytes);
+  else if ((al & 3) == 0) carry_copy<uint32_t>(dst, src, bytes);
+  else carry_copy<uint8_t>(dst, src, bytes);
+}
+}
+
+extern "C" int mava_rollout_carry(int T, int E, int A, int obs_dim, long gs_dim, int n_actions, float* agents_view,
+                                  float* global_state, uint8_t* action_mask, int32_t* step_count, hipStream_t s) {
+  MAVA_ARG_CHECK(T >= 1 && E >= 1 && A >= 1 && obs_dim >= 1 && gs_dim >= 0 && n_actions >= 1, 0,
+                 "mava_rollout_carry: bad shape T=%d E=%d A=%d obs_dim=%d gs_dim=%ld nA=%d", T, E, A, obs_dim, gs_dim, n_actions);
+  MAVA_ARG_CHECK(agents_view && action_mask && step_count && (gs_dim == 0 || global_state), 1,
+                 "mava_rollout_carry: null pointer argument");
+  CarryArgs c = {};
+  c.T = T;
+  c.base[0] = reinterpret_cast<uint8_t*>(agents_view); c.slot_bytes[0] = (long)E * A * obs_dim * 4;
+  c.base[1] = gs_dim ? reinterpret_cast<uint8_t*>(global_state) : nullptr; c.slot_bytes[1] = (long)E * gs_dim * 4;
+  c.base[2] = action_mask; c.slot_bytes[2] = (long)E * A * n_actions;
+  c.base[3] = reinterpret_cast<uint8_t*>(step_count); c.slot_bytes[3] = (long)E * A * 4;
+  long most = 0;
+  for (int i = 0; i < 4; ++i) most = c.slot_bytes[i] > most ? c.slot_bytes[i] : most;
+  const long blocks = mava_cdiv(most, 256L * 16 * 4);
+  hipLaunchKernelGGL(rollout_carry_kernel, dim3((unsigned)(blocks < 1 ? 1 : blocks > 2048 ? 2048 : blocks), 4), dim3(256), 0, s, c);
+  MAVA_LAUNCH_CHECK();
+  return MAVA_OK;
+}
diff --git a/mava_amd/learner.py b/mava_amd/learner.py
--- a/mava_amd/learner.py
+++ b/mava_amd/learner.py
@@ -295,17 +295,15 @@
                 action=rep.action, value=rep.value, reward=rep.reward, log_prob=rep.log_prob, done=rep.done,
                 last_val=rep.last_val, info_return=rep.info_return[n], info_length=rep.info_length[n],
                 info_terminal=rep.info_terminal[n], adv=rep.adv, tgt=rep.tgt, gamma=float(s.gamma),
-                gae_lambda=float(s.gae_lambda))
+                gae_lambda=float(s.gae_lambda), last_reward=rep.last_reward, last_done=rep.last_done,
+                step_counter=self.step_dev if u == 0 else None)
               if not ok:
                 assert u == 0
                 self.fused_rollout = False
                 return False
-              rep.last_reward.copy_(rep.reward[self.T - 1])
-              rep.last_done.copy_(rep.done[self.T - 1])
         if side:
             for st in self._roll_streams:
                 main.wait_stream(st)
-        self.step_dev.add_(self.T)
         return True
 
     def _rollout_body(self) -> None:
@@ -514,9 +512,9 @@
             self._perm_all = torch.empty((self.K, self.T * self.E), dtype=torch.int32, device=self.device)
             self._perm_bufs = [self._perm_all[k] for k in range(self.K)]
             self._stats_all = torch.empty((self.U, self.K * self.M, self.stats.shape[0], 2), dtype=torch.float64, device=self.device)
-        for buf in self._perm_bufs:
-            ops.permutation(self.T * self.E, self.seed, self.perm_count, out=buf)
-            self.perm_count += 1
+        for k0 in range(0, self.K, 16):
+            ops.permutation_batched(self.T * self.E, self.seed, self.perm_count + k0, self._perm_all[k0 : k0 + 16])
+        self.perm_count += self.K
         return self._perm_bufs
 
     def update(self, n: int, permutations: Optional[List[torch.Tensor]] = None) -> None:
@@ -535,10 +533,7 @@
             for mb in range(self.M):
                 self._minibatch(n, k, mb, perm)
         for rep in self.reps:
-            rep.agents_view[0].copy_(rep.agents_view[self.T])
-            rep.global_state[0].copy_(rep.global_state[self.T])
-            rep.action_mask[0].copy_(rep.action_mask[self.T])
-            rep.step_count[0].copy_(rep.step_count[self.T])
+            ops.rollout_carry(rep.agents_view, rep.global_state, rep.action_mask, rep.step_count)
 
     def learn(self, learner_state: LearnerState) -> ExperimentOutput:
         self.adopt(learner_state)
diff --git a/mava_amd/ops.py b/mava_amd/ops.py
--- a/mava_amd/ops.py
+++ b/mava_amd/ops.py
@@ -32,6 +32,36 @@
     _req(out, torch.int32, "out", (n,))
     check(lib().mava_permutation_i32(n, seed & (2**64 - 1), counter & (2**64 - 1), ptr(out), stream_ptr()), "mava_permutation_i32")
     return out
+
+
+def permutation_batched(n: int, seed: int, counter: int, out: torch.Tensor) -> torch.Tensor:
+    _req(out, torch.int32, "out")
+    if out.dim() != 2 or out.shape[1] != n or out.stride(1) != 1 or out.stride(0) < n:
+        raise ValueError(f"out: expected a (K, {n}) tensor with contiguous rows, got {tuple(out.shape)}")
+    check(lib().mava_permutation_batched_i32(n, seed & (2**64 - 1), counter & (2**64 - 1), out.shape[0], ptr(out),
+                                             out.stride(0), stream_ptr()), "mava_permutation_batched_i32")
+    return out
+
+
+def rollout_carry(agents_view: torch.Tensor, global_state: Optional[torch.Tensor], action_mask: torch.Tensor,
+                  step_count: torch.Tensor) -> None:
+    T1, E, A, W = agents_view.shape
+    _req(agents_view, torch.float32, "agents_view")
+    _req(action_mask, torch.uint8, "action_mask")
+    if tuple(action_mask.shape[:3]) != (T1, E, A) or action_mask.dim() != 4:
+        raise ValueError(f"action_mask: expected ({T1}, {E}, {A}, n_actions), got {tuple(action_mask.shape)}")
+    _req(step_count, torch.int32, "step_count", (T1, E, A))
+    gs_dim = 0
+    if global_state is not None and global_state.numel() > 0:
+        _req(global_state, torch.float32, "global_state")
+        if global_state.shape[0] != T1 or global_state.shape[1] != E:
+            raise ValueError(f"global_state: expected ({T1}, {E}, ...), got {tuple(global_state.shape)}")
+        gs_dim = global_state.numel() // (T1 * E)
+    if T1 < 2:
+        raise ValueError("a trajectory has at least two slots")
+    check(lib().mava_rollout_carry(T1 - 1, E, A, W, gs_dim, action_mask.shape[3], ptr(agents_view),
+                                   ptr(global_state) if gs_dim else None, ptr(action_mask), ptr(step_count), stream_ptr()),
+          "mava_rollout_carry")
 
 
 def gae(reward, value, done, last_val, gamma: float, gae_lambda: float, last_done=None, out=None, ctx: Optional[Ctx] = None):
@@ -437,7 +467,7 @@
                time_limit: int, policy_seed: int, env_seed: int, t0: int, row_offset: int, env_offset: int,
                reward_mode: int, env_state, agents_view, global_state, action_mask, obs_step_count, action, value,
                reward, log_prob, done, last_val, info_return, info_length, info_terminal, adv=None, tgt=None,
-               gamma: float = 0.99, gae_lambda: float = 0.95) -> bool:
+               gamma: float = 0.99, gae_lambda: float = 0.95, last_reward=None, last_done=None, step_counter=None) -> bool:
     W = A + O
     _req(actor_params, torch.float32, "actor_params")
     _req(critic_params, torch.float32, "critic_params")
@@ -465,15 +495,25 @@
     for name, t, dt in (("run_return", env_state.run_return, torch.float32), ("run_length", env_state.run_length, torch.int32),
                         ("ep_return", env_state.ep_return, torch.float32), ("ep_length", env_state.ep_length, torch.int32)):
         _req(t, dt, name, (E,))
-    rc = lib().mava_rollout_ff_f32(
+    args = (
         ptr(actor_params), n_actions, ptr(critic_params), int(critic_shared), E, A, O, T, time_limit,
         policy_seed & 0xFFFFFFFFFFFFFFFF, env_seed & 0xFFFFFFFFFFFFFFFF, t0 & 0xFFFFFFFF, row_offset & 0xFFFFFFFF,
         env_offset & 0xFFFFFFFF, reward_mode, ptr(env_state.step_count), ptr(env_state.run_return),
         ptr(env_state.run_length), ptr(env_state.ep_return), ptr(env_state.ep_length), ptr(agents_view),
         ptr(global_state) if critic_shared else None, ptr(action_mask), ptr(obs_step_count), ptr(action), ptr(value),
         ptr(reward), ptr(log_prob), ptr(done), ptr(last_val), ptr(info_return), ptr(info_length), ptr(info_terminal),
-        ptr(adv), ptr(tgt), gamma, gae_lambda, stream_ptr())
+        ptr(adv), ptr(tgt), gamma, gae_lambda)
+    if last_reward is None and last_done is None and step_counter is None:
+        name = "mava_rollout_ff_f32"
+        rc = lib().mava_rollout_ff_f32(*args, stream_ptr())
+    else:
+        name = "mava_rollout_ff_tail_f32"
+        _req(last_reward, torch.float32, "last_reward", (E, A))
+        _req(last_done, torch.uint8, "last_done", (E, A))
+        if step_counter is not None:
+            _req(step_counter, torch.int32, "step_counter", (1,))
+        rc = lib().mava_rollout_ff_tail_f32(*args, ptr(last_reward), ptr(last_done), ptr(step_counter), stream_ptr())
     if rc == 1:
         return False
-    check(rc, "mava_rollout_ff_f32")
+    check(rc, name)
     return True
```

New measurement: 79.88 million env-steps/s (median of 6 runs). +1.7%, better.
